# nirvanesque/headCT_foundation

Hardware: AMD Instinct MI355X
Metric: CT-volumes/sec MAE pretrain step (96^3, ViT-B/16^3, mask 0.75) (higher is better)
Workload: dtype bf16; 1 GPU; BASELINE config #2: MAE ViT-B/16^3, 96^3x1ch, mask 0.75, full train step (fwd+bwd+clip+AdamW+LR); per_gpu_batch=256, global_batch=256, parallelism=dp1, init=reference init, seed 42

## Files before the change

headct_foundation_amd/_lib.py:

```python
from __future__ import annotations

import ctypes as C
import os
from typing import Optional

HERE = os.path.dirname(os.path.abspath(__file__))
LIB_PATH = os.path.join(HERE, "libheadct_hip.so")

HCT_F32, HCT_BF16, HCT_F16 = 0, 1, 2
NORM_LAYERNORM, NORM_RMSNORM = 0, 1
HCT_ACT_NONE, HCT_ACT_GELU, HCT_ACT_DGELU, HCT_ACT_TANH, HCT_ACT_GELU_D, HCT_ACT_MULAUX = 0, 1, 2, 3, 4, 5
ACT_NONE, ACT_GELU, ACT_DGELU = 0, 1, 2

c_void_p, c_int, c_float, c_size_t, c_int64 = C.c_void_p, C.c_int, C.c_float, C.c_size_t, C.c_int64


class GemmArgs(C.Structure):
    _fields_ = [
        ("M", c_int), ("N", c_int), ("K", c_int),
        ("A", c_void_p), ("a_dtype", c_int), ("lda", c_int64), ("transA", c_int),
        ("B", c_void_p), ("b_dtype", c_int), ("ldb", c_int64), ("transB", c_int),
        ("C", c_void_p), ("c_dtype", c_int), ("ldc", c_int64),
        ("bias", c_void_p), ("residual", c_void_p), ("ldr", c_int64),
        ("act", c_int),
        ("aux", c_void_p), ("aux_dtype", c_int), ("ldaux", c_int64),
        ("C2", c_void_p), ("c2_dtype", c_int), ("ldc2", c_int64),
        ("alpha", c_float), ("force_generic", c_int), ("colsum_out", c_void_p), ("workspace_armed", c_int),
    ]


class GemmPlanInfo(C.Structure):
    _fields_ = [("kernel", c_int), ("epilogue_mode", c_int), ("fuse_colsum", c_int), ("row_tiles_per_wave", c_int), ("tiles", c_int),
                ("grid", c_int), ("sk_tiles", c_int), ("sk_wgs", c_int), ("splits", c_int), ("r_chunk", c_int), ("colsum_bytes", c_size_t),
                ("stream_k_offset", c_size_t), ("slab_bytes", c_size_t), ("workspace_bytes", c_size_t), ("walk_width", c_int)]


class ProfShape(C.Structure):
    _fields_ = [("M", c_int), ("N", c_int), ("K", c_int), ("mode", c_int), ("tiles", c_int), ("sk_tiles", c_int),
                ("launches", c_int64), ("total_ms", C.c_double), ("work", C.c_double), ("bytes", C.c_double)]


def prof_shapes(lib, kernel_class: int, cap: int = 256):
    buf = (ProfShape * cap)()
    n = lib.hct_prof_shapes(kernel_class, C.cast(buf, c_void_p), cap)
    if n < 0:
        raise HctError("hct_prof_shapes failed")
    return [buf[i] for i in range(min(n, cap))]


class MaeConfig(C.Structure):
    _fields_ = [
        ("input_size", c_int), ("patch_size", c_int), ("in_chans", c_int), ("mask_ratio", C.c_double),
        ("pos_embed", c_int),
        ("encoder_depth", c_int), ("encoder_embed_dim", c_int), ("encoder_mlp_dim", c_int), ("encoder_num_heads", c_int),
        ("decoder_depth", c_int), ("decoder_embed_dim", c_int), ("decoder_mlp_dim", c_int), ("decoder_num_heads", c_int),
        ("norm_pix_loss", c_int), ("use_bias", c_int),
        ("encoder_only", c_int), ("num_register_tokens", c_int), ("final_norm_eps", c_float),
        ("lora_rank", c_int),
        ("norm_kind", c_int),
        ("dropout_rate", c_float),
        ("drop_path_rate", c_float),
        ("patch_dropout", C.c_double),
    ]


class ParamInfo(C.Structure):
    _fields_ = [
        ("name", C.c_char * 96), ("ndim", c_int), ("shape", c_int64 * 5), ("offset", c_int64), ("numel", c_int64),
        ("requires_grad", c_int), ("is_matrix", c_int), ("bf16_t_offset", c_int64),
    ]


_PROTOS = {
    "hct_last_error_string": (C.c_char_p, []),
    "hct_version": (c_int, []),
    "hct_has_mfma_kernels": (c_int, []),
    "hct_gemm_workspace_bytes": (c_size_t, [C.POINTER(GemmArgs)]),
    "hct_gemm_nt_flags_offset": (c_size_t, [c_size_t]),
    "hct_gemm_describe": (c_int, [C.POINTER(GemmArgs), c_int, c_size_t, C.POINTER(GemmPlanInfo)]),
    "hct_gemm_stream_k_items": (c_int, [c_int, c_int, c_int, c_int, C.POINTER(C.c_uint32), C.POINTER(C.c_uint32)]),
    "hct_gemm_nt_walk": (c_int, [c_int, c_int, c_int, c_int, C.POINTER(c_int)]),
    "hct_set_cu_reserve": (None, [c_int]),
    "hct_gemm": (c_int, [C.POINTER(GemmArgs), c_void_p, c_size_t, c_void_p]),
    "hct_mask_rank": (c_int, [c_void_p, c_int, c_int, c_int, c_void_p, c_void_p, c_void_p, c_void_p]),
    "hct_patch_gather": (c_int, [c_void_p, c_int, c_void_p, c_int, c_int, c_int, c_int, c_int, c_int, c_void_p, c_int, c_void_p]),
    "hct_encoder_assemble_fwd": (c_int, [c_void_p, c_int, c_void_p, c_void_p, c_void_p, c_int, c_int, c_int, c_int, c_void_p, c_void_p]),
    "hct_encoder_assemble_bwd": (c_int, [c_void_p, c_void_p, c_int, c_int, c_int, c_int, c_void_p, c_int, c_void_p, c_void_p, c_void_p, c_size_t, c_void_p]),
    "hct_assemble_bwd_workspace_bytes": (c_size_t, [c_int]),
    "hct_layernorm_fwd": (c_int, [c_void_p, c_void_p, c_void_p, c_int, c_int, c_float, c_void_p, c_int, c_void_p, c_void_p, c_void_p]),
    "hct_layernorm_bwd_workspace_bytes": (c_size_t, [c_int, c_int]),
    "hct_layernorm_bwd": (c_int, [c_void_p, c_int, c_void_p, c_void_p, c_void_p, c_void_p, c_void_p, c_int, c_int, c_void_p, c_void_p,
                                  c_int, c_void_p, c_void_p, c_void_p, c_void_p, c_size_t, c_void_p]),
    "hct_layernorm_bwd_mapped": (c_int, [c_void_p, c_int, c_void_p, c_void_p, c_void_p, c_void_p, c_void_p, c_void_p, c_int, c_int, c_void_p,
                                         c_void_p, c_int, c_void_p, c_void_p, c_void_p, c_void_p, c_size_t, c_void_p]),
    "hct_rmsnorm_fwd": (c_int, [c_void_p, c_void_p, c_int, c_int, c_float, c_void_p, c_int, c_void_p, c_void_p]),
    "hct_rmsnorm_bwd_workspace_bytes": (c_size_t, [c_int, c_int]),
    "hct_rmsnorm_bwd": (c_int, [c_void_p, c_int, c_void_p, c_void_p, c_void_p, c_void_p, c_int, c_int, c_void_p, c_void_p, c_int, c_void_p,
                                c_void_p, c_void_p, c_size_t, c_void_p]),
    "hct_rmsnorm_bwd_mapped": (c_int, [c_void_p, c_int, c_void_p, c_void_p, c_void_p, c_void_p, c_void_p, c_int, c_int, c_void_p, c_void_p,
                                       c_int, c_void_p, c_void_p, c_void_p, c_size_t, c_void_p]),
    "hct_tail_rows": (c_int, [c_void_p, c_int, c_int, c_int, c_void_p, c_void_p, c_void_p]),
    "hct_gather_rows": (c_int, [c_void_p, c_void_p, c_int, c_int, c_void_p, c_void_p]),
    "hct_attention_fwd": (c_int, [c_void_p, c_int, c_int, c_int, c_int, c_int, c_void_p, c_void_p, c_void_p]),
    "hct_attention_bwd": (c_int, [c_void_p, c_void_p, c_void_p, c_void_p, c_int, c_int, c_int, c_int, c_int, c_void_p, c_void_p]),
    "hct_debug_force_simple_attention": (None, [c_int]),
    "hct_dropout_mask": (c_int, [C.c_uint64, c_int, c_int, c_int64, c_int, c_int, c_float, c_void_p, c_void_p]),
    "hct_dropout_apply": (c_int, [c_void_p, c_int, c_void_p, c_int, c_void_p, c_void_p, c_void_p, c_int64, c_int64, c_int64, c_int64, C.c_uint64,
                                  c_int, c_float, c_void_p]),
    "hct_attention_dropout_fwd": (c_int, [c_void_p, c_int, c_int, c_int, c_int, c_int, c_float, C.c_uint64, c_int, c_void_p, c_void_p, c_void_p]),
    "hct_attention_dropout_bwd": (c_int, [c_void_p, c_void_p, c_void_p, c_void_p, c_int, c_int, c_int, c_int, c_int, c_float, C.c_uint64, c_int,
                                          c_void_p, c_void_p]),
    "hct_drop_path_scales": (c_int, [C.c_uint64, C.POINTER(c_int), C.POINTER(c_float), c_int, c_int, c_void_p, c_void_p]),
    "hct_residual_drop_apply": (c_int, [c_void_p, c_int, c_void_p, c_int, c_void_p, c_int64, c_int64, c_void_p, C.c_uint64, c_int, c_float,
                                        c_void_p]),
    "hct_mae_plan_set_dropout": (c_int, [c_void_p, c_int, C.c_uint64]),
    "hct_decoder_assemble_fwd": (c_int, [c_void_p, c_int, c_void_p, c_void_p, c_void_p, c_void_p, c_int, c_int, c_int, c_int, c_void_p, c_void_p]),
    "hct_decoder_assemble_bwd": (c_int, [c_void_p, c_void_p, c_void_p, c_int, c_int, c_int, c_int, c_void_p, c_int, c_void_p, c_void_p,
                                         c_void_p, c_size_t, c_void_p]),
    "hct_masked_mse": (c_int, [c_void_p, c_int, c_void_p, c_int, c_void_p, c_int, c_int, c_int, c_int, c_int, c_float, c_void_p, c_void_p, c_void_p, c_void_p, c_void_p]),
    "hct_unpatchify": (c_int, [c_void_p, c_int, c_int, c_int, c_int, c_int, c_int, c_void_p, c_void_p]),
    "hct_vit_assemble_fwd": (c_int, [c_void_p, c_int, c_void_p, c_void_p, c_void_p, c_int, c_int, c_int, c_int, c_void_p, c_void_p]),
    "hct_channel_norm": (c_int, [c_void_p, c_void_p, c_void_p, c_float, c_void_p, c_int, c_int64, c_int, c_void_p]),
    "hct_query_attention": (c_int, [c_void_p, c_int, c_void_p, c_int, c_int, c_int, c_int, c_int, c_float, c_void_p, c_void_p]),
    "hct_head_linear": (c_int, [c_void_p, c_int64, c_int, c_void_p, c_void_p, c_float, c_void_p, c_void_p, c_int, c_void_p, c_int, c_int,
                                c_int, c_void_p]),
    "hct_batchnorm_stats": (c_int, [c_void_p, c_int, c_int, c_float, c_void_p, c_void_p, c_void_p, c_void_p, c_void_p]),
    "hct_softmax_xent": (c_int, [c_void_p, c_void_p, c_int, c_int, c_void_p, c_void_p, c_void_p, c_void_p]),
    "hct_sigmoid_bce_workspace_bytes": (c_size_t, [c_int, c_int]),
    "hct_sigmoid_bce": (c_int, [c_void_p, c_void_p, c_void_p, c_int, c_int, c_void_p, c_void_p, c_void_p, c_void_p, c_void_p, c_size_t, c_void_p]),
    "hct_mix_volumes": (c_int, [c_void_p, c_int, c_int, c_int, c_void_p, c_void_p, c_void_p]),
    "hct_mix_xent": (c_int, [c_void_p, c_void_p, c_void_p, c_float, c_int, c_int, c_void_p, c_void_p, c_void_p, c_void_p]),
    "hct_head_linear_wgrad": (c_int, [c_void_p, c_void_p, c_void_p, c_float, c_void_p, c_int, c_int, c_int, c_void_p, c_void_p, c_void_p]),
    "hct_bn_rows_workspace_bytes": (c_size_t, [c_int, c_int]),
    "hct_bn_stats_rows": (c_int, [c_void_p, c_int, c_int64, c_int, c_int, c_float, c_void_p, c_void_p, c_void_p, c_void_p, c_void_p,
                                  c_size_t, c_void_p]),
    "hct_bn_norm": (c_int, [c_void_p, c_int, c_int64, c_int64, c_int, c_void_p, c_void_p, c_float, c_void_p, c_int, c_void_p]),
    "hct_bn_bwd_input": (c_int, [c_void_p, c_int, c_int64, c_void_p, c_void_p, c_float, c_void_p, c_int64, c_void_p, c_void_p, c_int,
                                 c_int, c_int, c_int, c_void_p, c_int, c_int64, c_void_p, c_size_t, c_void_p]),
    "hct_head_linear_x": (c_int, [c_void_p, c_int, c_int64, c_int, c_void_p, c_void_p, c_float, c_void_p, c_void_p, c_void_p, c_int,
                                  c_int, c_int, c_void_p]),
    "hct_head_linear_bwd": (c_int, [c_void_p, c_int, c_int64, c_int, c_void_p, c_void_p, c_float, c_void_p, c_int, c_int, c_int,
                                    c_void_p, c_void_p, c_void_p]),
    "hct_query_attention_lse": (c_int, [c_void_p, c_int, c_void_p, c_int, c_int, c_int, c_int, c_int, c_float, c_void_p, c_void_p,
                                        c_void_p]),
    "hct_query_attention_bwd_workspace_bytes": (c_size_t, [c_int, c_int, c_int, c_int]),
    "hct_query_attention_bwd": (c_int, [c_void_p, c_int, c_void_p, c_int, c_int, c_int, c_int, c_int, c_float, c_void_p, c_void_p,
                                        c_void_p, c_void_p, c_void_p, c_void_p, c_size_t, c_void_p]),
    "hct_clip_total_norm": (c_int, [c_void_p, c_int64, c_void_p, c_int, c_float, c_void_p, c_void_p]),
    "hct_add_f32": (c_int, [c_void_p, c_void_p, c_int64, c_void_p]),
    "hct_dino_loss_workspace_bytes": (c_size_t, [c_int, c_int, c_int]),
    "hct_dino_loss": (c_int, [c_void_p, c_void_p, c_int, c_int, c_int, c_int, c_void_p, c_float, c_float, c_void_p, c_void_p, c_void_p, c_void_p,
                              c_void_p, c_size_t, c_void_p]),
    "hct_dino_center_update": (c_int, [c_void_p, c_void_p, c_int, C.c_double, C.c_double, c_void_p]),
    "hct_dino_sk_workspace_bytes": (c_size_t, [c_int, c_int]),
    "hct_dino_sk_col_lse": (c_int, [c_void_p, c_int, c_int, c_int, c_float, c_void_p, c_void_p, c_void_p, c_size_t, c_void_p]),
    "hct_dino_sk_row_lse": (c_int, [c_void_p, c_int, c_int, c_int, c_float, c_void_p, c_void_p, c_void_p]),
    "hct_dino_loss_sk_workspace_bytes": (c_size_t, [c_int, c_int, c_int]),
    "hct_dino_loss_sk": (c_int, [c_void_p, c_void_p, c_int, c_int, c_int, c_int, c_void_p, c_void_p, c_float, c_float, c_float, c_void_p, c_void_p,
                                 c_void_p, c_void_p, c_size_t, c_void_p]),
    "hct_koleo_fwd": (c_int, [c_void_p, c_int, c_int, c_int, c_int64, c_void_p, c_void_p, c_void_p, c_void_p, c_void_p]),
    "hct_koleo_bwd": (c_int, [c_void_p, c_int, c_int, c_int, c_int64, c_void_p, c_void_p, c_void_p, c_void_p, c_void_p, c_int64, c_void_p]),
    "hct_ema_update": (c_int, [c_void_p, c_void_p, c_int64, C.c_double, c_void_p]),
    "hct_l2norm_rows_fwd": (c_int, [c_void_p, c_int, c_int, c_void_p, c_int, c_void_p, c_void_p]),
    "hct_l2norm_rows_bwd": (c_int, [c_void_p, c_void_p, c_int, c_void_p, c_int, c_int, c_void_p, c_void_p]),
    "hct_weight_norm_fwd": (c_int, [c_void_p, c_void_p, c_int, c_int, c_void_p, c_int, c_void_p, c_void_p]),
    "hct_weight_norm_bwd": (c_int, [c_void_p, c_void_p, c_void_p, c_void_p, c_int, c_int, c_void_p, c_void_p, c_void_p]),
    "hct_bn_gelu_fwd": (c_int, [c_void_p, c_void_p, c_void_p, c_void_p, c_void_p, c_float, c_int, c_int, c_void_p, c_int, c_void_p, c_void_p, c_void_p]),
    "hct_bn_gelu_bwd_sums": (c_int, [c_void_p, c_int, c_void_p, c_void_p, c_int, c_int, c_void_p, c_void_p]),
    "hct_bn_gelu_bwd_apply": (c_int, [c_void_p, c_int, c_void_p, c_void_p, c_void_p, c_void_p, c_float, c_void_p, C.c_double, c_int, c_int, c_void_p, c_int,
                                      c_void_p]),
    "hct_hu_window": (c_int, [c_void_p, c_int, c_void_p, c_int, c_int, c_int64, c_int, c_void_p, c_void_p, c_void_p]),
    "hct_augment_volume": (c_int, [c_void_p, c_int, c_void_p, c_int, c_int, c_int, c_void_p, c_void_p, c_void_p]),
    "hct_gather_augment": (c_int, [c_void_p, c_void_p, c_void_p, c_int, c_int, c_int, c_int64, c_void_p, c_void_p, c_void_p]),
    "hct_affine_augment": (c_int, [c_void_p, c_int, c_void_p, c_int64, c_void_p, c_int, c_int, c_int, c_void_p, c_void_p, c_void_p, c_void_p,
                                   c_void_p]),
    "hct_gaussian_smooth3d": (c_int, [c_void_p, c_void_p, c_void_p, c_int, c_int, c_int, c_void_p, c_void_p, c_void_p]),
    "hct_crop_resize_area": (c_int, [c_void_p, c_int, c_int, c_int, c_int, c_void_p, c_int, c_int, c_void_p, c_void_p, c_void_p, c_void_p]),
    "hct_adjust_contrast_workspace_bytes": (c_size_t, [c_int, c_int64]),
    "hct_adjust_contrast": (c_int, [c_void_p, c_int, c_int64, c_void_p, c_void_p, c_void_p, c_size_t, c_void_p]),
    "hct_volume_to_ras": (c_int, [c_void_p, c_int, c_int, c_int, c_int, C.POINTER(c_int), C.POINTER(c_int), c_int, C.c_double, C.c_double,
                                  c_void_p, c_void_p]),
    "hct_bspline3_resample_workspace_bytes": (c_size_t, [c_int] * 6),
    "hct_bspline3_resample": (c_int, [c_void_p, c_int, c_int, c_int, c_void_p, c_int, c_int, c_int, c_void_p, c_void_p, c_void_p, c_size_t, c_void_p]),
    "hct_foreground_bbox_workspace_bytes": (c_size_t, [c_int] * 3),
    "hct_foreground_bbox": (c_int, [c_void_p, c_int, c_int, c_int, c_void_p, c_void_p, c_void_p, c_size_t, c_void_p]),
    "hct_crop_window_resize_area": (c_int, [c_void_p, c_int, c_int, c_int, c_void_p, c_int, c_void_p, c_void_p, c_void_p, c_int, c_int, c_int,
                                            c_void_p]),
# ... 154 lines not shown
```

headct_foundation_amd/csrc/attention.hip:

```cpp
#include "common.h"
#include "philox.h"
#include "prof.h"

namespace hct {
int attention_fwd_simple(const void* qkv, int B, int N, int H, int dh, int dtype, void* o, float* lse, hipStream_t s);
int attention_bwd_simple(const void* qkv, const void* o, const void* d_o, const float* lse, int B, int N, int H, int dh,
                         int dtype, void* dqkv, hipStream_t s);
bool attention_mfma_supported(int N, int H, int dh);
int attention_fwd_mfma(const void* qkv, int B, int N, int H, int dh, void* o, float* lse, hipStream_t s);
int attention_bwd_mfma(const void* qkv, const void* o, const void* d_o, const float* lse, int B, int N, int H, int dh,
                       void* dqkv, hipStream_t s);
int attention_dropout_fwd_simple(const void* qkv, int B, int N, int H, int dh, int dtype, void* o, float* lse, const DropArgs& da, hipStream_t s);
int attention_dropout_bwd_simple(const void* qkv, const void* o, const void* d_o, const float* lse, int B, int N, int H, int dh,
                                 int dtype, void* dqkv, const DropArgs& da, hipStream_t s);
int attention_dropout_fwd_mfma(const void* qkv, int B, int N, int H, int dh, void* o, float* lse, const DropArgs& da, hipStream_t s);
int attention_dropout_bwd_mfma(const void* qkv, const void* o, const void* d_o, const float* lse, int B, int N, int H, int dh, void* dqkv,
                               const DropArgs& da, hipStream_t s);
int check_drop_rate(const char* who, float p);
int g_force_simple_attention = 0;
extern int g_attn_general;
}

using namespace hct;

extern "C" {

void hct_debug_force_simple_attention(int mode) {
  g_force_simple_attention = mode == 1;
  g_attn_general = mode == 2;
}

int hct_attention_fwd(const void* qkv, int B, int N, int H, int dh, int dtype, void* o, float* lse, void* stream) {
  HCT_REQUIRE(B > 0 && N > 0 && H > 0 && dh > 0, "hct_attention_fwd: bad shape");
  ProfScope ps(PROF_ATTN_FWD, 4.0 * B * H * (double)N * N * dh, (hipStream_t)stream);
  if (dtype == HCT_BF16 && !g_force_simple_attention && attention_mfma_supported(N, H, dh))
    return attention_fwd_mfma(qkv, B, N, H, dh, o, lse, (hipStream_t)stream);
  return attention_fwd_simple(qkv, B, N, H, dh, dtype, o, lse, (hipStream_t)stream);
}

int hct_attention_bwd(const void* qkv, const void* o, const void* d_o, const float* lse, int B, int N, int H, int dh,
                      int dtype, void* dqkv, void* stream) {
  HCT_REQUIRE(B > 0 && N > 0 && H > 0 && dh > 0, "hct_attention_bwd: bad shape");
  ProfScope ps(PROF_ATTN_BWD, 10.0 * B * H * (double)N * N * dh, (hipStream_t)stream);
  if (dtype == HCT_BF16 && !g_force_simple_attention && attention_mfma_supported(N, H, dh))
    return attention_bwd_mfma(qkv, o, d_o, lse, B, N, H, dh, dqkv, (hipStream_t)stream);
  return attention_bwd_simple(qkv, o, d_o, lse, B, N, H, dh, dtype, dqkv, (hipStream_t)stream);
}

int hct_attention_dropout_fwd(const void* qkv, int B, int N, int H, int dh, int dtype, float p, uint64_t seed, int site, void* o, float* lse,
                              void* stream) {
  HCT_REQUIRE(B > 0 && N > 0 && H > 0 && dh > 0 && site >= 0, "hct_attention_dropout_fwd: bad shape or site");
  if (int rc = check_drop_rate("hct_attention_dropout_fwd", p)) return rc;
  const DropArgs da = make_drop_args(seed, site, p);
  ProfScope ps(PROF_ATTN_FWD, 4.0 * B * H * (double)N * N * dh, (hipStream_t)stream);
  if (dtype == HCT_BF16 && !g_force_simple_attention && attention_mfma_supported(N, H, dh))
    return attention_dropout_fwd_mfma(qkv, B, N, H, dh, o, lse, da, (hipStream_t)stream);
  return attention_dropout_fwd_simple(qkv, B, N, H, dh, dtype, o, lse, da, (hipStream_t)stream);
}

int hct_attention_dropout_bwd(const void* qkv, const void* o, const void* d_o, const float* lse, int B, int N, int H, int dh, int dtype, float p,
                              uint64_t seed, int site, void* dqkv, void* stream) {
  HCT_REQUIRE(B > 0 && N > 0 && H > 0 && dh > 0 && site >= 0, "hct_attention_dropout_bwd: bad shape or site");
  if (int rc = check_drop_rate("hct_attention_dropout_bwd", p)) return rc;
  const DropArgs da = make_drop_args(seed, site, p);
  ProfScope ps(PROF_ATTN_BWD, 10.0 * B * H * (double)N * N * dh, (hipStream_t)stream);
  if (dtype == HCT_BF16 && !g_force_simple_attention && attention_mfma_supported(N, H, dh))
    return attention_dropout_bwd_mfma(qkv, o, d_o, lse, B, N, H, dh, dqkv, da, (hipStream_t)stream);
  return attention_dropout_bwd_simple(qkv, o, d_o, lse, B, N, H, dh, dtype, dqkv, da, (hipStream_t)stream);
}

}
```

headct_foundation_amd/csrc/attention_mfma.hip:

```cpp
#include "common.h"
#include "philox.h"

#include <type_traits>

namespace hct {

int g_attn_general = 0;

namespace {

constexpr int kRowBytes = 128;

__device__ __forceinline__ int img_off(int r, int c) { return r * kRowBytes + ((c ^ ((r >> 1) & 7)) << 4); }

template <int DH>
__device__ __forceinline__ void load_image(unsigned char* img, const bf16* __restrict__ g, int64_t rs, int N, int Npad,
                                           int nthreads) {
  constexpr int U = 8;
  const int total = Npad * 8;
  for (int base = threadIdx.x; base < total; base += nthreads * U) {
    bf16x8 v[U];
#pragma unroll
    for (int u = 0; u < U; ++u) {
      const int idx = base + u * nthreads;
      const int r = idx >> 3, c = idx & 7;
      v[u] = bf16x8{0, 0, 0, 0, 0, 0, 0, 0};
      if (idx < total && r < N && c * 8 < DH) v[u] = *reinterpret_cast<const bf16x8*>(g + (int64_t)r * rs + c * 8);
    }
#pragma unroll
    for (int u = 0; u < U; ++u) {
      const int idx = base + u * nthreads;
      if (idx < total) *reinterpret_cast<bf16x8*>(img + img_off(idx >> 3, idx & 7)) = v[u];
    }
  }
}

__device__ __forceinline__ void dma_image128(unsigned char* img, const bf16* __restrict__ g, int64_t rs, int N, int Npad, int valid_cols,
                                             int wave, int nwaves, int lane) {
  const int64_t bytes = ((int64_t)(N - 1) * rs + valid_cols) * 2;
  __amdgpu_buffer_rsrc_t rsrc = __builtin_amdgcn_make_buffer_rsrc((void*)g, 0, bytes > 0xFFFFFFFFll ? 0xFFFFFFFFu : (uint32_t)bytes, 0x00020000);
  const int pieces = Npad * 8 / 64;
  for (int p = wave; p < pieces; p += nwaves) {
    const int ci = p * 64 + lane;
    const int row = ci >> 3, slot = ci & 7;
    const uint32_t voff = (uint32_t)(row * (int)rs * 2 + ((slot ^ ((row >> 1) & 7)) << 4));
    __builtin_amdgcn_raw_ptr_buffer_load_lds(rsrc, (__attribute__((address_space(3))) void*)(img + p * 1024), 16, voff, 0, 0, 0);
  }
}

template <int DH>
__device__ __forceinline__ void compute_delta(const bf16* __restrict__ ob, const bf16* __restrict__ dob, int64_t os,
                                              const float* __restrict__ lse_row, int N, int Npad, float* sLse, float* sDel,
                                              int nthreads, float lse_mul = 1.44269504088896340736f, float del_mul = 1.0f) {
  constexpr int U = 4;
  const int total = Npad * 8;
  for (int base = threadIdx.x; base < total; base += nthreads * U) {
    bf16x8 a[U], d[U];
#pragma unroll
    for (int u = 0; u < U; ++u) {
      const int idx = base + u * nthreads;
      const int r = idx >> 3, c = idx & 7;
      a[u] = d[u] = bf16x8{0, 0, 0, 0, 0, 0, 0, 0};
      if (idx < total && r < N && c * 8 < DH) {
        a[u] = *reinterpret_cast<const bf16x8*>(ob + (int64_t)r * os + c * 8);
        d[u] = *reinterpret_cast<const bf16x8*>(dob + (int64_t)r * os + c * 8);
      }
    }
#pragma unroll
    for (int u = 0; u < U; ++u) {
      const int idx = base + u * nthreads;
      float part = 0.f;
#pragma unroll
      for (int e = 0; e < 8; ++e) part += (float)a[u][e] * (float)d[u][e];
      part += __shfl_xor(part, 1, 64);
      part += __shfl_xor(part, 2, 64);
      part += __shfl_xor(part, 4, 64);
      if (idx < total && (idx & 7) == 0) {
        const int r = idx >> 3;
        sDel[r] = r < N ? part * del_mul : 0.f;
        sLse[r] = r < N ? lse_row[r] * lse_mul : (lse_mul < 0.f ? -INFINITY : INFINITY);
      }
    }
  }
}

__device__ __forceinline__ bf16x8 frag_row(const unsigned char* img, int r0, int ks, int lane) {
  const int r = r0 + (lane & 15), c = ks * 4 + (lane >> 4);
  return *reinterpret_cast<const bf16x8*>(img + img_off(r, c));
}

__device__ __forceinline__ bf16x8 frag_tr(const unsigned char* img, int rA, int rB, int d0, int lane) {
  const int g = lane >> 4, qq = (lane & 15) >> 2, pp = lane & 3;
  const int c = (d0 >> 3) + (pp >> 1), sub = (pp & 1) * 8;
  const unsigned char* pa = img + img_off(rA + 4 * g + qq, c) + sub;
  const unsigned char* pb = img + img_off(rB + 4 * g + qq, c) + sub;
  s16x4 lo = __builtin_amdgcn_ds_read_tr16_b64_v4i16((__attribute__((address_space(3))) s16x4*)(pa));
  s16x4 hi = __builtin_amdgcn_ds_read_tr16_b64_v4i16((__attribute__((address_space(3))) s16x4*)(pb));
  typedef __attribute__((ext_vector_type(8))) short s16x8;
  s16x8 v = {lo[0], lo[1], lo[2], lo[3], hi[0], hi[1], hi[2], hi[3]};
  return __builtin_bit_cast(bf16x8, v);
}

__device__ __forceinline__ bf16x8 pack8(f32x4 a, f32x4 b) {
  bf16x8 v = {(bf16)a[0], (bf16)a[1], (bf16)a[2], (bf16)a[3], (bf16)b[0], (bf16)b[1], (bf16)b[2], (bf16)b[3]};
  return v;
}

#define MFMA(a, b, c) __builtin_amdgcn_mfma_f32_16x16x32_bf16(a, b, c, 0, 0, 0)

__device__ __forceinline__ int xcd_bh() {
  const int n = gridDim.x, i = blockIdx.x;
  const int xcd = i & 7, q = n >> 3, r = n & 7;
  return (xcd < r ? xcd * (q + 1) : r * (q + 1) + (xcd - r) * q) + (i >> 3);
}

template <int DH, bool DROP = false>
__global__ void __launch_bounds__(256) attn_fwd_mfma_kernel(const bf16* __restrict__ qkv, int N, int H, int Npad,
                                                            bf16* __restrict__ o, float* __restrict__ lse, DropArgs da = DropArgs{}) {
  extern __shared__ __attribute__((aligned(16))) unsigned char smem[];
  unsigned char* Kimg = smem;
  unsigned char* Vimg = smem + Npad * kRowBytes;
  const int lane = threadIdx.x & 63, wave = threadIdx.x >> 6;
  const int bh = xcd_bh(), b = bh / H, h = bh - b * H;
  const int64_t rs = (int64_t)3 * H * DH;
  const bf16* qb = qkv + (int64_t)b * N * rs + h * DH;
  load_image<DH>(Kimg, qb + H * DH, rs, N, Npad, 256);
  load_image<DH>(Vimg, qb + 2 * H * DH, rs, N, Npad, 256);
  __syncthreads();
  const float scale = rsqrtf((float)DH);
  const int g = lane >> 4;
  constexpr int ND = DH / 16;
  const int nqt = (N + 15) >> 4;
  for (int qt = wave; qt < nqt; qt += 4) {
    const int q = qt * 16 + (lane & 15);
    bf16x8 qf[2];
#pragma unroll
    for (int ks = 0; ks < 2; ++ks) {
      const int d = ks * 32 + 8 * g;
      bf16x8 v = {0, 0, 0, 0, 0, 0, 0, 0};
      if (q < N && d < DH) v = *reinterpret_cast<const bf16x8*>(qb + (int64_t)q * rs + d);
      qf[ks] = v;
    }
    float m = -INFINITY, lsum = 0.f;
    f32x4 oacc[ND];
#pragma unroll
    for (int dt = 0; dt < ND; ++dt) oacc[dt] = f32x4{0, 0, 0, 0};
    for (int s = 0; s < (Npad >> 5); ++s) {
      const int k0 = s * 32;
      f32x4 st0 = {0, 0, 0, 0}, st1 = {0, 0, 0, 0};
#pragma unroll
      for (int ks = 0; ks < 2; ++ks) {
        st0 = MFMA(frag_row(Kimg, k0, ks, lane), qf[ks], st0);
        st1 = MFMA(frag_row(Kimg, k0 + 16, ks, lane), qf[ks], st1);
      }
      float mx = -INFINITY;
#pragma unroll
      for (int r = 0; r < 4; ++r) {
        st0[r] = (k0 + 4 * g + r < N) ? st0[r] * scale : -INFINITY;
        st1[r] = (k0 + 16 + 4 * g + r < N) ? st1[r] * scale : -INFINITY;
        mx = fmaxf(mx, fmaxf(st0[r], st1[r]));
      }
      mx = fmaxf(mx, __shfl_xor(mx, 16, 64));
      mx = fmaxf(mx, __shfl_xor(mx, 32, 64));
      const float mnew = fmaxf(m, mx);
      const float corr = __expf(m - mnew);
      float ps = 0.f;
#pragma unroll
      for (int r = 0; r < 4; ++r) {
        st0[r] = __expf(st0[r] - mnew);
        st1[r] = __expf(st1[r] - mnew);
        ps += st0[r] + st1[r];
      }
      lsum = lsum * corr + ps;
      if constexpr (DROP) {
        const Philox4 z0 = drop_words_attn(da, (uint32_t)((k0 >> 2) + g), (uint32_t)q, (uint32_t)bh);
        const Philox4 z1 = drop_words_attn(da, (uint32_t)((k0 >> 2) + 4 + g), (uint32_t)q, (uint32_t)bh);
#pragma unroll
        for (int r = 0; r < 4; ++r) {
          st0[r] *= drop_mul(da, z0.w[r]);
          st1[r] *= drop_mul(da, z1.w[r]);
        }
      }
      const bf16x8 pb = pack8(st0, st1);
#pragma unroll
      for (int dt = 0; dt < ND; ++dt) {
        oacc[dt] = oacc[dt] * corr;
        oacc[dt] = MFMA(frag_tr(Vimg, k0, k0 + 16, dt * 16, lane), pb, oacc[dt]);
      }
      m = mnew;
    }
    lsum += __shfl_xor(lsum, 16, 64);
    lsum += __shfl_xor(lsum, 32, 64);
    if (q < N) {
      const float inv = 1.0f / lsum;
      bf16* orow = o + ((int64_t)b * N + q) * (H * DH) + h * DH + 4 * g;
#pragma unroll
      for (int dt = 0; dt < ND; ++dt) Vec4<bf16>::store(orow + dt * 16, oacc[dt] * inv);
      if (g == 0) lse[(int64_t)bh * N + q] = m + __logf(lsum);
    }
  }
}

template <int DH, int NT, int NW = (NT <= 4 ? 4 : 8)>
__global__ void __launch_bounds__(NW * 64) attn_fwd_row_kernel(const bf16* __restrict__ qkv, int N, int H, bf16* __restrict__ o,
                                                           float* __restrict__ lse) {
  constexpr int Npad = NT * 16;
  extern __shared__ __attribute__((aligned(16))) unsigned char smem[];
  unsigned char* Kimg = smem;
  unsigned char* Vimg = smem + Npad * kRowBytes;
  const int lane = threadIdx.x & 63, wave = threadIdx.x >> 6;
  const int bh = xcd_bh(), b = bh / H, h = bh - b * H;
  const int64_t rs = (int64_t)3 * H * DH;
  const bf16* qb = qkv + (int64_t)b * N * rs + h * DH;
  const int g = lane >> 4;
  constexpr int ND = DH / 16;
  constexpr int MAXT = (NT + NW - 1) / NW;
  const int nqt = (N + 15) >> 4;
  constexpr int QA = MAXT <= 2 ? MAXT : 1;
  bf16x8 qall[QA][2];
  auto load_q = [&](int it, bf16x8* dst) {
    const int q = (wave + it * NW) * 16 + (lane & 15);
#pragma unroll
    for (int ks = 0; ks < 2; ++ks) {
      const int d = ks * 32 + 8 * g;
      bf16x8 v = {0, 0, 0, 0, 0, 0, 0, 0};
      if (q < N && d < DH) v = *reinterpret_cast<const bf16x8*>(qb + (int64_t)q * rs + d);
      dst[ks] = v;
    }
  };
#pragma unroll
  for (int it = 0; it < QA; ++it) load_q(it, qall[it]);
  dma_image128(Kimg, qb + H * DH, rs, N, Npad, DH, wave, NW, lane);
  dma_image128(Vimg, qb + 2 * H * DH, rs, N, Npad, DH, wave, NW, lane);
  __syncthreads();
  const float scale = rsqrtf((float)DH) * 1.44269504088896340736f;
#pragma unroll
  for (int it = 0; it < MAXT; ++it) {
    const int qt = wave + it * NW;
    if (qt >= nqt) break;
    const int q = qt * 16 + (lane & 15);
    bf16x8 qf[2];
    if constexpr (MAXT <= 2) { qf[0] = qall[it][0]; qf[1] = qall[it][1]; }
    else if (it == 0) { qf[0] = qall[0][0]; qf[1] = qall[0][1]; }
    else load_q(it, qf);
    f32x4 st[NT];
#pragma unroll
    for (int t = 0; t < NT; ++t) {
      st[t] = MFMA(frag_row(Kimg, t * 16, 0, lane), qf[0], (f32x4{0, 0, 0, 0}));
      st[t] = MFMA(frag_row(Kimg, t * 16, 1, lane), qf[1], st[t]);
    }
    constexpr int kPrevNT = NT <= 4 ? 0 : NT <= 10 ? 4 : NT <= 14 ? 10 : NT <= 18 ? 14 : 18;
    float mraw = -INFINITY;
#pragma unroll
    for (int t = 0; t < NT; ++t)
#pragma unroll
      for (int r = 0; r < 4; ++r) {
        if (t >= kPrevNT && t * 16 + 4 * g + r >= N) st[t][r] = -INFINITY;
        mraw = fmaxf(mraw, st[t][r]);
      }
    mraw = fmaxf(mraw, __shfl_xor(mraw, 16, 64));
    mraw = fmaxf(mraw, __shfl_xor(mraw, 32, 64));
    const float mx = mraw * scale;
#pragma unroll
    for (int t = 0; t < NT; ++t)
#pragma unroll
      for (int r = 0; r < 4; ++r) st[t][r] = __builtin_amdgcn_exp2f(fmaf(st[t][r], scale, -mx));
    const bf16 one = (bf16)1.0f, zero = (bf16)0.0f, ov = (lane & 3) == 0 ? one : zero;
    const bf16x8 ones_rows = {ov, ov, ov, ov, ov, ov, ov, ov};
    f32x4 oacc[ND], psum = {0, 0, 0, 0};
#pragma unroll
    for (int dt = 0; dt < ND; ++dt) oacc[dt] = f32x4{0, 0, 0, 0};
#pragma unroll
    for (int s2 = 0; s2 < NT / 2; ++s2) {
      const bf16x8 pb = pack8(st[2 * s2], st[2 * s2 + 1]);
#pragma unroll
      for (int dt = 0; dt < ND; ++dt) oacc[dt] = MFMA(frag_tr(Vimg, s2 * 32, s2 * 32 + 16, dt * 16, lane), pb, oacc[dt]);
      psum = MFMA(ones_rows, pb, psum);
    }
    const float ps = psum[0];
    if (q < N) {
      const float inv = 1.0f / ps;
      bf16* orow = o + ((int64_t)b * N + q) * (H * DH) + h * DH + 4 * g;
#pragma unroll
      for (int dt = 0; dt < ND; ++dt) Vec4<bf16>::store(orow + dt * 16, oacc[dt] * inv);
      if (g == 0) lse[(int64_t)bh * N + q] = (mx + __builtin_amdgcn_logf(ps)) * 0.69314718055994530942f;
    }
  }
}

template <int DH>
__device__ __forceinline__ bf16x8 gfrag(const bf16* __restrict__ base, int64_t rs, int r0, int ks, int lane, int N) {
  const int r = r0 + (lane & 15), d = ks * 32 + 8 * (lane >> 4);
  bf16x8 v = {0, 0, 0, 0, 0, 0, 0, 0};
  if (r < N && d < DH) v = *reinterpret_cast<const bf16x8*>(base + (int64_t)r * rs + d);
  return v;
}

constexpr int kBwd2WavesPerEU = 4;
template <int DH, int NW, bool DROP = false>
__global__ void __launch_bounds__(NW * 64, (NW >= 8 ? kBwd2WavesPerEU : 2)) attn_bwd2_mfma_kernel(const bf16* __restrict__ qkv, const bf16* __restrict__ o,
                                                                const bf16* __restrict__ d_o, const float* __restrict__ lse,
                                                                int N, int H, int Npad, bf16* __restrict__ dqkv, DropArgs da = DropArgs{}) {
  extern __shared__ __attribute__((aligned(16))) unsigned char smem[];
  unsigned char* img0 = smem;
  unsigned char* img1 = smem + Npad * kRowBytes;
  float* sLse = reinterpret_cast<float*>(img1 + Npad * kRowBytes);
  float* sDel = sLse + Npad;
  const int lane = threadIdx.x & 63, wave = threadIdx.x >> 6;
  const int bh = xcd_bh(), b = bh / H, h = bh - b * H;
  const int64_t rs = (int64_t)3 * H * DH;
  const int64_t os = (int64_t)H * DH;
  const bf16* qb = qkv + (int64_t)b * N * rs + h * DH;
  const bf16* kb = qb + H * DH;
  const bf16* vb = qb + 2 * H * DH;
  const bf16* ob = o + (int64_t)b * N * os + h * DH;
  const bf16* dob = d_o + (int64_t)b * N * os + h * DH;
  const float scale = rsqrtf((float)DH);
  const float scale2 = scale * 1.44269504088896340736f;
  const int g = lane >> 4;
  constexpr int ND = DH / 16;
  const int npair = Npad >> 5;

  constexpr bool kAhead = DH != 64;
  bf16x8 kf[2], vf[2], kn[2], vn[2];
#pragma unroll
  for (int ks = 0; ks < 2; ++ks) {
    kf[ks] = gfrag<DH>(kb, rs, wave * 16, ks, lane, N);
    vf[ks] = gfrag<DH>(vb, rs, wave * 16, ks, lane, N);
  }
  load_image<DH>(img0, qb, rs, N, Npad, NW * 64);
  load_image<DH>(img1, dob, os, N, Npad, NW * 64);
  compute_delta<DH>(ob, dob, os, lse + (int64_t)bh * N, N, Npad, sLse, sDel, NW * 64, 1.44269504088896340736f, scale);
  __syncthreads();
  for (int kt = wave; kt * 16 < N; kt += NW) {
    const int key0 = kt * 16;
#pragma unroll
    for (int ks = 0; ks < 2; ++ks) {
      if (kAhead) {
        kn[ks] = gfrag<DH>(kb, rs, key0 + NW * 16, ks, lane, N);
        vn[ks] = gfrag<DH>(vb, rs, key0 + NW * 16, ks, lane, N);
      } else if (kt != wave) {
        kf[ks] = gfrag<DH>(kb, rs, key0, ks, lane, N);
        vf[ks] = gfrag<DH>(vb, rs, key0, ks, lane, N);
      }
    }
    const bool key_ok = key0 + (lane & 15) < N;
    const bool tail_tile = key0 + 16 > N;
    f32x4 dKt[ND], dVt[ND];
#pragma unroll
    for (int dt = 0; dt < ND; ++dt) dKt[dt] = dVt[dt] = f32x4{0, 0, 0, 0};
    for (int qp = 0; qp < npair; ++qp) {
      f32x4 P[2], dS[2];
      [[maybe_unused]] f32x4 Pz[2];
#pragma unroll
      for (int hh = 0; hh < 2; ++hh) {
        const int q0 = qp * 32 + hh * 16;
        f32x4 sacc = {0, 0, 0, 0}, dp = {0, 0, 0, 0};
#pragma unroll
        for (int ks = 0; ks < 2; ++ks) {
          sacc = MFMA(frag_row(img0, q0, ks, lane), kf[ks], sacc);
          dp = MFMA(frag_row(img1, q0, ks, lane), vf[ks], dp);
        }
        const f32x4 L4 = *reinterpret_cast<const f32x4*>(sLse + q0 + 4 * g);
        const f32x4 D4 = *reinterpret_cast<const f32x4*>(sDel + q0 + 4 * g);
#pragma unroll
        for (int r = 0; r < 4; ++r) {
          float pv = __builtin_amdgcn_exp2f(fmaf(sacc[r], scale2, -L4[r]));
// ... 267 lines not shown
            for (int r = 0; r < 4; ++r) {
              P[hh][r] = hct_prob(__builtin_amdgcn_exp2f(sacc[r] * scale2));
              dS[hh][r] = P[hh][r] * dp[r];
            }
          }
          const bf16x8 pa = pack8(P[0], P[1]);
          const bf16x8 dsa = pack8(dS[0], dS[1]);
          const bf16x4 d0 = {dsa[0], dsa[1], dsa[2], dsa[3]}, d1 = {dsa[4], dsa[5], dsa[6], dsa[7]};
          if (key0 < Npad) {
            *reinterpret_cast<bf16x4*>(dsT + dst_off(Npad, 0, key, g)) = d0;
            *reinterpret_cast<bf16x4*>(dsT + dst_off(Npad, 1, key, g)) = d1;
          }
#pragma unroll
          for (int dt = 0; dt < ND; ++dt) {
            if constexpr (kHoist) {
              dVt[t][dt] = MFMA(dT[dt], pa, dVt[t][dt]);
              dKt[t][dt] = MFMA(qT[dt], dsa, dKt[t][dt]);
            } else {
              dVt[t][dt] = MFMA(cols_lds<DH>(Dimg, q0, q0 + 16, dt * 16, lane), pa, dVt[t][dt]);
              dKt[t][dt] = MFMA(cols_lds<DH>(Qimg, q0, q0 + 16, dt * 16, lane), dsa, dKt[t][dt]);
            }
          }
        }
      }
    }
    __syncthreads();
    for (int dt = wave; dt < ND; dt += GS) {
      f32x4 dq0 = {0, 0, 0, 0}, dq1 = {0, 0, 0, 0};
      const int G = lane >> 4, qq = (lane & 15) >> 2, pp = lane & 3;
      auto ds_frag = [&](int hh, int k0) -> bf16x8 {
        const int ka = k0 + 4 * G + qq;
        s16x4 lo = __builtin_amdgcn_ds_read_tr16_b64_v4i16((__attribute__((address_space(3))) s16x4*)(dsT + dst_off(Npad, hh, ka, pp)));
        s16x4 hi = __builtin_amdgcn_ds_read_tr16_b64_v4i16((__attribute__((address_space(3))) s16x4*)(dsT + dst_off(Npad, hh, ka + 16, pp)));
        typedef __attribute__((ext_vector_type(8))) short s16x8;
        s16x8 v = {lo[0], lo[1], lo[2], lo[3], hi[0], hi[1], hi[2], hi[3]};
        return __builtin_bit_cast(bf16x8, v);
      };
      bf16x8 kT = cols_lds<DH>(Kimg, 0, 16, dt * 16, lane), b0 = ds_frag(0, 0), b1 = ds_frag(1, 0);
      for (int k0 = 32; k0 < Npad; k0 += 32) {
        const bf16x8 kTn = cols_lds<DH>(Kimg, k0, k0 + 16, dt * 16, lane), b0n = ds_frag(0, k0), b1n = ds_frag(1, k0);
        dq0 = MFMA(kT, b0, dq0);
        dq1 = MFMA(kT, b1, dq1);
        kT = kTn; b0 = b0n; b1 = b1n;
      }
      dq0 = MFMA(kT, b0, dq0);
      dq1 = MFMA(kT, b1, dq1);
      const int q = q0 + (lane & 15);
      if (q < N) Vec4<bf16>::store(dqkv + ((int64_t)b * N + q) * rs + h * DH + dt * 16 + 4 * g, dq0 * scale);
      if (q + 16 < N) Vec4<bf16>::store(dqkv + ((int64_t)b * N + q + 16) * rs + h * DH + dt * 16 + 4 * g, dq1 * scale);
    }
    __syncthreads();
  }
#pragma unroll
  for (int t = 0; t < KT; ++t) {
    const int key = key_base + t * 16 + (lane & 15);
    if (key < N) {
      bf16* outk = dqkv + ((int64_t)b * N + key) * rs + H * DH + h * DH + 4 * g;
      bf16* outv = outk + H * DH;
#pragma unroll
      for (int dt = 0; dt < ND; ++dt) {
        Vec4<bf16>::store(outk + dt * 16, dKt[t][dt] * scale);
        Vec4<bf16>::store(outv + dt * 16, dVt[t][dt]);
      }
    }
  }
}

template <int DH>
inline size_t bwd3_lds(int Npad) { return (size_t)3 * Npad * HeadImg<DH>::kRow + (size_t)2 * Npad * 32 + (size_t)2 * Npad * sizeof(float); }


typedef __attribute__((ext_vector_type(4))) int attn_i32x4;
typedef __attribute__((ext_vector_type(2))) unsigned int u32x2a;
__device__ __forceinline__ attn_i32x4 attn_srd(const void* base, int64_t bytes) {
  const uint64_t pa = (uint64_t)base;
  const uint32_t rec = bytes > 0xFFFFFFFFll ? 0xFFFFFFFFu : (bytes < 0 ? 0u : (uint32_t)bytes);
  return attn_i32x4{(int)__builtin_amdgcn_readfirstlane((uint32_t)pa), (int)(__builtin_amdgcn_readfirstlane((uint32_t)(pa >> 32)) & 0xFFFF),
                    (int)__builtin_amdgcn_readfirstlane(rec), 0x00020000};
}
__device__ __forceinline__ void attn_dma16(attn_i32x4 rsrc, uint32_t lds_base, uint32_t voff) {
  asm volatile("s_mov_b32 m0, %0\n\ts_nop 0\n\tbuffer_load_dwordx4 %1, %2, 0 offen lds" ::"s"(lds_base), "v"(voff), "s"(rsrc) : "memory", "m0");
}

template <int DH, int Npad, int KT = 2>
__global__ void __launch_bounds__(1024 / KT, 2 * 2 / KT) attn_bwd4_kernel(const bf16* __restrict__ qkv, const bf16* __restrict__ o,
                                                           const bf16* __restrict__ d_o, const float* __restrict__ lse, int N, int H,
                                                           bf16* __restrict__ dqkv, int nbh) {
  extern __shared__ __attribute__((aligned(16))) unsigned char smem[];
  constexpr int ROW = HeadImg<DH>::kRow, CH = HeadImg<DH>::kChunks, ND = DH / 16, NW = 16 / KT;
  constexpr int img = Npad * ROW;
  constexpr int bufsz = 3 * img + 32 + 2 * Npad * 4;
  unsigned char* const dsT0 = smem + 2 * bufsz;
  constexpr int dstsz = 2 * Npad * 32;
  const uint32_t lds0 = (uint32_t)(size_t)((__attribute__((address_space(3))) unsigned char*)smem);
  const int lane = threadIdx.x & 63, wave = __builtin_amdgcn_readfirstlane(threadIdx.x >> 6);
  const int64_t rs = (int64_t)3 * H * DH, os = (int64_t)H * DH;
  const float scale = rsqrtf((float)DH);
  const float scale2 = scale * 1.44269504088896340736f;
  const int key_base = wave * (KT * 16);
  constexpr int nqb = Npad >> 5;
  constexpr int pieces = Npad * CH / 64;
  constexpr int MAXP = (pieces + NW - 1) / NW;
  auto opaque = [](int v) { asm volatile("" : "+v"(v)); return v; };
  if (threadIdx.x < 16) {
    *reinterpret_cast<uint32_t*>(smem + (threadIdx.x >> 3) * bufsz + 3 * img + (threadIdx.x & 7) * 4) = 0u;
  }
  auto item_bh = [&](int item) {
    const int xcd = item & 7, q = nbh >> 3, r = nbh & 7;
    return (xcd < r ? xcd * (q + 1) : r * (q + 1) + (xcd - r) * q) + (item >> 3);
  };
  int dq_hh, dq_dt0, dq_n;
  if (KT == 1) {
    dq_hh = wave - (NW - 2); dq_dt0 = 0; dq_n = wave >= NW - 2 ? ND : 0;
  } else if (key_base >= Npad) { dq_hh = 0; dq_dt0 = 0; dq_n = ND; }
  else if (8 * KT * 16 > Npad) { dq_hh = 1; dq_dt0 = wave - 4; dq_n = (wave >= 4 && wave < 4 + ND) ? 1 : 0; }
  else { dq_hh = (wave - 2) / ND; dq_dt0 = (wave - 2) - dq_hh * ND; dq_n = wave >= 2 ? 1 : 0; }

  auto prefetch_images = [&](int item, int buf) {
    const int bh = item_bh(item), b = bh / H, h = bh - b * H;
    const bf16* qb = qkv + (int64_t)b * N * rs + h * DH;
    const bf16* dob = d_o + (int64_t)b * N * os + h * DH;
    const attn_i32x4 rq = attn_srd(qb, ((int64_t)(N - 1) * rs + DH) * 2);
    const attn_i32x4 rk = attn_srd(qb + H * DH, ((int64_t)(N - 1) * rs + DH) * 2);
    const attn_i32x4 rd = attn_srd(dob, ((int64_t)(N - 1) * os + DH) * 2);
    const uint32_t base = lds0 + buf * bufsz;
    const int ln = opaque(lane);
#pragma unroll
    for (int i = 0; i < MAXP; ++i) {
      const int p = wave + NW * i;
      if (p < pieces) {
        const int ci = p * 64 + ln, row = ci / CH, slot = ci - row * CH;
        const uint32_t src = (uint32_t)((DH == 48 ? slot : (slot ^ ((row >> 1) & 7))) * 16);
        const uint32_t vq = (uint32_t)row * (uint32_t)(rs * 2) + src, vd = (uint32_t)row * (uint32_t)(os * 2) + src;
        attn_dma16(rq, base + p * 1024, vq);
        attn_dma16(rd, base + img + p * 1024, vd);
        attn_dma16(rk, base + 2 * img + p * 1024, vq);
      }
    }
  };
  RowFrag<DH> vfN[KT];
  constexpr int NU = (Npad * 8 + NW * 64 - 1) / (NW * 64);
  bf16x8 oN[NU];
  float lN = 0.f;
  auto prefetch_regs = [&](int item) {
    const int bh = item_bh(item), b = bh / H, h = bh - b * H;
    const bf16* vb = qkv + (int64_t)b * N * rs + 2 * H * DH + h * DH;
    const int ln = opaque(lane), tid = wave * 64 + ln;
#pragma unroll
    for (int t = 0; t < KT; ++t) vfN[t] = rows_global<DH>(vb, rs, key_base + t * 16, ln, N);
    const bf16* ob = o + (int64_t)b * N * os + h * DH;
#pragma unroll
    for (int u = 0; u < NU; ++u) {
      const int idx = tid + u * NW * 64, r = idx >> 3, c = idx & 7;
      oN[u] = bf16x8{0, 0, 0, 0, 0, 0, 0, 0};
      if (r < N && c * 8 < DH) oN[u] = *reinterpret_cast<const bf16x8*>(ob + (int64_t)r * os + c * 8);
    }
    lN = tid < N ? lse[(int64_t)bh * N + tid] : 0.f;
  };

  int item = blockIdx.x;
  if (item >= nbh) return;
  prefetch_images(item, 0);
  prefetch_regs(item);
  for (int it = 0; item < nbh; item += gridDim.x, ++it) {
    const int cur = it & 1;
    unsigned char* Qimg = smem + cur * bufsz;
    unsigned char* Dimg = Qimg + img;
    unsigned char* Kimg = Dimg + img;
    float* sLse = reinterpret_cast<float*>(Kimg + img + 32);
    float* sDel = sLse + Npad;
    const int bh = item_bh(item), b = bh / H, h = bh - b * H;
    asm volatile("" ::"v"(lN) : "memory");
    __builtin_amdgcn_s_barrier();
    RowFrag<DH> vf[KT];
#pragma unroll
    for (int t = 0; t < KT; ++t) vf[t] = vfN[t];
    RowFrag<DH> kfh = vf[0];
    if constexpr (KT == 1) kfh = rows_lds<DH>(Kimg, key_base < Npad ? key_base : 0, opaque(lane), true);
    const int tid_top = wave * 64 + opaque(lane);
#pragma unroll
    for (int u = 0; u < NU; ++u) {
      const int idx = tid_top + u * NW * 64, r = idx >> 3, c = idx & 7;
      float part = 0.f;
      if (idx < Npad * 8 && c * 8 < DH) {
        const bf16x8 dv = *reinterpret_cast<const bf16x8*>(Dimg + HeadImg<DH>::off(r, c));
#pragma unroll
        for (int e = 0; e < 8; ++e) part += (float)oN[u][e] * (float)dv[e];
      }
      part += __shfl_xor(part, 1, 64);
      part += __shfl_xor(part, 2, 64);
      part += __shfl_xor(part, 4, 64);
      if (idx < Npad * 8 && c == 0) sDel[r] = r < N ? part * scale : 0.f;
    }
    if (tid_top < Npad) sLse[tid_top] = tid_top < N ? lN * 1.44269504088896340736f : INFINITY;
    asm volatile("s_waitcnt lgkmcnt(0)" ::: "memory");
    __builtin_amdgcn_s_barrier();
    const int next = item + gridDim.x;
    if (next < nbh) prefetch_images(next, cur ^ 1);

    f32x4 dKt[KT][ND], dVt[KT][ND];
#pragma unroll
    for (int t = 0; t < KT; ++t)
#pragma unroll
      for (int dt = 0; dt < ND; ++dt) dKt[t][dt] = dVt[t][dt] = f32x4{0, 0, 0, 0};

    auto main_part = [&](int qbk) {
      const int q0 = qbk * 32;
      unsigned char* dsT = dsT0 + (qbk & 1) * dstsz;
      const int ln = KT == 1 ? opaque(lane) : lane, g = ln >> 4;
      RowFrag<DH> qr[2], dr[2];
      f32x4 L4[2], D4[2];
      if constexpr (KT > 1) {
#pragma unroll
        for (int hh = 0; hh < 2; ++hh) {
          qr[hh] = rows_lds<DH>(Qimg, q0 + 16 * hh, ln, true);
          dr[hh] = rows_lds<DH>(Dimg, q0 + 16 * hh, ln, false);
          L4[hh] = *reinterpret_cast<const f32x4*>(sLse + q0 + 16 * hh + 4 * g);
          D4[hh] = *reinterpret_cast<const f32x4*>(sDel + q0 + 16 * hh + 4 * g);
        }
      }
      bf16x8 qT[ND], dT[ND];
#pragma unroll
      for (int dt = 0; dt < ND; ++dt) {
        qT[dt] = cols_lds<DH>(Qimg, q0, q0 + 16, dt * 16, ln);
        dT[dt] = cols_lds<DH>(Dimg, q0, q0 + 16, dt * 16, ln);
      }
#pragma unroll
      for (int t = 0; t < KT; ++t) {
        const int key0 = key_base + t * 16;
        const RowFrag<DH> kf = KT == 1 ? kfh : rows_lds<DH>(Kimg, key0, ln, false);
        const int key = key0 + (ln & 15);
        f32x4 P[2], dS[2];
#pragma unroll
        for (int hh = 0; hh < 2; ++hh) {
          if constexpr (KT == 1) {
            qr[hh] = rows_lds<DH>(Qimg, q0 + 16 * hh, ln, false);
            dr[hh] = rows_lds<DH>(Dimg, q0 + 16 * hh, ln, false);
            L4[hh] = *reinterpret_cast<const f32x4*>(sLse + q0 + 16 * hh + 4 * g);
            D4[hh] = *reinterpret_cast<const f32x4*>(sDel + q0 + 16 * hh + 4 * g);
          }
          const f32x4 sacc = mma_rows<DH>(qr[hh], kf, f32x4{0, 0, 0, 0});
          const f32x4 dp = mma_rows<DH>(dr[hh], vf[t], f32x4{0, 0, 0, 0});
#pragma unroll
          for (int r = 0; r < 4; ++r) {
            P[hh][r] = hct_prob(__builtin_amdgcn_exp2f(fmaf(sacc[r], scale2, -L4[hh][r])));
            dS[hh][r] = P[hh][r] * fmaf(dp[r], scale, -D4[hh][r]);
          }
        }
        const bf16x8 pa = pack8(P[0], P[1]);
        const bf16x8 dsa = pack8(dS[0], dS[1]);
        const bf16x4 d0 = {dsa[0], dsa[1], dsa[2], dsa[3]}, d1 = {dsa[4], dsa[5], dsa[6], dsa[7]};
        *reinterpret_cast<bf16x4*>(dsT + dst_off(Npad, 0, key, g)) = d0;
        *reinterpret_cast<bf16x4*>(dsT + dst_off(Npad, 1, key, g)) = d1;
#pragma unroll
        for (int dt = 0; dt < ND; ++dt) {
          dVt[t][dt] = MFMA(dT[dt], pa, dVt[t][dt]);
          dKt[t][dt] = MFMA(qT[dt], dsa, dKt[t][dt]);
        }
      }
    };
    auto dq_tiles = [&](int qbk, int hh, int dt0, auto nt_tag, int ln) {
      constexpr int NT = decltype(nt_tag)::value;
      const unsigned char* dsT = dsT0 + (qbk & 1) * dstsz;
      const int qq = (ln & 15) >> 2, pp = ln & 3, g = ln >> 4;
      auto ds_frag = [&](int k0) -> bf16x8 {
        const int ka = k0 + 4 * g + qq;
        s16x4 lo = __builtin_amdgcn_ds_read_tr16_b64_v4i16((__attribute__((address_space(3))) s16x4*)(dsT + dst_off(Npad, hh, ka, pp)));
        s16x4 hi = __builtin_amdgcn_ds_read_tr16_b64_v4i16((__attribute__((address_space(3))) s16x4*)(dsT + dst_off(Npad, hh, ka + 16, pp)));
        typedef __attribute__((ext_vector_type(8))) short s16x8;
        s16x8 v = {lo[0], lo[1], lo[2], lo[3], hi[0], hi[1], hi[2], hi[3]};
        return __builtin_bit_cast(bf16x8, v);
      };
      f32x4 dq[NT];
#pragma unroll
      for (int j = 0; j < NT; ++j) dq[j] = f32x4{0, 0, 0, 0};
      constexpr int kHalf = (KT == 1 && NT > 1) ? (nqb + 1) / 2 : nqb;
#pragma unroll
      for (int k0 = 0; k0 < nqb; k0 += kHalf) {
        bf16x8 kT[kHalf][NT], bq[kHalf];
#pragma unroll
        for (int kb = 0; kb < kHalf; ++kb)
          if (k0 + kb < nqb) {
            bq[kb] = ds_frag((k0 + kb) * 32);
#pragma unroll
            for (int j = 0; j < NT; ++j) kT[kb][j] = cols_lds<DH>(Kimg, (k0 + kb) * 32, (k0 + kb) * 32 + 16, (dt0 + j) * 16, ln);
          }
#pragma unroll
        for (int kb = 0; kb < kHalf; ++kb)
          if (k0 + kb < nqb) {
#pragma unroll
            for (int j = 0; j < NT; ++j) dq[j] = MFMA(kT[kb][j], bq[kb], dq[j]);
          }
      }
      const int q = qbk * 32 + 16 * hh + (ln & 15);
#pragma unroll
      for (int j = 0; j < NT; ++j)
        if (q < N) Vec4<bf16>::store(dqkv + ((int64_t)b * N + q) * rs + h * DH + (dt0 + j) * 16 + 4 * g, dq[j]);
    };
    auto dq_part = [&](int qbk, int ln) {
      if (dq_n == 1) dq_tiles(qbk, dq_hh, dq_dt0, std::integral_constant<int, 1>{}, ln);
      else if (dq_n == ND) dq_tiles(qbk, dq_hh, dq_dt0, std::integral_constant<int, ND>{}, ln);
    };
    const bool owns_keys = key_base < Npad;
    for (int qbk = 0; qbk < nqb; ++qbk) {
      if (wave < NW / 2) {
        if (owns_keys) main_part(qbk);
        if (qbk > 0) dq_part(qbk - 1, KT == 1 ? opaque(lane) : lane);
      } else {
        if (qbk > 0) dq_part(qbk - 1, KT == 1 ? opaque(lane) : lane);
        if (owns_keys) main_part(qbk);
      }
      asm volatile("s_waitcnt lgkmcnt(0)" ::: "memory");
      __builtin_amdgcn_s_barrier();
    }
    if (next < nbh) prefetch_regs(next);
    dq_part(nqb - 1, opaque(lane));
    if (owns_keys) {
      const int ln = opaque(lane);
#pragma unroll
      for (int t = 0; t < KT; ++t) {
        const int key = key_base + t * 16 + (ln & 15);
        if (key < N) {
          bf16* outk = dqkv + ((int64_t)b * N + key) * rs + H * DH + h * DH + 4 * (ln >> 4);
          bf16* outv = outk + H * DH;
#pragma unroll
          for (int dt = 0; dt < ND; ++dt) {
            Vec4<bf16>::store(outk + dt * 16, dKt[t][dt]);
            Vec4<bf16>::store(outv + dt * 16, dVt[t][dt]);
          }
        }
      }
    }
  }
}

template <int DH, int KT>
__global__ void __launch_bounds__(256, 1) attn_bwd5_kernel(const bf16* __restrict__ qkv, const bf16* __restrict__ o,
                                                           const bf16* __restrict__ d_o, const float* __restrict__ lse, int N, int H,
                                                           int Npad, bf16* __restrict__ dqkv) {
  extern __shared__ __attribute__((aligned(16))) unsigned char smem[];
  constexpr int ROW = HeadImg<DH>::kRow, CH = HeadImg<DH>::kChunks, ND = DH / 16;
  constexpr int blk = 32 * ROW;
  unsigned char* const Kimg = smem;
  unsigned char* const ring = Kimg + Npad * ROW + 32;
  unsigned char* const dsT0 = ring + 4 * blk + 32;
  constexpr int kRows = 4 * KT * 16;
  constexpr int dstsz = 2 * kRows * 32;
  float* const sLse = reinterpret_cast<float*>(dsT0 + 2 * dstsz);
  float* const sDel = sLse + 64;
  const int lane = threadIdx.x & 63, wave = __builtin_amdgcn_readfirstlane(threadIdx.x >> 6);
  const int bh = xcd_bh(), b = bh / H, h = bh - b * H;
  const int64_t rs = (int64_t)3 * H * DH, os = (int64_t)H * DH;
  const bf16* qb = qkv + (int64_t)b * N * rs + h * DH;
  const bf16* kb = qb + H * DH;
  const bf16* vb = qb + 2 * H * DH;
  const bf16* ob = o + (int64_t)b * N * os + h * DH;
  const bf16* dob = d_o + (int64_t)b * N * os + h * DH;
  const float* lse_row = lse + (int64_t)bh * N;
  const float scale = rsqrtf((float)DH);
  const float scale2 = scale * 1.44269504088896340736f;
  const int g = lane >> 4;
  const int key_base = wave * (KT * 16);
  const int nqb = Npad >> 5;

  for (int i = threadIdx.x * 16; i < 4 * blk + 32; i += 256 * 16) *reinterpret_cast<f32x4*>(ring + i) = f32x4{0, 0, 0, 0};
  if (threadIdx.x < 2) *reinterpret_cast<f32x4*>(Kimg + Npad * ROW + threadIdx.x * 16) = f32x4{0, 0, 0, 0};
  dma_image<DH>(Kimg, kb, rs, N, Npad, wave, 4, lane);
  RowFrag<DH> vf[KT];
#pragma unroll
  for (int t = 0; t < KT; ++t) vf[t] = rows_global<DH>(vb, rs, key_base + t * 16, lane, N);

  const int srow = threadIdx.x >> 3, sc = threadIdx.x & 7;
  bf16x8 sq, sd, so;
  float sl = 0.f;
  auto stage_load = [&](int j) {
    const int r = j * 32 + srow;
    sq = sd = so = bf16x8{0, 0, 0, 0, 0, 0, 0, 0};
    if (r < N && sc < CH) {
      sq = *reinterpret_cast<const bf16x8*>(qb + (int64_t)r * rs + sc * 8);
      sd = *reinterpret_cast<const bf16x8*>(dob + (int64_t)r * os + sc * 8);
      so = *reinterpret_cast<const bf16x8*>(ob + (int64_t)r * os + sc * 8);
    }
    const int rl = j * 32 + (int)threadIdx.x;
    sl = (threadIdx.x < 32 && rl < N) ? lse_row[rl] : 0.f;
  };
  auto stage_write = [&](int j) {
    unsigned char* Qb = ring + (j & 1) * 2 * blk;
    if (sc < CH) {
      *reinterpret_cast<bf16x8*>(Qb + HeadImg<DH>::off(srow, sc)) = sq;
      *reinterpret_cast<bf16x8*>(Qb + blk + HeadImg<DH>::off(srow, sc)) = sd;
    }
    float part = 0.f;
#pragma unroll
    for (int e = 0; e < 8; ++e) part += (float)so[e] * (float)sd[e];
    part += __shfl_xor(part, 1, 64);
    part += __shfl_xor(part, 2, 64);
    part += __shfl_xor(part, 4, 64);
// ... 88 lines not shown
      constexpr int D = 4;
      bf16x8 kT[D], b0[D], b1[D];
#pragma unroll
      for (int u = 0; u < D; ++u) {
        const int k0 = u * 32 < Npad ? u * 32 : 0;
        kT[u] = cols_lds<DH>(Kimg, k0, k0 + 16, dt * 16, lane);
        b0[u] = ds_frag(0, k0);
        b1[u] = ds_frag(1, k0);
      }
      for (int k0 = 0; k0 < Npad; k0 += 32 * D) {
#pragma unroll
        for (int u = 0; u < D; ++u) {
          if (k0 + u * 32 < Npad) {
            dq0 = MFMA(kT[u], b0[u], dq0);
            dq1 = MFMA(kT[u], b1[u], dq1);
          }
          const int kn = k0 + (u + D) * 32;
          if (kn < Npad) {
            kT[u] = cols_lds<DH>(Kimg, kn, kn + 16, dt * 16, lane);
            b0[u] = ds_frag(0, kn);
            b1[u] = ds_frag(1, kn);
          }
        }
      }
      const int q = j * 32 + (lane & 15);
      if (q < N) Vec4<bf16>::store(dqkv + ((int64_t)b * N + q) * rs + h * DH + dt * 16 + 4 * g, dq0);
      if (q + 16 < N) Vec4<bf16>::store(dqkv + ((int64_t)b * N + q + 16) * rs + h * DH + dt * 16 + 4 * g, dq1);
    }
  };

  for (int j = 0; j < nqb; ++j) {
    if (j + 1 < nqb) stage_load(j + 1);
    main_part(j);
    if (j > 0) dq_part(j - 1);
    if (j + 1 < nqb) stage_write(j + 1);
    asm volatile("s_waitcnt lgkmcnt(0)" ::: "memory");
    __builtin_amdgcn_s_barrier();
  }
  dq_part(nqb - 1);
#pragma unroll
  for (int t = 0; t < KT; ++t) {
    const int key = key_base + t * 16 + (lane & 15);
    if (key < N) {
      bf16* outk = dqkv + ((int64_t)b * N + key) * rs + H * DH + h * DH + 4 * g;
      bf16* outv = outk + H * DH;
#pragma unroll
      for (int dt = 0; dt < ND; ++dt) {
        Vec4<bf16>::store(outk + dt * 16, dKt[t][dt]);
        Vec4<bf16>::store(outv + dt * 16, dVt[t][dt]);
      }
    }
  }
}
template <int DH>
inline size_t bwd5_lds(int Npad, int KT) { return (size_t)Npad * HeadImg<DH>::kRow + 32 + (size_t)4 * 32 * HeadImg<DH>::kRow + 32 + (size_t)2 * 2 * (4 * KT * 16) * 32 + 512; }

template <int DH>
constexpr size_t bwd4_lds(int Npad) { return (size_t)2 * (3 * Npad * HeadImg<DH>::kRow + 32 + 2 * Npad * 4) + (size_t)2 * (2 * Npad * 32); }

inline size_t bwd2_lds(int N) { return (size_t)2 * ((N + 31) / 32 * 32) * kRowBytes + (size_t)2 * ((N + 31) / 32 * 32) * sizeof(float); }

constexpr int kMaxLds = 160 * 1024;
inline int npad_of(int N) { return (N + 31) / 32 * 32; }
inline size_t fwd_lds(int N) { return (size_t)2 * npad_of(N) * kRowBytes; }

template <typename F>
int set_lds(F func, size_t bytes) {
  if (bytes <= 64 * 1024) return 0;
  return check_hip(hipFuncSetAttribute(reinterpret_cast<const void*>(func), hipFuncAttributeMaxDynamicSharedMemorySize, (int)bytes),
                   "hipFuncSetAttribute(LDS)");
}

}

bool attention_mfma_supported(int N, int H, int dh) {
  (void)H;
  return (dh == 48 || dh == 64) && fwd_lds(N) <= (size_t)kMaxLds && bwd2_lds(N) <= (size_t)kMaxLds;
}

template <int DH, int NT>
static int launch_fwd_row(const void* qkv, int B, int N, int H, void* o, float* lse, hipStream_t s) {
  const size_t lds = (size_t)2 * NT * 16 * kRowBytes;
  if (int rc = set_lds(attn_fwd_row_kernel<DH, NT>, lds)) return rc;
  hipLaunchKernelGGL((attn_fwd_row_kernel<DH, NT>), dim3(B * H), dim3(NT <= 4 ? 256 : 512), lds, s, (const bf16*)qkv, N, H, (bf16*)o, lse);
  return check_hip(hipGetLastError(), "attention_fwd_row");
}

static int num_cus_cached() {
  static int n = 0;
  if (n == 0) {
    int dev = 0;
    hipDeviceProp_t prop;
    n = (hipGetDevice(&dev) == hipSuccess && hipGetDeviceProperties(&prop, dev) == hipSuccess) ? prop.multiProcessorCount : 256;
  }
  return n;
}

int attention_fwd_mfma(const void* qkv, int B, int N, int H, int dh, void* o, float* lse, hipStream_t s) {
  const int Npad = npad_of(N);
  const size_t lds = fwd_lds(N);
  if (!g_attn_general) {
    const int nt = Npad / 16;
#define HCT_ROW(DH_, NT_) if (dh == DH_ && nt <= NT_) return launch_fwd_row<DH_, NT_>(qkv, B, N, H, o, lse, s)
    HCT_ROW(64, 4); HCT_ROW(48, 4); HCT_ROW(64, 10); HCT_ROW(48, 10); HCT_ROW(64, 14); HCT_ROW(48, 14); HCT_ROW(64, 18); HCT_ROW(48, 18);
    HCT_ROW(64, 34); HCT_ROW(48, 34);
#undef HCT_ROW
  }
  if (dh == 48) {
    if (int rc = set_lds(attn_fwd_mfma_kernel<48>, lds)) return rc;
    hipLaunchKernelGGL(attn_fwd_mfma_kernel<48>, dim3(B * H), dim3(256), lds, s, (const bf16*)qkv, N, H, Npad, (bf16*)o, lse, DropArgs{});
  } else {
    if (int rc = set_lds(attn_fwd_mfma_kernel<64>, lds)) return rc;
    hipLaunchKernelGGL(attn_fwd_mfma_kernel<64>, dim3(B * H), dim3(256), lds, s, (const bf16*)qkv, N, H, Npad, (bf16*)o, lse, DropArgs{});
  }
  return check_hip(hipGetLastError(), "attention_fwd_mfma");
}

int attention_bwd_mfma(const void* qkv, const void* o, const void* d_o, const float* lse, int B, int N, int H, int dh,
                       void* dqkv, hipStream_t s) {
  const int Npad = npad_of(N);
  const int ncu = num_cus_cached();
  const int nbh = B * H, grid = nbh < ncu ? nbh : ncu;
#define HCT_BWD4(DH_, NPAD_)                                                                                                  \
  do {                                                                                                                     \
    constexpr size_t l4 = bwd4_lds<DH_>(NPAD_);                                                                            \
    static_assert(l4 <= (size_t)kMaxLds, "bwd4 LDS");                                                                      \
    if (int rc = set_lds(attn_bwd4_kernel<DH_, NPAD_, 1>, l4)) return rc;                                                  \
    hipLaunchKernelGGL((attn_bwd4_kernel<DH_, NPAD_, 1>), dim3(grid), dim3(1024), l4, s, (const bf16*)qkv, (const bf16*)o, \
                       (const bf16*)d_o, lse, N, H, (bf16*)dqkv, nbh);                                                     \
    return check_hip(hipGetLastError(), "attention_bwd4");                                                                 \
  } while (0)
  if (!g_attn_general) {
    if (dh == 64 && Npad == 160) HCT_BWD4(64, 160);
    if (dh == 48 && Npad == 224) HCT_BWD4(48, 224);
    if (dh == 64 && Npad <= 64) {
      const size_t l3 = bwd3_lds<64>(Npad);
      if (int rc = set_lds(attn_bwd3_kernel<64, 4, 1, 4>, l3)) return rc;
      hipLaunchKernelGGL((attn_bwd3_kernel<64, 4, 1, 4>), dim3(B * H), dim3(4 * 64), l3, s, (const bf16*)qkv, (const bf16*)o,
                         (const bf16*)d_o, lse, N, H, Npad, (bf16*)dqkv, ncu, (int)(Npad * Npad / 4096));
      return check_hip(hipGetLastError(), "attention_bwd3");
    }
    if (dh == 48 && Npad > 448 && Npad <= 576) {
      const size_t l5 = bwd5_lds<48>(Npad, 9);
      if (int rc = set_lds(attn_bwd5_kernel<48, 9>, l5)) return rc;
      hipLaunchKernelGGL((attn_bwd5_kernel<48, 9>), dim3(B * H), dim3(256), l5, s, (const bf16*)qkv, (const bf16*)o, (const bf16*)d_o,
                         lse, N, H, Npad, (bf16*)dqkv);
      return check_hip(hipGetLastError(), "attention_bwd5");
    }
  }
#undef HCT_BWD4
  const size_t l2 = bwd2_lds(N);
#define HCT_BWD2(DH_, NW_)                                                                                           \
  do {                                                                                                               \
    if (int rc = set_lds(attn_bwd2_mfma_kernel<DH_, NW_>, l2)) return rc;                                            \
    hipLaunchKernelGGL((attn_bwd2_mfma_kernel<DH_, NW_>), dim3(B * H), dim3(NW_ * 64), l2, s, (const bf16*)qkv,       \
                       (const bf16*)o, (const bf16*)d_o, lse, N, H, Npad, (bf16*)dqkv, DropArgs{});                  \
  } while (0)
  const bool w8 = N > 64;
  const bool w16 = w8 && l2 > (size_t)81408;
  if (dh == 48) { if (w16) HCT_BWD2(48, 16); else if (w8) HCT_BWD2(48, 8); else HCT_BWD2(48, 4); }
  else { if (w16) HCT_BWD2(64, 16); else if (w8) HCT_BWD2(64, 8); else HCT_BWD2(64, 4); }
#undef HCT_BWD2
  return check_hip(hipGetLastError(), "attention_bwd2_mfma");
}

int attention_dropout_fwd_mfma(const void* qkv, int B, int N, int H, int dh, void* o, float* lse, const DropArgs& da, hipStream_t s) {
  const int Npad = npad_of(N);
  const size_t lds = fwd_lds(N);
  if (dh == 48) {
    if (int rc = set_lds(attn_fwd_mfma_kernel<48, true>, lds)) return rc;
    hipLaunchKernelGGL((attn_fwd_mfma_kernel<48, true>), dim3(B * H), dim3(256), lds, s, (const bf16*)qkv, N, H, Npad, (bf16*)o, lse, da);
  } else {
    if (int rc = set_lds(attn_fwd_mfma_kernel<64, true>, lds)) return rc;
    hipLaunchKernelGGL((attn_fwd_mfma_kernel<64, true>), dim3(B * H), dim3(256), lds, s, (const bf16*)qkv, N, H, Npad, (bf16*)o, lse, da);
  }
  return check_hip(hipGetLastError(), "attention_dropout_fwd_mfma");
}

int attention_dropout_bwd_mfma(const void* qkv, const void* o, const void* d_o, const float* lse, int B, int N, int H, int dh, void* dqkv,
                               const DropArgs& da, hipStream_t s) {
  const int Npad = npad_of(N);
  const size_t l2 = bwd2_lds(N);
#define HCT_BWD2D(DH_, NW_)                                                                                                 \
  do {                                                                                                                      \
    if (int rc = set_lds(attn_bwd2_mfma_kernel<DH_, NW_, true>, l2)) return rc;                                             \
    hipLaunchKernelGGL((attn_bwd2_mfma_kernel<DH_, NW_, true>), dim3(B * H), dim3(NW_ * 64), l2, s, (const bf16*)qkv,       \
                       (const bf16*)o, (const bf16*)d_o, lse, N, H, Npad, (bf16*)dqkv, da);                                 \
  } while (0)
  const bool w8 = N > 64, w16 = w8 && l2 > (size_t)81408;
  if (dh == 48) { if (w16) HCT_BWD2D(48, 16); else if (w8) HCT_BWD2D(48, 8); else HCT_BWD2D(48, 4); }
  else { if (w16) HCT_BWD2D(64, 16); else if (w8) HCT_BWD2D(64, 8); else HCT_BWD2D(64, 4); }
#undef HCT_BWD2D
  return check_hip(hipGetLastError(), "attention_dropout_bwd_mfma");
}

}
```

headct_foundation_amd/csrc/mae_plan.hip:

```cpp
#include <cstdlib>
#include "common.h"
#include "gemm_plan.h"

#include <algorithm>
#include <map>
#include <string>
#include <vector>

using namespace hct;

namespace {

constexpr int64_t kUnitElems = 1024;

struct BlockP {
  int ln1_w, ln1_b, qkv_w, qkv_b, proj_w, proj_b, ln2_w, ln2_b, fc1_w, fc1_b, fc2_w, fc2_b;
  int lq_b = -1, lq_a = -1, lv_b = -1, lv_a = -1;
  int site = 0;
  float path_q = 0.f;
  int path_row = 0;
};
struct BlockA {
  size_t x1, mean1, rstd1, qkv, o, lse, h_mid, x2, mean2, rstd2, u, g;
  size_t lora_t = 0;
};
struct Act { size_t off; int64_t rows, cols; int dtype; };
struct BlockG { size_t out, big, mid, qkv, lora_du = 0, lora_dt = 0, dm_out = 0, dm_mid = 0; };
constexpr int kWgSlots = 8;

struct Side {
  const std::vector<BlockP>& bp;
  const std::vector<BlockA>& ba;
  const std::vector<BlockG>& ring;
  const std::vector<size_t>& h;
  int N, d, m, heads;
};
enum class Rows {
  kEvery,
  kCat,
  kTail,
};
struct Mode {
  bool can = false;
  bool on = false;
  bool fwd = false;
};
struct SinkScope {
  FoldSink* prev;
  explicit SinkScope(FoldSink* sink) : prev(g_fold_sink) { g_fold_sink = sink; }
  ~SinkScope() { g_fold_sink = prev; }
};

}

struct hct_mae_plan {
  hct_mae_config cfg;
  int B, dt;
  int g, L, K, pd, Ne, Nd, Me, Md;
  int D, Dd, Mlp, Mlpd, H, Hd;
  std::vector<hct_param_info> params;
  std::map<std::string, int> pindex;
  int64_t param_elems = 0, bf16t_elems = 0;
  bool vit = false;
  bool keep = false;
  int R = 0;
  int lora = 0;
  int norm_kind = 0;
  float drop_p = 0.f;
  Mode drop;
  uint64_t drop_seed = 0;
  size_t s_drop_y = 0;
  Mode path;
  size_t s_path = 0;
  bool t_all_done = false;
  float norm_eps = 1e-5f;
  int p_reg = -1;
  int p_pe_w, p_pe_b, p_pos, p_cls, p_norm_w, p_norm_b, p_de_w, p_de_b, p_mask, p_dcls, p_dpos, p_dnorm_w, p_dnorm_b,
      p_pred_w, p_pred_b;
  std::vector<BlockP> enc, dec;
  std::vector<std::pair<int64_t, int64_t>> stage_range;
  size_t ws_bytes = 0;
  size_t a_ids_restore, a_ids_shuffle, a_mask, a_row_loss, a_patches, a_tok, a_latent, a_lat_mean, a_lat_rstd, a_e,
      a_ynorm, a_yn_mean, a_yn_rstd, a_pred, a_dpred;
  Mode tail;
  int Mc = 0;
  size_t a_tail_rows = 0, a_tail_inv = 0, a_oc = 0, s_dhc = 0;
  Mode dec0;
  int Rcat = 0;
  size_t a_kept_rows = 0, a_cat_idx = 0, a_hk = 0, a_x1c = 0, a_mean_c = 0, a_rstd_c = 0, a_qkv_cat = 0, a_dqkv_cat = 0, a_dcat = 0;
  std::vector<size_t> h_enc, h_dec;
  std::vector<BlockA> aenc, adec;
  size_t s_dh, s_dh_shadow, s_dx, s_do, s_small, s_small_bytes, s_gemm, s_gemm_bytes, s_nt_bytes = 0;
  size_t s_fold_a = 0, s_fold_b = 0, s_fold_bytes = 0, s_small2 = 0, s_small2_bytes = 0;
  bool defer_folds = true;
  std::map<std::string, Act> acts;
  bool wg_defer = false;
  int wg_blocks = 0;
  int wg_blocks_pending = 0, wg_slot = 0;
  std::vector<BlockG> genc, gdec;
  size_t a_de = 0, a_dtok = 0;
  std::vector<hct_gemm_args> wg_pending;
  std::vector<hct_gemm_args> wg_prepared[kWgSlots];
  size_t s_wg[kWgSlots] = {0}, s_wg_bytes = 0;
  int64_t final_off = 0;
  float* params_f32 = nullptr;
  float* grads = nullptr;
  bf16* params_bf16 = nullptr;
  bf16* params_bf16_t = nullptr;
  unsigned char* ws = nullptr;
  bool fwd_done = false;
  bool nt_ws_armed = false;
  bool dpred_done = false;
  const float* dloss = nullptr;

  size_t esz() const { return dtype_size(dt); }
  template <typename T> T* W(size_t off) const { return reinterpret_cast<T*>(ws + off); }
  const float* pf(int i) const { return i < 0 ? nullptr : params_f32 + params[i].offset; }
  float* gf(int i) const { return i < 0 ? nullptr : grads + params[i].offset; }
  const void* wop(int i) const { return dt == HCT_BF16 ? (const void*)(params_bf16 + params[i].offset) : (const void*)(params_f32 + params[i].offset); }
  const void* wop_t(int i) const { return (const void*)(params_bf16_t + params[i].bf16_t_offset); }
  int tr(int i) const { return i >= 0 && params[i].requires_grad ? i : -1; }
  Side enc_side() const { return Side{enc, aenc, genc, h_enc, Ne, D, Mlp, H}; }
  Side dec_side() const { return Side{dec, adec, gdec, h_dec, Nd, Dd, Mlpd, Hd}; }
  size_t out_grad(const Side& sd, int i) const { return i >= 0 ? sd.ring[i % sd.ring.size()].out : s_dh_shadow; }
  bool path_drops(const BlockP& bp) const { return path.fwd && bp.path_q > 0.f; }
  bool masks_residual(const BlockP& bp) const { return drop.fwd || path_drops(bp); }
  Rows decoder_rows(int i) const {
    return dec0.fwd && i == 0 ? Rows::kCat : tail.fwd && i == cfg.decoder_depth - 1 ? Rows::kTail : Rows::kEvery;
  }
};

namespace {

int add_param(hct_mae_plan* p, const std::string& name, std::vector<int64_t> shape, bool rg, bool matrix, bool needs_t) {
  hct_param_info pi;
  memset(&pi, 0, sizeof(pi));
  snprintf(pi.name, sizeof(pi.name), "%s", name.c_str());
  pi.ndim = (int)shape.size();
  int64_t n = 1;
  for (size_t i = 0; i < shape.size(); ++i) { pi.shape[i] = shape[i]; n *= shape[i]; }
  pi.numel = n;
  pi.offset = p->param_elems;
  pi.requires_grad = rg ? 1 : 0;
  pi.is_matrix = matrix ? 1 : 0;
  pi.bf16_t_offset = -1;
  if (needs_t) {
    pi.bf16_t_offset = p->bf16t_elems;
    p->bf16t_elems += (n + 63) / 64 * 64;
  }
  p->param_elems += (n + kUnitElems - 1) / kUnitElems * kUnitElems;
  p->params.push_back(pi);
  p->pindex[name] = (int)p->params.size() - 1;
  return (int)p->params.size() - 1;
}

BlockP add_block(hct_mae_plan* p, const std::string& pre, int d, int m, bool use_bias) {
  BlockP b;
  b.ln1_w = add_param(p, pre + ".att_norm.weight", {d}, true, false, false);
  b.ln1_b = p->norm_kind == 1 ? -1 : add_param(p, pre + ".att_norm.bias", {d}, true, false, false);
  b.qkv_w = add_param(p, pre + ".attn.qkv.weight", {3 * d, d}, true, true, true);
  b.qkv_b = use_bias ? add_param(p, pre + ".attn.qkv.bias", {3 * d}, true, false, false) : -1;
  b.proj_w = add_param(p, pre + ".attn.proj.weight", {d, d}, true, true, true);
  b.proj_b = add_param(p, pre + ".attn.proj.bias", {d}, true, false, false);
  if (p->lora > 0) {
    const int r = p->lora;
    b.lq_b = add_param(p, pre + ".attn.lora_q.lora_matrix_B", {d, r}, true, true, true);
    b.lv_b = add_param(p, pre + ".attn.lora_v.lora_matrix_B", {d, r}, true, true, true);
    b.lq_a = add_param(p, pre + ".attn.lora_q.lora_matrix_A", {r, d}, true, true, true);
    b.lv_a = add_param(p, pre + ".attn.lora_v.lora_matrix_A", {r, d}, true, true, true);
  }
  b.ln2_w = add_param(p, pre + ".ffn_norm.weight", {d}, true, false, false);
  b.ln2_b = p->norm_kind == 1 ? -1 : add_param(p, pre + ".ffn_norm.bias", {d}, true, false, false);
  b.fc1_w = add_param(p, pre + ".mlp.linear1.weight", {m, d}, true, true, true);
  b.fc1_b = add_param(p, pre + ".mlp.linear1.bias", {m}, true, false, false);
  b.fc2_w = add_param(p, pre + ".mlp.linear2.weight", {d, m}, true, true, true);
  b.fc2_b = add_param(p, pre + ".mlp.linear2.bias", {d}, true, false, false);
  return b;
}

constexpr int kMaxT = 112;
struct TransposeTable {
  int n;
  int tile_start[kMaxT + 1];
  int rows[kMaxT], cols[kMaxT];
  long long src[kMaxT], dst[kMaxT];
};

__global__ void __launch_bounds__(256) transpose_cast_batched_kernel(const float* __restrict__ src, bf16* __restrict__ dst,
                                                                     TransposeTable t) {
  __shared__ float tile[64][65];
  int lo = 0, hi = t.n;
  while (hi - lo > 1) {
    const int mid = (lo + hi) >> 1;
    if (t.tile_start[mid] <= (int)blockIdx.x) lo = mid; else hi = mid;
  }
  const int rows = t.rows[lo], cols = t.cols[lo];
  const int local = blockIdx.x - t.tile_start[lo];
  const int tcols = (cols + 63) >> 6;
  const int r0 = (local / tcols) * 64, c0 = (local % tcols) * 64;
  const float* s = src + t.src[lo];
  bf16* d = dst + t.dst[lo];
  const int q = threadIdx.x & 15, rr = threadIdx.x >> 4;
  const bool vec = (cols & 3) == 0 && (rows & 3) == 0;
  if (vec) {
#pragma unroll
    for (int i = 0; i < 4; ++i) {
      const int r = r0 + rr + 16 * i, c = c0 + q * 4;
      f32x4 v = {0, 0, 0, 0};
      if (r < rows && c < cols) v = Vec4<float>::load(s + (size_t)r * cols + c);
#pragma unroll
      for (int e = 0; e < 4; ++e) tile[rr + 16 * i][q * 4 + e] = v[e];
    }
    __syncthreads();
#pragma unroll
    for (int i = 0; i < 4; ++i) {
      const int c = c0 + rr + 16 * i, r = r0 + q * 4;
      if (c < cols && r < rows) {
        const f32x4 v = {tile[q * 4 + 0][rr + 16 * i], tile[q * 4 + 1][rr + 16 * i], tile[q * 4 + 2][rr + 16 * i], tile[q * 4 + 3][rr + 16 * i]};
        Vec4<bf16>::store(d + (size_t)c * rows + r, v);
      }
    }
    return;
  }
  const int tx = threadIdx.x & 63, ty = threadIdx.x >> 6;
  for (int i = ty; i < 64; i += 4) {
    const int r = r0 + i, c = c0 + tx;
    tile[i][tx] = (r < rows && c < cols) ? s[(size_t)r * cols + c] : 0.f;
  }
  __syncthreads();
  for (int i = ty; i < 64; i += 4) {
    const int c = c0 + i, r = r0 + tx;
    if (c < cols && r < rows) d[(size_t)c * rows + r] = (bf16)tile[tx][i];
  }
}

struct WsAlloc {
  size_t cur = 0;
  size_t take(size_t bytes) {
    size_t o = cur;
    cur += align_up(bytes ? bytes : 16, 256);
    return o;
  }
};

BlockA alloc_block(WsAlloc& w, size_t M, size_t d, size_t m, size_t heads_tokens, size_t es) {
  BlockA a;
  a.x1 = w.take(M * d * es);
  a.mean1 = w.take(M * 4);
  a.rstd1 = w.take(M * 4);
  a.qkv = w.take(M * 3 * d * es);
  a.o = w.take(M * d * es);
  a.lse = w.take(heads_tokens * 4);
  a.h_mid = w.take(M * d * 4);
  a.x2 = w.take(M * d * es);
  a.mean2 = w.take(M * 4);
  a.rstd2 = w.take(M * 4);
  a.u = w.take(M * m * es);
  a.g = w.take(M * m * es);
  return a;
}

#define RC(x)            \
  do {                   \
    int _rc = (x);       \
    if (_rc) return _rc; \
  } while (0)

constexpr float kRmsEps = 1e-6f;

int norm_fwd(hct_mae_plan* p, const float* x, const float* gamma, const float* beta, int rows, int D, float eps, void* y, int y_dtype,
             float* mean, float* rstd, hipStream_t s) {
  if (p->norm_kind == 1) return hct_rmsnorm_fwd(x, gamma, rows, D, kRmsEps, y, y_dtype, rstd, s);
  return hct_layernorm_fwd(x, gamma, beta, rows, D, eps, y, y_dtype, mean, rstd, s);
}

int norm_bwd(hct_mae_plan* p, const void* dy, int dy_dtype, const float* x, const float* mean, const float* rstd, const float* gamma,
             const float* dres, const int32_t* dres_rows, int rows, int D, float* dx, void* dx_shadow, int shadow_dtype, float* dgamma,
             float* dbeta, float* dcolsum, void* workspace, size_t workspace_bytes, hipStream_t s) {
  if (p->norm_kind == 1)
    return hct_rmsnorm_bwd_mapped(dy, dy_dtype, x, rstd, gamma, dres, dres_rows, rows, D, dx, dx_shadow, shadow_dtype, dgamma, dcolsum,
                                  workspace, workspace_bytes, s);
  return hct_layernorm_bwd_mapped(dy, dy_dtype, x, mean, rstd, gamma, dres, dres_rows, rows, D, dx, dx_shadow, shadow_dtype, dgamma, dbeta,
                                  dcolsum, workspace, workspace_bytes, s);
}

hct_gemm_args base_args() {
  hct_gemm_args a;
  memset(&a, 0, sizeof(a));
  a.alpha = 1.0f;
  return a;
}

int nt_gemm(hct_mae_plan* p, hct_gemm_args& a, hipStream_t s) {
  if (p->s_nt_bytes == 0) return hct_gemm(&a, a.colsum_out ? p->ws + p->s_small : nullptr, a.colsum_out ? p->s_small_bytes : 0, s);
  if (!p->nt_ws_armed) {
    if (hipMemsetAsync(p->ws + p->s_small + p->s_small_bytes, 0, p->s_nt_bytes, s) != hipSuccess) {
      set_error("plan: clearing the stream-K region of the GEMM workspace failed");
      return HCT_E_WORKSPACE;
    }
    p->nt_ws_armed = true;
  }
  a.workspace_armed = 1;
  return hct_gemm(&a, p->ws + p->s_small, p->s_small_bytes + p->s_nt_bytes, s);
}

int linear_fwd(hct_mae_plan* p, const void* X, int M, int K, int w, int b, int N, void* Y, int y_dtype, int act, void* aux,
               const float* residual, hipStream_t s) {
  hct_gemm_args a = base_args();
  a.M = M; a.N = N; a.K = K;
  a.A = X; a.a_dtype = p->dt; a.lda = K; a.transA = 0;
  a.B = p->wop(w); a.b_dtype = p->dt; a.ldb = K; a.transB = 1;
  a.C = Y; a.c_dtype = y_dtype; a.ldc = N;
  a.bias = p->pf(b);
  a.residual = residual; a.ldr = N;
  a.act = act; a.aux = aux; a.aux_dtype = p->dt; a.ldaux = N;
  return nt_gemm(p, a, s);
}

// ... 104 lines not shown
  std::vector<hct_gemm_args>& jobs = p->wg_pending;
  std::stable_sort(jobs.begin(), jobs.end(), [](const hct_gemm_args& x, const hct_gemm_args& y) { return x.K > y.K; });
  const int slot = p->wg_slot < kWgSlots ? p->wg_slot : kWgSlots - 1;
  ++p->wg_slot;
  const int n = (int)jobs.size();
  if (hct_gemm_tn_group_workspace_bytes(n) > p->s_wg_bytes) {
    set_error("plan: %d queued weight gradients exceed the grouped launch's workspace", n);
    return HCT_E_WORKSPACE;
  }
  std::vector<hct_gemm_args>& prep = p->wg_prepared[slot];
  if (prep.size() != jobs.size() || memcmp(prep.data(), jobs.data(), jobs.size() * sizeof(hct_gemm_args)) != 0) {
    RC(hct_gemm_tn_group_prepare(jobs.data(), n, p->ws + p->s_wg[slot], p->s_wg_bytes, s));
    prep = jobs;
  }
  RC(hct_gemm_tn_group_run(jobs.data(), n, p->ws + p->s_wg[slot], p->s_wg_bytes, s));
  jobs.clear();
  return 0;
}

int end_stage(hct_mae_plan* p, int stage, bool block_stage, bool boundary, int ring, int depth, hipStream_t s) {
  if (block_stage) ++p->wg_blocks_pending;
  const bool last = stage + 1 == (int)p->stage_range.size();
  int limit = p->wg_blocks > 0 ? p->wg_blocks : (1 << 30);
  if (ring > 0 && ring < depth && ring - 1 < limit) limit = ring - 1;
  if (last || boundary || p->wg_blocks_pending >= limit) RC(flush_wgrads(p, s));
  if (p->wg_pending.empty()) p->final_off = p->stage_range[stage].first;
  return 0;
}

constexpr int kActFc1 = HCT_ACT_GELU_D, kActFc2Dgrad = HCT_ACT_MULAUX;

int drop_apply(hct_mae_plan* p, const void* x, int x_dtype, void* y, int y_dtype, const float* residual, const void* x2, void* y2, int64_t n,
               int site, hipStream_t s) {
  return hct_dropout_apply(x, x_dtype, y, y_dtype, residual, x2, y2, 1, 0, 0, n, p->drop_seed, site, p->drop_p, s);
}
int branch_apply(hct_mae_plan* p, const BlockP& bp, int branch, const void* x, int x_dtype, void* y, int y_dtype, const float* residual, int M, int d,
                 hipStream_t s) {
  const int site = bp.site + 1 + 2 * branch;
  if (!p->path_drops(bp)) return drop_apply(p, x, x_dtype, y, y_dtype, residual, nullptr, nullptr, (int64_t)M * d, site, s);
  const float* scales = (const float*)(p->ws + p->s_path) + (size_t)(bp.path_row + branch) * p->B;
  return hct_residual_drop_apply(x, x_dtype, y, y_dtype, residual, p->B, (int64_t)(M / p->B) * d, scales, p->drop_seed, site,
                                 p->drop.fwd ? p->drop_p : 0.f, s);
}
int drop_embedding(hct_mae_plan* p, float* h, hipStream_t s) {
  const int64_t lead = 1 + p->R;
  return hct_dropout_apply(h, HCT_F32, h, HCT_F32, nullptr, nullptr, nullptr, p->B, (int64_t)p->Ne * p->D, lead * p->D, (int64_t)(p->Ne - lead) * p->D,
                           p->drop_seed, 0, p->drop_p, s);
}

int back_half_forward(hct_mae_plan* p, const BlockP& bp, const BlockA& ba, int M, const void* o, const float* h_in, float* h_out, int d, int m,
                      hipStream_t s) {
  unsigned char* ws = p->ws;
  float* h_mid = (float*)(ws + ba.h_mid);
  const bool masked = p->masks_residual(bp);
  void* y = ws + p->s_drop_y;
  if (masked) {
    RC(linear_fwd(p, o, M, d, bp.proj_w, bp.proj_b, d, y, p->dt, HCT_ACT_NONE, nullptr, nullptr, s));
    RC(branch_apply(p, bp, 0, y, p->dt, h_mid, HCT_F32, h_in, M, d, s));
  } else {
    RC(linear_fwd(p, o, M, d, bp.proj_w, bp.proj_b, d, h_mid, HCT_F32, HCT_ACT_NONE, nullptr, h_in, s));
  }
  RC(norm_fwd(p, h_mid, p->pf(bp.ln2_w), p->pf(bp.ln2_b), M, d, 1e-5f, ws + ba.x2, p->dt, (float*)(ws + ba.mean2), (float*)(ws + ba.rstd2), s));
  RC(linear_fwd(p, ws + ba.x2, M, d, bp.fc1_w, bp.fc1_b, m, ws + ba.g, p->dt, kActFc1, ws + ba.u, nullptr, s));
  if (!masked) return linear_fwd(p, ws + ba.g, M, m, bp.fc2_w, bp.fc2_b, d, h_out, HCT_F32, HCT_ACT_NONE, nullptr, h_mid, s);
  if (p->drop.fwd) RC(drop_apply(p, ws + ba.g, p->dt, ws + ba.g, p->dt, nullptr, ws + ba.u, ws + ba.u, (int64_t)M * m, bp.site + 2, s));
  RC(linear_fwd(p, ws + ba.g, M, m, bp.fc2_w, bp.fc2_b, d, y, p->dt, HCT_ACT_NONE, nullptr, nullptr, s));
  return branch_apply(p, bp, 1, y, p->dt, h_out, HCT_F32, h_mid, M, d, s);
}

int block_forward(hct_mae_plan* p, const Side& sd, int i, Rows rows, hipStream_t s) {
  const BlockP& bp = sd.bp[i];
  const BlockA& ba = sd.ba[i];
  const int B = p->B, N = sd.N, d = sd.d, heads = sd.heads, M = B * N;
  unsigned char* ws = p->ws;
  const float* h_in = (const float*)(ws + sd.h[i]);
  float* h_out = (float*)(ws + sd.h[i + 1]);
  if (rows == Rows::kCat) {
    const int Rc = p->Rcat, Nc = p->Me;
    float* hk = (float*)(ws + p->a_hk);
    RC(hct_gather_rows(h_in, (const int32_t*)(ws + p->a_kept_rows), Nc, d * 4, hk, s));
    RC(dec0_table(p->pf(p->p_mask), p->pf(p->p_dpos), p->L, d, hk + (size_t)Nc * d, s));
    RC(norm_fwd(p, hk, p->pf(bp.ln1_w), p->pf(bp.ln1_b), Rc, d, 1e-5f, ws + p->a_x1c, p->dt, (float*)(ws + p->a_mean_c), (float*)(ws + p->a_rstd_c), s));
    RC(linear_fwd(p, ws + p->a_x1c, Rc, d, bp.qkv_w, bp.qkv_b, 3 * d, ws + p->a_qkv_cat, p->dt, HCT_ACT_NONE, nullptr, nullptr, s));
    RC(hct_gather_rows(ws + p->a_qkv_cat, (const int32_t*)(ws + p->a_cat_idx), M, (int)(3 * d * p->esz()), ws + ba.qkv, s));
  } else {
    RC(norm_fwd(p, h_in, p->pf(bp.ln1_w), p->pf(bp.ln1_b), M, d, 1e-5f, ws + ba.x1, p->dt, (float*)(ws + ba.mean1), (float*)(ws + ba.rstd1), s));
    RC(linear_fwd(p, ws + ba.x1, M, d, bp.qkv_w, bp.qkv_b, 3 * d, ws + ba.qkv, p->dt, HCT_ACT_NONE, nullptr, nullptr, s));
    if (bp.lq_a >= 0) RC(lora_forward(p, bp, ba, B, N, d, heads, s));
  }
  if (p->drop.fwd)
    RC(hct_attention_dropout_fwd(ws + ba.qkv, B, N, heads, d / heads, p->dt, p->drop_p, p->drop_seed, bp.site, ws + ba.o, (float*)(ws + ba.lse), s));
  else
    RC(hct_attention_fwd(ws + ba.qkv, B, N, heads, d / heads, p->dt, ws + ba.o, (float*)(ws + ba.lse), s));
  if (rows != Rows::kTail) return back_half_forward(p, bp, ba, M, ws + ba.o, h_in, h_out, d, sd.m, s);
  const int32_t* tail_rows = (const int32_t*)(ws + p->a_tail_rows);
  float* hin_c = (float*)(ws + p->s_dh);
  RC(hct_gather_rows(ws + ba.o, tail_rows, p->Mc, (int)(d * p->esz()), ws + p->a_oc, s));
  RC(hct_gather_rows(h_in, tail_rows, p->Mc, d * 4, hin_c, s));
  return back_half_forward(p, bp, ba, p->Mc, ws + p->a_oc, hin_c, h_out, d, sd.m, s);
}

int back_half_backward(hct_mae_plan* p, const BlockP& bp, const BlockA& ba, const BlockG& bg, int M, const void* o, float* dh, void* d_o, int d, int m,
                       hipStream_t s) {
  unsigned char* ws = p->ws;
  const void* dhs = ws + bg.out;
  void* dhs_mid = ws + bg.mid;
  void* dbig = ws + bg.big;
  void* dx = ws + p->s_dx;
  const bool masked = p->masks_residual(bp);
  if (masked) {
    RC(branch_apply(p, bp, 1, dh, HCT_F32, ws + bg.dm_out, p->dt, nullptr, M, d, s));
    dhs = ws + bg.dm_out;
    if (p->tr(bp.fc2_b) >= 0) RC(hct_colsum(dhs, p->dt, M, d, d, p->gf(bp.fc2_b), ws + p->s_small2, p->s_small2_bytes, s));
  }
  RC(linear_wgrad(p, dhs, ws + ba.g, M, d, m, p->tr(bp.fc2_w), -1, s));
  RC(linear_dgrad(p, dhs, M, d, bp.fc2_w, m, dbig, kActFc2Dgrad, ws + ba.u, s, p->gf(bp.fc1_b)));
  RC(linear_wgrad(p, dbig, ws + ba.x2, M, m, d, p->tr(bp.fc1_w), -1, s));
  RC(linear_dgrad(p, dbig, M, m, bp.fc1_w, d, dx, HCT_ACT_NONE, nullptr, s));
  RC(norm_bwd(p, dx, p->dt, (const float*)(ws + ba.h_mid), (const float*)(ws + ba.mean2), (const float*)(ws + ba.rstd2), p->pf(bp.ln2_w), dh, nullptr,
              M, d, dh, dhs_mid, p->dt, p->gf(bp.ln2_w), p->gf(bp.ln2_b), masked ? nullptr : p->gf(bp.proj_b), ws + p->s_fold_a, p->s_fold_bytes, s));
  if (masked) {
    RC(branch_apply(p, bp, 0, dh, HCT_F32, ws + bg.dm_mid, p->dt, nullptr, M, d, s));
    dhs_mid = ws + bg.dm_mid;
    if (p->tr(bp.proj_b) >= 0) RC(hct_colsum(dhs_mid, p->dt, M, d, d, p->gf(bp.proj_b), ws + p->s_small2, p->s_small2_bytes, s));
  }
  RC(linear_wgrad(p, dhs_mid, o, M, d, d, p->tr(bp.proj_w), -1, s));
  return linear_dgrad(p, dhs_mid, M, d, bp.proj_w, d, d_o, HCT_ACT_NONE, nullptr, s);
}

int block_backward(hct_mae_plan* p, const Side& sd, int i, Rows rows, hipStream_t s) {
  const BlockP& bp = sd.bp[i];
  const BlockA& ba = sd.ba[i];
  const BlockG& bg = sd.ring[i % sd.ring.size()];
  const int B = p->B, N = sd.N, d = sd.d, heads = sd.heads, M = B * N;
  const bool tail = rows == Rows::kTail, drop = p->drop.fwd;
  unsigned char* ws = p->ws;
  float* dh = (float*)(ws + p->s_dh);
  void* dx = ws + p->s_dx;
  void* d_o = ws + p->s_do;
  void* dqkv = ws + bg.qkv;
  FoldSink sink;
  SinkScope scope(p->defer_folds ? &sink : g_fold_sink);
  if (tail) {
    const int32_t* inv = (const int32_t*)(ws + p->a_tail_inv);
    RC(back_half_backward(p, bp, ba, bg, p->Mc, ws + p->a_oc, (float*)(ws + p->s_dhc), dx, d, sd.m, s));
    RC(hct_gather_rows(dx, inv, M, (int)(d * p->esz()), d_o, s));
  } else {
    RC(back_half_backward(p, bp, ba, bg, M, ws + ba.o, dh, d_o, d, sd.m, s));
  }
  if (drop)
    RC(hct_attention_dropout_bwd(ws + ba.qkv, ws + ba.o, d_o, (const float*)(ws + ba.lse), B, N, heads, d / heads, p->dt, p->drop_p, p->drop_seed,
                                 bp.site, dqkv, s));
  else
    RC(hct_attention_bwd(ws + ba.qkv, ws + ba.o, d_o, (const float*)(ws + ba.lse), B, N, heads, d / heads, p->dt, dqkv, s));
  if (rows == Rows::kCat) {
    const int Rc = p->Rcat;
    const int32_t* kept = (const int32_t*)(ws + p->a_kept_rows);
    if (p->tr(bp.qkv_b) >= 0) RC(hct_colsum(dqkv, p->dt, M, 3 * d, 3 * d, p->gf(bp.qkv_b), ws + p->s_small2, p->s_small2_bytes, s));
    RC(dec0_aggregate(dqkv, p->dt, kept, (const int32_t*)(ws + p->a_ids_restore), B, p->L, p->K, 3 * d, ws + p->a_dqkv_cat, s));
    RC(linear_wgrad(p, ws + p->a_dqkv_cat, ws + p->a_x1c, Rc, 3 * d, d, p->tr(bp.qkv_w), -1, s));
    RC(linear_dgrad(p, ws + p->a_dqkv_cat, Rc, 3 * d, bp.qkv_w, d, dx, HCT_ACT_NONE, nullptr, s));
    RC(norm_bwd(p, dx, p->dt, (const float*)(ws + p->a_hk), (const float*)(ws + p->a_mean_c), (const float*)(ws + p->a_rstd_c), p->pf(bp.ln1_w), dh, kept,
                Rc, d, (float*)(ws + p->a_dcat), ws + p->a_de, p->dt, p->gf(bp.ln1_w), p->gf(bp.ln1_b), nullptr, ws + p->s_fold_b, p->s_fold_bytes, s));
  } else {
    RC(linear_wgrad(p, dqkv, ws + ba.x1, M, 3 * d, d, p->tr(bp.qkv_w), p->tr(bp.qkv_b), s));
    RC(linear_dgrad(p, dqkv, M, 3 * d, bp.qkv_w, d, dx, HCT_ACT_NONE, nullptr, s));
    if (bp.lq_a >= 0) RC(lora_backward(p, bp, ba, bg, dqkv, dx, B, N, d, heads, s));
    const float* dres = tail ? (const float*)(ws + p->s_dhc) : dh;
    const int32_t* dres_rows = tail ? (const int32_t*)(ws + p->a_tail_inv) : nullptr;
    float* prev_fc2_b = i > 0 && !p->masks_residual(sd.bp[i - 1]) ? p->gf(sd.bp[i - 1].fc2_b) : nullptr;
    RC(norm_bwd(p, dx, p->dt, (const float*)(ws + sd.h[i]), (const float*)(ws + ba.mean1), (const float*)(ws + ba.rstd1), p->pf(bp.ln1_w), dres, dres_rows,
                M, d, dh, ws + p->out_grad(sd, i - 1), p->dt, p->gf(bp.ln1_w), p->gf(bp.ln1_b), prev_fc2_b, ws + p->s_fold_b, p->s_fold_bytes, s));
  }
  return fold_flush(sink, s);
}

int encoder_forward(hct_mae_plan* p, float eps, hipStream_t s) {
  unsigned char* ws = p->ws;
  const int ne = p->cfg.encoder_depth;
  const Side enc = p->enc_side();
  if (p->drop.fwd) RC(drop_embedding(p, (float*)(ws + p->h_enc[0]), s));
  for (int i = 0; i < ne; ++i) RC(block_forward(p, enc, i, Rows::kEvery, s));
  return norm_fwd(p, (const float*)(ws + p->h_enc[ne]), p->pf(p->p_norm_w), p->pf(p->p_norm_b), p->Me, p->D, eps, ws + p->a_latent, p->dt,
                  (float*)(ws + p->a_lat_mean), (float*)(ws + p->a_lat_rstd), s);
}

int encoder_norm_backward(hct_mae_plan* p, const void* dlatent, hipStream_t s) {
  unsigned char* ws = p->ws;
  const int ne = p->cfg.encoder_depth;
  const Side enc = p->enc_side();
  return norm_bwd(p, dlatent, p->dt, (const float*)(ws + p->h_enc[ne]), (const float*)(ws + p->a_lat_mean), (const float*)(ws + p->a_lat_rstd),
                  p->pf(p->p_norm_w), nullptr, nullptr, p->Me, p->D, (float*)(ws + p->s_dh), ws + p->out_grad(enc, ne - 1), p->dt, p->gf(p->p_norm_w),
                  p->gf(p->p_norm_b), ne > 0 && !p->masks_residual(p->enc[ne - 1]) ? p->gf(p->enc[ne - 1].fc2_b) : nullptr, ws + p->s_small, p->s_small_bytes, s);
}

int encoder_block_stage(hct_mae_plan* p, int stage, int i, hipStream_t s) {
  const Side enc = p->enc_side();
  RC(block_backward(p, enc, i, Rows::kEvery, s));
  return end_stage(p, stage, true, false, (int)enc.ring.size(), p->cfg.encoder_depth, s);
}

void read_env(hct_mae_plan* p) {
  auto off = [](const char* name) { const char* v = getenv(name); return v && v[0] == '0'; };
  p->defer_folds = !off("HCT_DEFER_FOLDS");
  p->dec0.on = p->dec0.can && !off("HCT_DEC0_TABLE");
  p->wg_defer = p->dt == HCT_BF16 && !off("HCT_WGRAD_DEFER");
  const char* eb = getenv("HCT_WGRAD_GROUP_BLOCKS");
  p->wg_blocks = eb && *eb ? std::max(0, atoi(eb)) : 0;
}

int vit_arm_modes(hct_mae_plan* p, hipStream_t s) {
  p->drop.fwd = p->drop.can && p->drop.on;
  p->path.fwd = p->path.can && p->path.on;
  if (p->path.fwd) {
    std::vector<int> sites;
    std::vector<float> rates;
    for (const BlockP& bp : p->enc)
      for (int branch = 0; branch < 2; ++branch) { sites.push_back(bp.site + 1 + 2 * branch); rates.push_back(bp.path_q); }
    RC(hct_drop_path_scales(p->drop_seed, sites.data(), rates.data(), (int)sites.size(), p->B, (float*)(p->ws + p->s_path), s));
  }
  return 0;
}

}

extern "C" {

hct_mae_plan* hct_mae_plan_create(const hct_mae_config* c, int batch, int compute_dtype) {
  if (!c || batch <= 0 || (compute_dtype != HCT_F32 && compute_dtype != HCT_BF16)) { set_error("hct_mae_plan_create: bad arguments"); return nullptr; }
  if (c->patch_size <= 0 || c->input_size % c->patch_size || c->patch_size % 4) { set_error("hct_mae_plan_create: input_size %% patch_size != 0 or patch_size %% 4 != 0"); return nullptr; }
  const bool enc_only = c->encoder_only != 0;
  if (c->encoder_embed_dim % c->encoder_num_heads || (!enc_only && c->decoder_embed_dim % c->decoder_num_heads)) { set_error("hidden size should be divisible by num_heads"); return nullptr; }
  if (c->encoder_embed_dim % 4 || c->encoder_mlp_dim % 4 || (!enc_only && (c->decoder_embed_dim % 4 || c->decoder_mlp_dim % 4))) { set_error("embed/mlp dims must be multiples of 4"); return nullptr; }
  if (c->lora_rank != 0 && !enc_only) { set_error("hct_mae_plan_create: lora_rank is for encoder-only (plain ViT) plans; the MAE plan has no adapters"); return nullptr; }
  if (c->lora_rank < 0 || c->lora_rank % 32) { set_error("hct_mae_plan_create: lora_rank must be 0 or a positive multiple of 32 (%d)", c->lora_rank); return nullptr; }
  if (c->norm_kind != 0 && c->norm_kind != 1) { set_error("hct_mae_plan_create: norm_kind must be 0 (LayerNorm) or 1 (RMSNorm), got %d", c->norm_kind); return nullptr; }
  if (!(c->dropout_rate >= 0.f) || !(c->dropout_rate < 1.f)) { set_error("hct_mae_plan_create: dropout_rate must satisfy 0 <= p < 1 (p = 1 drops everything), got %g", (double)c->dropout_rate); return nullptr; }
  if (!(c->drop_path_rate >= 0.f) || !(c->drop_path_rate < 1.f)) { set_error("hct_mae_plan_create: drop_path_rate must satisfy 0 <= r < 1 (r = 1 drops every sample in the last block), got %g", (double)c->drop_path_rate); return nullptr; }
  if (c->drop_path_rate > 0.f && !enc_only) { set_error("hct_mae_plan_create: drop_path_rate is for encoder-only (plain ViT) plans; the MAE plan has no stochastic depth"); return nullptr; }
  if (!(c->patch_dropout >= 0.0) || !(c->patch_dropout < 1.0)) { set_error("hct_mae_plan_create: patch_dropout must satisfy 0 <= r < 1 (r = 1 drops every patch), got %g", c->patch_dropout); return nullptr; }
  if (c->patch_dropout > 0.0 && !enc_only) { set_error("hct_mae_plan_create: patch_dropout is for encoder-only (plain ViT) plans; the MAE plan masks by mask_ratio"); return nullptr; }
  hct_mae_plan* p = new hct_mae_plan();
  p->cfg = *c;
  p->drop_p = c->dropout_rate;
  p->lora = c->lora_rank;
  p->norm_kind = c->norm_kind;
  p->B = batch; p->dt = compute_dtype;
  p->g = c->input_size / c->patch_size;
  p->L = p->g * p->g * p->g;
  p->vit = c->encoder_only != 0;
  p->R = p->vit ? c->num_register_tokens : 0;
  p->norm_eps = (p->vit && c->final_norm_eps > 0.f) ? c->final_norm_eps : 1e-5f;
  if (p->R < 0) { set_error("num_register_tokens < 0"); delete p; return nullptr; }
  p->K = (int)((double)p->L * (1.0 - c->mask_ratio));
  p->keep = p->vit && c->patch_dropout > 0.0;
  if (p->vit) p->K = p->keep ? (int)((double)p->L * (1.0 - c->patch_dropout)) : p->L;
  p->pd = c->in_chans * c->patch_size * c->patch_size * c->patch_size;
  p->Ne = p->K + 1 + p->R; p->Nd = p->vit ? 0 : p->L + 1;
  p->Me = batch * p->Ne; p->Md = batch * p->Nd;
  if (p->vit) p->cfg.decoder_depth = 0;
  p->D = c->encoder_embed_dim; p->Dd = p->vit ? c->encoder_embed_dim : c->decoder_embed_dim;
  p->Mlp = c->encoder_mlp_dim; p->Mlpd = p->vit ? c->encoder_mlp_dim : c->decoder_mlp_dim;
  p->H = c->encoder_num_heads; p->Hd = p->vit ? c->encoder_num_heads : c->decoder_num_heads;
  if (p->K < 1) { set_error(p->keep ? "hct_mae_plan_create: patch_dropout leaves no patch (K = int(L * (1 - r)) < 1)" : "mask_ratio leaves no visible patches"); delete p; return nullptr; }
  const bool ub = c->use_bias != 0;
  const int P = c->patch_size, C = c->in_chans;
  std::vector<std::pair<int64_t, int64_t>> seg;
  int64_t g0 = p->param_elems;
  p->p_pe_w = add_param(p, "patch_embedding.patch_embeddings.weight", {p->D, C, P, P, P}, true, true, false);
  p->p_pe_b = add_param(p, "patch_embedding.patch_embeddings.bias", {p->D}, true, false, false);
  p->p_pos = c->pos_embed ? add_param(p, "patch_embedding.position_embeddings", {1, p->L, p->D}, true, false, false) : -1;
  p->p_cls = add_param(p, "cls_token", {1, 1, p->D}, true, false, false);
  if (p->R > 0) p->p_reg = add_param(p, "register_tokens", {1, p->R, p->D}, true, false, false);
  seg.push_back({g0, p->param_elems});
  for (int i = 0; i < c->encoder_depth; ++i) {
    g0 = p->param_elems;
    p->enc.push_back(add_block(p, "blocks." + std::to_string(i), p->D, p->Mlp, ub));
    seg.push_back({g0, p->param_elems});
  }
  g0 = p->param_elems;
  p->p_norm_w = add_param(p, "norm.weight", {p->D}, true, false, false);
  p->p_norm_b = p->norm_kind == 1 ? -1 : add_param(p, "norm.bias", {p->D}, true, false, false);
  if (p->vit) {
    seg.push_back({g0, p->param_elems});
    p->p_de_w = p->p_de_b = p->p_mask = p->p_dcls = p->p_dpos = p->p_dnorm_w = p->p_dnorm_b = p->p_pred_w = p->p_pred_b = -1;
  } else {
  p->p_de_w = add_param(p, "decoder_embed.weight", {p->Dd, p->D}, true, true, true);
  p->p_de_b = ub ? add_param(p, "decoder_embed.bias", {p->Dd}, true, false, false) : -1;
  p->p_mask = add_param(p, "mask_token", {1, 1, p->Dd}, true, false, false);
  p->p_dcls = add_param(p, "decoder_cls_token", {1, 1, p->Dd}, true, false, false);
  p->p_dpos = add_param(p, "decoder_pos_embed", {1, p->L, p->Dd}, false, false, false);
  seg.push_back({g0, p->param_elems});
  for (int i = 0; i < p->cfg.decoder_depth; ++i) {
    g0 = p->param_elems;
    p->dec.push_back(add_block(p, "decoder_blocks." + std::to_string(i), p->Dd, p->Mlpd, ub));
    seg.push_back({g0, p->param_elems});
  }
  g0 = p->param_elems;
  p->p_dnorm_w = add_param(p, "decoder_norm.weight", {p->Dd}, true, false, false);
  p->p_dnorm_b = p->norm_kind == 1 ? -1 : add_param(p, "decoder_norm.bias", {p->Dd}, true, false, false);
  p->p_pred_w = add_param(p, "decoder_pred.weight", {p->pd, p->Dd}, true, true, true);
  p->p_pred_b = ub ? add_param(p, "decoder_pred.bias", {p->pd}, true, false, false) : -1;
  seg.push_back({g0, p->param_elems});
  }
  for (size_t i = 0; i < p->enc.size(); ++i) p->enc[i].site = 1 + 4 * (int)i;
  for (size_t i = 0; i < p->dec.size(); ++i) p->dec[i].site = 1 + 4 * (int)(p->enc.size() + i);
  for (size_t i = 0; i < p->enc.size(); ++i) {
    p->enc[i].path_q = p->enc.size() > 1 ? (float)((double)c->drop_path_rate * (double)i / (double)(p->enc.size() - 1)) : 0.f;
    p->enc[i].path_row = 2 * (int)i;
    if (p->enc[i].path_q > 0.f) p->path.can = true;
  }
  for (int i = (int)seg.size() - 1; i >= 0; --i) p->stage_range.push_back(seg[i]);

  const size_t es = p->esz();
  p->Mc = p->vit ? 0 : batch * (p->L - p->K);
  p->Rcat = p->vit ? 0 : p->Me + p->L;
  p->drop.can = p->drop_p > 0.f;
  p->tail.can = !p->vit && p->cfg.decoder_depth >= 1 && p->Mc > 0 && (p->Dd * es) % 16 == 0;
  p->dec0.can = !p->vit && p->cfg.decoder_depth >= 2 && (p->Dd * es) % 16 == 0 && (3 * p->Dd * es) % 16 == 0;
  read_env(p);

  WsAlloc w;
  const size_t B = batch, L = p->L, K = p->K, Me = p->Me, Md = p->Md, D = p->D, Dd = p->Dd;
  p->a_ids_restore = w.take(B * L * 4);
  p->a_ids_shuffle = w.take(B * L * 4);
  p->a_mask = w.take(B * L * 4);
  p->a_row_loss = w.take(B * L * 4);
  p->a_patches = w.take(B * K * p->pd * es);
  p->a_tok = w.take(B * K * D * es);
  for (int i = 0; i <= c->encoder_depth; ++i) p->h_enc.push_back(w.take(Me * D * 4));
  for (int i = 0; i < c->encoder_depth; ++i) {
    p->aenc.push_back(alloc_block(w, Me, D, p->Mlp, (size_t)batch * p->H * p->Ne, es));
    if (p->lora > 0) p->aenc.back().lora_t = w.take(Me * 2 * (size_t)p->lora * es);
  }
  p->a_latent = w.take(Me * D * es);
  p->a_lat_mean = w.take(Me * 4);
  p->a_lat_rstd = w.take(Me * 4);
  p->a_e = w.take(Me * Dd * es);
  for (int i = 0; i <= p->cfg.decoder_depth; ++i) p->h_dec.push_back(w.take(Md * Dd * 4));
  for (int i = 0; i < p->cfg.decoder_depth; ++i) p->adec.push_back(alloc_block(w, Md, Dd, p->Mlpd, (size_t)batch * p->Hd * p->Nd, es));
  p->a_ynorm = w.take(Md * Dd * es);
  p->a_yn_mean = w.take(Md * 4);
  p->a_yn_rstd = w.take(Md * 4);
  p->a_pred = w.take(Md * p->pd * es);
  p->a_dpred = w.take(Md * p->pd * es);
  p->a_tail_rows = w.take((size_t)p->Mc * 4);
  p->a_tail_inv = w.take(Md * 4);
  p->a_oc = w.take((size_t)p->Mc * Dd * es);
  p->s_dhc = w.take((size_t)p->Mc * Dd * 4);
  const size_t Mx = Md > Me ? Md : Me, Dx = Dd > D ? Dd : D;
  const size_t mlpx = (size_t)(p->Mlp > p->Mlpd ? p->Mlp : p->Mlpd);
  p->s_dh = w.take(Mx * Dx * 4);
  p->s_dh_shadow = w.take(Mx * Dx * es);
  p->s_dx = w.take(Mx * Dx * es);
  p->s_do = w.take(Mx * Dx * es);
  auto alloc_ring = [&](std::vector<BlockG>& ring, int depth, size_t M, size_t d, size_t m) {
    const size_t lora_cols = p->lora > 0 ? 2 * d + 2 * (size_t)p->lora : 0;
    const bool masked = p->drop_p > 0.f || c->drop_path_rate > 0.f;
    const size_t drop_cols = masked ? 2 * d : 0;
    const size_t set_bytes = M * (5 * d + m + lora_cols + drop_cols) * es, budget = (size_t)32 << 30;
    int nsets = depth;
    if (depth > 0 && set_bytes * (size_t)depth > budget) nsets = std::max(2, (int)(budget / set_bytes));
    nsets = std::min(nsets, depth);
    for (int i = 0; i < nsets; ++i) {
      BlockG g;
      g.out = w.take(M * d * es);
      g.big = w.take(M * m * es);
      g.mid = w.take(M * d * es);
      g.qkv = w.take(M * 3 * d * es);
      if (p->lora > 0) {
        g.lora_du = w.take(M * 2 * d * es);
        g.lora_dt = w.take(M * 2 * (size_t)p->lora * es);
      }
      if (masked) {
        g.dm_out = w.take(M * d * es);
        g.dm_mid = w.take(M * d * es);
      }
      ring.push_back(g);
    }
  };
  alloc_ring(p->genc, c->encoder_depth, Me, D, (size_t)p->Mlp);
  alloc_ring(p->gdec, p->cfg.decoder_depth, Md, Dd, (size_t)p->Mlpd);
  {
    const size_t Rc = (size_t)p->Rcat;
    p->a_kept_rows = w.take(Rc * 4);
    p->a_cat_idx = w.take(Md * 4);
    p->a_hk = w.take(Rc * Dd * 4);
    p->a_x1c = w.take(Rc * Dd * es);
    p->a_mean_c = w.take(Rc * 4);
    p->a_rstd_c = w.take(Rc * 4);
    p->a_qkv_cat = w.take(Rc * 3 * Dd * es);
    p->a_dqkv_cat = w.take(Rc * 3 * Dd * es);
    p->a_dcat = w.take(Rc * Dd * 4);
  }
  p->a_de = w.take((Me + L) * Dd * es);
  p->a_dtok = w.take(B * K * D * es);
  size_t small = hct_layernorm_bwd_workspace_bytes((int)Mx, (int)Dx);
  small = std::max(small, hct_assemble_bwd_workspace_bytes((int)Dx));
  small = std::max(small, hct_colsum_workspace_bytes((int)Mx, (int)(3 * Dx)));
  small = std::max(small, hct_colsum_workspace_bytes((int)Mx, (int)mlpx));
  small = std::max(small, hct_colsum_workspace_bytes((int)Md, p->pd));
  small = std::max(small, (size_t)((Mx + 255) / 256) * 4 * mlpx * sizeof(float));
// ... 1 lines not shown
  p->s_fold_bytes = hct_layernorm_bwd_workspace_bytes((int)Mx, (int)Dx);
  p->s_fold_a = w.take(p->s_fold_bytes);
  p->s_fold_b = w.take(p->s_fold_bytes);
  p->s_small2_bytes = small;
  p->s_small2 = w.take(p->s_small2_bytes);
  p->s_small_bytes = small;
  p->s_small = w.take(small);
  if (p->dt == HCT_BF16) {
    p->s_nt_bytes = hct_gemm_nt_stream_k_bytes();
    w.take(p->s_nt_bytes);
  }
  size_t gw = 0;
  for (int side = 0; side < 2; ++side) {
    const int M = side ? p->Md : p->Me, d = side ? p->Dd : p->D, m = side ? p->Mlpd : p->Mlp;
    gw = std::max(gw, wgrad_ws(p->dt, M, d, m));
    gw = std::max(gw, wgrad_ws(p->dt, M, m, d));
    gw = std::max(gw, wgrad_ws(p->dt, M, d, d));
    gw = std::max(gw, wgrad_ws(p->dt, M, 3 * d, d));
  }
  gw = std::max(gw, wgrad_ws(p->dt, p->Md, p->pd, p->Dd));
  gw = std::max(gw, wgrad_ws(p->dt, p->Me, p->Dd, p->D));
  gw = std::max(gw, wgrad_ws(p->dt, batch * p->K, p->D, p->pd));
  if (p->lora > 0) {
    gw = std::max(gw, strided_wgrad_ws(p->dt, p->Me, p->D, 2 * p->D, p->lora, 2 * p->lora));
    gw = std::max(gw, strided_wgrad_ws(p->dt, p->Me, p->lora, 2 * p->lora, p->D, p->D));
  }
  p->s_gemm_bytes = gw;
  p->s_gemm = w.take(gw);
  {
    p->s_wg_bytes = hct_gemm_tn_group_workspace_bytes((p->lora > 0 ? 8 : 4) * (c->encoder_depth + p->cfg.decoder_depth) + 4);
    for (int i = 0; i < kWgSlots; ++i) p->s_wg[i] = p->wg_defer ? w.take(p->s_wg_bytes) : 0;
  }
  if (p->drop_p > 0.f || c->drop_path_rate > 0.f) {
    p->s_drop_y = w.take(Mx * Dx * es);
    p->s_path = w.take(2 * p->enc.size() * B * sizeof(float));
  }
  p->final_off = p->param_elems;
  p->ws_bytes = w.cur;

  auto reg = [&](const std::string& n, size_t off, int64_t r, int64_t cc, int dtp) { p->acts[n] = Act{off, r, cc, dtp}; };
  reg("ids_restore", p->a_ids_restore, batch, p->L, 2);
  reg("ids_shuffle", p->a_ids_shuffle, batch, p->L, 2);
  reg("mask", p->a_mask, batch, p->L, HCT_F32);
  reg("patches", p->a_patches, (int64_t)batch * p->K, p->pd, p->dt);
  reg("tok", p->a_tok, (int64_t)batch * p->K, p->D, p->dt);
  reg("enc_in", p->h_enc[0], p->Me, p->D, HCT_F32);
  for (int i = 0; i < c->encoder_depth; ++i) reg("enc" + std::to_string(i) + ".out", p->h_enc[i + 1], p->Me, p->D, HCT_F32);
  reg("latent", p->a_latent, p->Me, p->D, p->dt);
  reg("dec_in", p->h_dec[0], p->Md, p->Dd, HCT_F32);
  for (int i = 0; i < p->cfg.decoder_depth; ++i) reg("dec" + std::to_string(i) + ".out", p->h_dec[i + 1], p->Md, p->Dd, HCT_F32);
  reg("tail_rows", p->a_tail_rows, 1, p->Mc, 2);
  reg("pred_full", p->a_pred, p->Md, p->pd, p->dt);
  reg("dpred_full", p->a_dpred, p->Md, p->pd, p->dt);
  if (c->encoder_depth > 0) {
    reg("enc0.qkv", p->aenc[0].qkv, p->Me, 3 * p->D, p->dt);
    reg("enc0.attn_o", p->aenc[0].o, p->Me, p->D, p->dt);
    if (p->lora > 0) reg("enc0.lora_t", p->aenc[0].lora_t, p->Me, 2 * p->lora, p->dt);
  }
  return p;
}

void hct_mae_plan_destroy(hct_mae_plan* p) { delete p; }
int hct_mae_plan_num_params(const hct_mae_plan* p) { return (int)p->params.size(); }
int hct_mae_plan_param_info(const hct_mae_plan* p, int index, hct_param_info* out) {
  HCT_REQUIRE(p && out && index >= 0 && index < (int)p->params.size(), "hct_mae_plan_param_info: bad index");
  *out = p->params[index];
  return 0;
}
int64_t hct_mae_plan_param_elems(const hct_mae_plan* p) { return p->param_elems; }
int64_t hct_mae_plan_bf16_t_elems(const hct_mae_plan* p) { return p->bf16t_elems; }
size_t hct_mae_plan_workspace_bytes(const hct_mae_plan* p) { return p->ws_bytes; }
int hct_mae_plan_len_keep(const hct_mae_plan* p) { return p ? p->K : -1; }
int hct_mae_plan_set_requires_grad(hct_mae_plan* p, int index, int flag) {
  HCT_REQUIRE(p && index >= 0 && index < (int)p->params.size(), "hct_mae_plan_set_requires_grad: bad index");
  if (p->params[index].requires_grad != (flag ? 1 : 0)) p->t_all_done = false;
  p->params[index].requires_grad = flag ? 1 : 0;
  return 0;
}
int hct_mae_plan_set_dec0(hct_mae_plan* p, int on) {
  if (!p) return -1;
  p->dec0.on = on != 0 && p->dec0.can;
  return p->dec0.on ? 1 : 0;
}
int hct_mae_plan_set_dropout(hct_mae_plan* p, int active, uint64_t seed) {
  if (!p) return -1;
  p->drop.on = active != 0 && p->drop.can;
  p->path.on = active != 0 && p->path.can;
  p->drop_seed = seed;
  return p->drop.on || p->path.on ? 1 : 0;
}
int hct_mae_plan_set_tail(hct_mae_plan* p, int compact) {
  if (!p) return -1;
  p->tail.on = compact != 0 && p->tail.can;
  return p->tail.on ? 1 : 0;
}

int hct_mae_plan_bind(hct_mae_plan* p, float* params, float* grads, void* params_bf16, void* params_bf16_t, void* workspace,
                      size_t workspace_bytes) {
  HCT_REQUIRE(p && params && workspace, "hct_mae_plan_bind: null buffer");
  HCT_REQUIRE(p->dt == HCT_F32 || (params_bf16 && params_bf16_t), "hct_mae_plan_bind: bf16 mode needs the bf16 weight buffers");
  if (workspace_bytes < p->ws_bytes) { set_error("hct_mae_plan_bind: workspace too small"); return HCT_E_WORKSPACE; }
  p->params_f32 = params; p->grads = grads;
  p->params_bf16 = (bf16*)params_bf16; p->params_bf16_t = (bf16*)params_bf16_t;
  p->ws = (unsigned char*)workspace;
  p->nt_ws_armed = false;
  p->t_all_done = false;
  p->fwd_done = false;
  for (auto& v : p->wg_prepared) v.clear();
  p->wg_pending.clear();
  return 0;
}

int hct_mae_refresh_weights(hct_mae_plan* p, int with_plain, void* stream) {
  HCT_REQUIRE(p && p->params_f32, "hct_mae_refresh_weights: plan not bound");
  if (p->dt != HCT_BF16) return 0;
  if (with_plain) RC(hct_cast(p->params_f32, HCT_F32, p->params_bf16, HCT_BF16, p->param_elems, stream));
  TransposeTable t;
  t.n = 0;
  t.tile_start[0] = 0;
  auto flush = [&]() -> int {
    if (t.n == 0) return 0;
    hipLaunchKernelGGL(transpose_cast_batched_kernel, dim3(t.tile_start[t.n]), dim3(256), 0, (hipStream_t)stream, p->params_f32,
                       p->params_bf16_t, t);
    t.n = 0;
    return check_hip(hipGetLastError(), "hct_mae_refresh_weights");
  };
  for (const auto& pi : p->params) {
    if (pi.bf16_t_offset < 0) continue;
    if (!with_plain && p->t_all_done && !pi.requires_grad) continue;
    const int rows = (int)pi.shape[0], cols = (int)(pi.numel / pi.shape[0]);
    t.rows[t.n] = rows; t.cols[t.n] = cols; t.src[t.n] = pi.offset; t.dst[t.n] = pi.bf16_t_offset;
    t.tile_start[t.n + 1] = t.tile_start[t.n] + ((rows + 63) / 64) * ((cols + 63) / 64);
    if (++t.n == kMaxT) RC(flush());
  }
  RC(flush());
  p->t_all_done = true;
  return 0;
}

int hct_mae_forward(hct_mae_plan* p, const void* x, int x_dtype, const float* noise, float* loss, float grad_scale, void* stream) {
  HCT_REQUIRE(p && p->ws && x && noise && loss, "hct_mae_forward: plan not bound or null argument");
  HCT_REQUIRE(!p->vit, "hct_mae_forward: encoder-only plans are driven by hct_vit_forward");
  HCT_REQUIRE(x_dtype == HCT_F32 || x_dtype == HCT_F16, "hct_mae_forward: volumes are fp32 or fp16");
  hipStream_t s = (hipStream_t)stream;
  unsigned char* ws = p->ws;
  const hct_mae_config& c = p->cfg;
  const int B = p->B;
  p->drop.fwd = p->drop.can && p->drop.on;
  p->path.fwd = false;
  p->tail.fwd = p->tail.can && p->tail.on && !p->drop.fwd;
  p->dec0.fwd = p->dec0.can && p->dec0.on && !p->drop.fwd;
  const bool tail = p->tail.fwd, dec0 = p->dec0.fwd;
  int32_t* ids_restore = (int32_t*)(ws + p->a_ids_restore);
  int32_t* ids_shuffle = (int32_t*)(ws + p->a_ids_shuffle);
  float* mask = (float*)(ws + p->a_mask);
  RC(hct_mask_rank(noise, B, p->L, p->K, ids_restore, ids_shuffle, mask, s));
  RC(hct_patch_gather(x, x_dtype, ids_shuffle, B, c.in_chans, c.input_size, c.patch_size, p->L, p->K, ws + p->a_patches, p->dt, s));
  RC(linear_fwd(p, ws + p->a_patches, B * p->K, p->pd, p->p_pe_w, p->p_pe_b, p->D, ws + p->a_tok, p->dt, HCT_ACT_NONE, nullptr, nullptr, s));
  RC(hct_encoder_assemble_fwd(ws + p->a_tok, p->dt, p->pf(p->p_cls), p->pf(p->p_pos), ids_shuffle, B, p->L, p->K, p->D, (float*)(ws + p->h_enc[0]), s));
  RC(encoder_forward(p, 1e-5f, s));
  RC(linear_fwd(p, ws + p->a_latent, p->Me, p->D, p->p_de_w, p->p_de_b, p->Dd, ws + p->a_e, p->dt, HCT_ACT_NONE, nullptr, nullptr, s));
  RC(hct_decoder_assemble_fwd(ws + p->a_e, p->dt, p->pf(p->p_mask), p->pf(p->p_dcls), p->pf(p->p_dpos), ids_restore, B, p->L, p->K, p->Dd,
                              (float*)(ws + p->h_dec[0]), s));
  if (tail) RC(hct_tail_rows(ids_restore, B, p->L, p->K, (int32_t*)(ws + p->a_tail_rows), (int32_t*)(ws + p->a_tail_inv), s));
  if (dec0) RC(dec0_index(ids_restore, B, p->L, p->K, (int32_t*)(ws + p->a_kept_rows), (int32_t*)(ws + p->a_cat_idx), s));
  const Side dec = p->dec_side();
  for (int i = 0; i < c.decoder_depth; ++i) RC(block_forward(p, dec, i, p->decoder_rows(i), s));
  const int Mt = tail ? p->Mc : p->Md;
  RC(norm_fwd(p, (const float*)(ws + p->h_dec[c.decoder_depth]), p->pf(p->p_dnorm_w), p->pf(p->p_dnorm_b), Mt, p->Dd, 1e-5f,
                       ws + p->a_ynorm, p->dt, (float*)(ws + p->a_yn_mean), (float*)(ws + p->a_yn_rstd), s));
  RC(linear_fwd(p, ws + p->a_ynorm, Mt, p->Dd, p->p_pred_w, p->p_pred_b, p->pd, ws + p->a_pred, p->dt, HCT_ACT_NONE, nullptr, nullptr, s));
  const bool train = grad_scale != 0.0f;
  RC(masked_mse_launch(ws + p->a_pred, p->dt, x, x_dtype, mask, B, c.in_chans, c.input_size, c.patch_size, c.norm_pix_loss,
                       (float)((int64_t)B * (p->L - p->K)), (float*)(ws + p->a_row_loss), loss, train ? ws + p->a_dpred : nullptr, nullptr,
                       train ? grad_scale : 1.0f, s, tail ? ids_shuffle : nullptr, p->K));
  p->fwd_done = true;
  p->dpred_done = train;
  return 0;
}

int hct_vit_forward(hct_mae_plan* p, const void* x, int x_dtype, void* stream) {
  HCT_REQUIRE(x, "hct_vit_forward: null argument");
  return hct_vit_forward_parts(p, &x, 1, x_dtype, stream);
}

int hct_vit_forward_parts(hct_mae_plan* p, const void* const* xs, int n_parts, int x_dtype, void* stream) {
  HCT_REQUIRE(p && p->ws && xs && n_parts > 0, "hct_vit_forward: plan not bound or null argument");
  HCT_REQUIRE(p->vit, "hct_vit_forward: the plan was not created with encoder_only = 1");
  HCT_REQUIRE(x_dtype == HCT_F32 || x_dtype == HCT_F16, "hct_vit_forward: volumes are fp32 or fp16");
  HCT_REQUIRE(p->B % n_parts == 0, "hct_vit_forward_parts: the plan's batch (%d) is not a multiple of the number of parts (%d)", p->B, n_parts);
  HCT_REQUIRE(!p->keep, "hct_vit_forward: the plan was created with patch_dropout > 0 and is driven by hct_vit_forward_parts_keep");
  hipStream_t s = (hipStream_t)stream;
  unsigned char* ws = p->ws;
  const hct_mae_config& c = p->cfg;
  const int B = p->B, Bp = B / n_parts;
  RC(vit_arm_modes(p, s));
  for (int i = 0; i < n_parts; ++i) {
    HCT_REQUIRE(xs[i], "hct_vit_forward_parts: null part %d", i);
    RC(hct_patch_gather(xs[i], x_dtype, nullptr, Bp, c.in_chans, c.input_size, c.patch_size, p->L, p->L,
                        ws + p->a_patches + (size_t)i * Bp * p->L * p->pd * p->esz(), p->dt, s));
  }
  RC(linear_fwd(p, ws + p->a_patches, B * p->L, p->pd, p->p_pe_w, p->p_pe_b, p->D, ws + p->a_tok, p->dt, HCT_ACT_NONE, nullptr, nullptr, s));
  RC(hct_vit_assemble_fwd(ws + p->a_tok, p->dt, p->pf(p->p_cls), p->p_reg >= 0 ? p->pf(p->p_reg) : nullptr, p->p_pos >= 0 ? p->pf(p->p_pos) : nullptr, B,
                          p->L, p->R, p->D, (float*)(ws + p->h_enc[0]), s));
  RC(encoder_forward(p, p->norm_eps, s));
  p->fwd_done = true;
  return 0;
}

int hct_vit_forward_parts_keep(hct_mae_plan* p, const void* const* xs, int n_parts, int x_dtype, const float* noise, void* stream) {
  HCT_REQUIRE(p && p->ws && xs && noise && n_parts > 0, "hct_vit_forward_parts_keep: plan not bound or null argument");
  HCT_REQUIRE(p->vit, "hct_vit_forward_parts_keep: the plan was not created with encoder_only = 1");
  HCT_REQUIRE(p->keep, "hct_vit_forward_parts_keep: the plan was created without patch_dropout and is driven by hct_vit_forward / hct_vit_forward_parts");
  HCT_REQUIRE(x_dtype == HCT_F32 || x_dtype == HCT_F16, "hct_vit_forward_parts_keep: volumes are fp32 or fp16");
  HCT_REQUIRE(p->B % n_parts == 0, "hct_vit_forward_parts_keep: the plan's batch (%d) is not a multiple of the number of parts (%d)", p->B, n_parts);
  hipStream_t s = (hipStream_t)stream;
  unsigned char* ws = p->ws;
  const hct_mae_config& c = p->cfg;
  const int B = p->B, Bp = B / n_parts;
  RC(vit_arm_modes(p, s));
  int32_t* ids_restore = (int32_t*)(ws + p->a_ids_restore);
  int32_t* ids_shuffle = (int32_t*)(ws + p->a_ids_shuffle);
  RC(hct_mask_rank(noise, B, p->L, p->K, ids_restore, ids_shuffle, (float*)(ws + p->a_mask), s));
  for (int i = 0; i < n_parts; ++i) {
    HCT_REQUIRE(xs[i], "hct_vit_forward_parts_keep: null part %d", i);
    RC(hct_patch_gather(xs[i], x_dtype, ids_shuffle + (size_t)i * Bp * p->L, Bp, c.in_chans, c.input_size, c.patch_size, p->L, p->K,
                        ws + p->a_patches + (size_t)i * Bp * p->K * p->pd * p->esz(), p->dt, s));
  }
  RC(linear_fwd(p, ws + p->a_patches, B * p->K, p->pd, p->p_pe_w, p->p_pe_b, p->D, ws + p->a_tok, p->dt, HCT_ACT_NONE, nullptr, nullptr, s));
  RC(hct_vit_assemble_keep_fwd(ws + p->a_tok, p->dt, p->pf(p->p_cls), p->p_reg >= 0 ? p->pf(p->p_reg) : nullptr,
                               p->p_pos >= 0 ? p->pf(p->p_pos) : nullptr, ids_shuffle, B, p->L, p->K, p->R, p->D, (float*)(ws + p->h_enc[0]), s));
  RC(encoder_forward(p, p->norm_eps, s));
  p->fwd_done = true;
  return 0;
// ... 122 lines not shown
```

headct_foundation_amd/mae.py:

```python
from __future__ import annotations

from typing import Optional

import numpy as np
import torch
import torch.nn as nn

from . import _lib
from ._lib import HCT_BF16, HCT_F32, HctError
from .flat import FlatPlanModule
from .layers import POS_CODES, _Affine, _Holder, _block, _norm, _to_3tuple, build_sincos_position_embedding, init_linear_, norm_kind


class _MAEFunction(torch.autograd.Function):

    @staticmethod
    def forward(ctx, anchor, model, x, noise, train):
        plan = model._plan_for(x.shape[0])
        st = _lib.stream_ptr()
        model._sync_frozen(plan)
        model._ensure_weights_fresh(plan, st)
        dropping = model._arm_dropout(plan)
        plan.tail = bool(plan.lib.hct_mae_plan_set_tail(plan.handle, int(train and not dropping and not getattr(model, "full_pred", False))) == 1)
        if not getattr(model, "dec0_table", True):
            plan.lib.hct_mae_plan_set_dec0(plan.handle, 0)
        _lib.check(plan.lib.hct_mae_forward(plan.handle, x.data_ptr(), _lib.dtype_code(x), noise.data_ptr(), plan.loss.data_ptr(),
                                            float(model._grad_prescale) if train else 0.0, st), "hct_mae_forward")
        plan.serial += 1
        ctx.model, ctx.plan, ctx.x, ctx.serial = model, plan, x, plan.serial
        return plan.loss[0].clone()

    @staticmethod
    def backward(ctx, grad_out):
        model, plan, x = ctx.model, ctx.plan, ctx.x
        if plan.serial != ctx.serial:
            raise HctError("backward of a stale forward: another forward at the same batch size has overwritten the activation "
                           "workspace (run loss.backward() before the next model(...) call, e.g. before an eval pass)")
        model._run_backward(plan, x, grad_out)
        return None, None, None, None, None


class MaskedAutoencoderViT(FlatPlanModule):

    def __init__(self, input_size: int, patch_size: int, mask_ratio: float, in_chans: int = 1, dropout_rate: float = 0.,
                 spatial_dims: int = 3, patch_embed: str = 'conv', pos_embed: str = 'learnable', encoder_depth: int = 12,
                 encoder_embed_dim: int = 768, encoder_mlp_dim: int = 3072, encoder_num_heads: int = 12,
                 decoder_depth: int = 8, decoder_embed_dim: int = 768, decoder_mlp_dim: int = 3072,
                 decoder_num_heads: int = 16, norm_pix_loss: bool = False, use_bias: bool = False,
                 norm_layer=nn.LayerNorm, compute_dtype: str = "bf16"):
        super().__init__()
        input_size, patch_size = _to_3tuple(input_size), _to_3tuple(patch_size)
        if spatial_dims != 3 or len(set(input_size)) != 1 or len(set(patch_size)) != 1:
            raise HctError("the HIP MAE path supports cubic 3-D volumes and patches")
        if patch_embed != "conv":
            raise ValueError(f"patch_embed type {patch_embed} not supported.")
        if pos_embed not in POS_CODES:
            raise ValueError(f"pos_embed type {pos_embed} not supported.")
        if not (0 <= dropout_rate <= 1):
            raise ValueError("dropout_rate should be between 0 and 1.")
        if dropout_rate == 1:
            raise ValueError("dropout_rate 1 drops every value and has no finite scale 1 / (1 - p): the HIP path takes 0 <= dropout_rate < 1")
        self.norm_kind = norm_kind(norm_layer, "MaskedAutoencoderViT")
        if encoder_embed_dim % encoder_num_heads or decoder_embed_dim % decoder_num_heads:
            raise ValueError("hidden_size should be divisible by num_heads.")
        for m, p in zip(input_size, patch_size):
            if m < p:
                raise ValueError("patch_size should be smaller than img_size.")
            assert m % p == 0, "input size and patch size are not proper"
        if compute_dtype not in ("bf16", "fp32"):
            raise ValueError("compute_dtype must be 'bf16' or 'fp32'")

        self.input_size, self.patch_size = input_size, patch_size
        self.mask_ratio, self.spatial_dims, self.pos_embed, self.norm_pix_loss = mask_ratio, spatial_dims, pos_embed, norm_pix_loss
        self.encoder_embed_dim, self.decoder_embed_dim = encoder_embed_dim, decoder_embed_dim
        self.in_chans = in_chans
        self.out_chans = in_chans * int(np.prod(patch_size))
        self.grid_size = [i // p for i, p in zip(input_size, patch_size)]
        self.compute_dtype = compute_dtype
        num_patches = int(np.prod(self.grid_size))
        self.num_patches = num_patches
        D, Dd, P = encoder_embed_dim, decoder_embed_dim, patch_size[0]

        self.cls_token = nn.Parameter(torch.zeros(1, 1, D))
        self.decoder_cls_token = nn.Parameter(torch.zeros(1, 1, Dd))
        self.decoder_pos_embed = nn.Parameter(torch.zeros(1, num_patches, Dd), requires_grad=False)
        self.patch_embedding = _Holder()
        self.patch_embedding.n_patches = num_patches
        if pos_embed != "none":
            self.patch_embedding.position_embeddings = nn.Parameter(torch.zeros(1, num_patches, D))
        else:
            self.patch_embedding.position_embeddings = None
        self.patch_embedding.patch_embeddings = _Affine(D, in_chans, P, P, P, bias_shape=(D,))
        self.blocks = nn.ModuleList([_block(D, encoder_mlp_dim, use_bias, norm_layer=norm_layer) for _ in range(encoder_depth)])
        self.decoder_blocks = nn.ModuleList([_block(Dd, decoder_mlp_dim, use_bias, norm_layer=norm_layer) for _ in range(decoder_depth)])
        self.norm = _norm(D, norm_layer)
        self.decoder_norm = _norm(Dd, norm_layer)
        self.decoder_embed = _Affine(Dd, D, bias_shape=(Dd,) if use_bias else None)
        self.decoder_pred = _Affine(P ** 3 * in_chans, Dd, bias_shape=(P ** 3 * in_chans,) if use_bias else None)
        self.mask_token = nn.Parameter(torch.zeros(1, 1, Dd))

        self._ccfg = _lib.MaeConfig(
            input_size=input_size[0], patch_size=P, in_chans=in_chans, mask_ratio=float(mask_ratio), pos_embed=POS_CODES[pos_embed],
            encoder_depth=encoder_depth, encoder_embed_dim=D, encoder_mlp_dim=encoder_mlp_dim, encoder_num_heads=encoder_num_heads,
            decoder_depth=decoder_depth, decoder_embed_dim=Dd, decoder_mlp_dim=decoder_mlp_dim, decoder_num_heads=decoder_num_heads,
            norm_pix_loss=int(bool(norm_pix_loss)), use_bias=int(bool(use_bias)), norm_kind=self.norm_kind, dropout_rate=float(dropout_rate))
        self._dt = HCT_BF16 if compute_dtype == "bf16" else HCT_F32
        self.len_keep = int(num_patches * (1 - mask_ratio))
        self.full_pred = False
# ... 100 lines not shown
```

include/headct_hip.h:

```cpp
#ifndef HEADCT_HIP_H
#define HEADCT_HIP_H

#include <stddef.h>
#include <stdint.h>

#ifdef __cplusplus
extern "C" {
#endif

#define HCT_F32 0
#define HCT_BF16 1
#define HCT_F16 2

#define HCT_E_BADARG (-1)
#define HCT_E_UNSUPPORTED (-2)
#define HCT_E_WORKSPACE (-3)
#define HCT_E_STATE (-4)

#define HCT_ACT_NONE 0
#define HCT_ACT_GELU 1
#define HCT_ACT_DGELU 2
#define HCT_ACT_TANH 3
#define HCT_ACT_GELU_D 4
#define HCT_ACT_MULAUX 5
// ... 10 lines not shown
  const float* bias;
  const float* residual;
  int64_t ldr;
  int act;
  void* aux; int aux_dtype; int64_t ldaux;
  void* C2; int c2_dtype; int64_t ldc2;
  float alpha;
  int force_generic;
  float* colsum_out;
  int workspace_armed;
} hct_gemm_args;

size_t hct_gemm_workspace_bytes(const hct_gemm_args* a);
size_t hct_gemm_nt_flags_offset(size_t workspace_bytes);
size_t hct_gemm_nt_stream_k_bytes(void);
void hct_set_cu_reserve(int n);
int hct_gemm(const hct_gemm_args* a, void* workspace, size_t workspace_bytes, void* stream);
#define HCT_GEMM_GENERIC 0
#define HCT_GEMM_NT128 1
#define HCT_GEMM_NT256 2
#define HCT_GEMM_TN128 3
#define HCT_GEMM_TN256 4
typedef struct hct_gemm_plan_info {
  int kernel;
  int epilogue_mode;
  int fuse_colsum;
  int row_tiles_per_wave;
  int tiles, grid;
  int sk_tiles, sk_wgs;
  int splits, r_chunk;
  size_t colsum_bytes;
  size_t stream_k_offset;
  size_t slab_bytes;
  size_t workspace_bytes;
  int walk_width;
} hct_gemm_plan_info;
int hct_gemm_describe(const hct_gemm_args* a, int num_cus, size_t workspace_bytes, hct_gemm_plan_info* out);
int hct_gemm_stream_k_items(int grid, int sk_tiles, int sk_wgs, int pairs, uint32_t* first, uint32_t* owner);
int hct_gemm_nt_walk(int tiles, int n_col_tiles, int sk_tiles, int walk_width, int* ids);
size_t hct_gemm_tn_group_workspace_bytes(int n_jobs);
int hct_gemm_tn_group_prepare(const hct_gemm_args* jobs, int n_jobs, void* workspace, size_t workspace_bytes, void* stream);
int hct_gemm_tn_group_run(const hct_gemm_args* jobs, int n_jobs, void* workspace, size_t workspace_bytes, void* stream);

int hct_mask_rank(const float* noise, int B, int L, int K, int32_t* ids_restore, int32_t* ids_shuffle,
                  float* mask, void* stream);

int hct_patch_gather(const void* x, int x_dtype , const int32_t* ids_shuffle, int B, int C, int S, int P, int L, int K,
                     void* rows, int rows_dtype, void* stream);

int hct_encoder_assemble_fwd(const void* tok, int tok_dtype, const float* cls, const float* pos,
                             const int32_t* ids_shuffle, int B, int L, int K, int D, float* h0, void* stream);
int hct_encoder_assemble_bwd(const float* dh0, const int32_t* ids_restore, int B, int L, int K, int D,
                             void* dtok, int dtok_dtype, float* dcls, float* dpos, void* workspace,
                             size_t workspace_bytes, void* stream);
size_t hct_assemble_bwd_workspace_bytes(int D);

int hct_layernorm_fwd(const float* x, const float* gamma, const float* beta, int rows, int D, float eps,
                      void* y, int y_dtype, float* mean, float* rstd, void* stream);
size_t hct_layernorm_bwd_workspace_bytes(int rows, int D);
int hct_layernorm_bwd(const void* dy, int dy_dtype, const float* x, const float* mean, const float* rstd,
                      const float* gamma, const float* dres, int rows, int D, float* dx, void* dx_shadow,
                      int shadow_dtype, float* dgamma, float* dbeta, float* dcolsum, void* workspace,
                      size_t workspace_bytes, void* stream);
int hct_layernorm_bwd_mapped(const void* dy, int dy_dtype, const float* x, const float* mean, const float* rstd,
                             const float* gamma, const float* dres, const int32_t* dres_rows, int rows, int D, float* dx,
                             void* dx_shadow, int shadow_dtype, float* dgamma, float* dbeta, float* dcolsum, void* workspace,
                             size_t workspace_bytes, void* stream);
int hct_rmsnorm_fwd(const float* x, const float* gamma, int rows, int D, float eps, void* y, int y_dtype, float* rstd,
                    void* stream);
size_t hct_rmsnorm_bwd_workspace_bytes(int rows, int D);
int hct_rmsnorm_bwd(const void* dy, int dy_dtype, const float* x, const float* rstd, const float* gamma, const float* dres,
                    int rows, int D, float* dx, void* dx_shadow, int shadow_dtype, float* dgamma, float* dcolsum,
                    void* workspace, size_t workspace_bytes, void* stream);
int hct_rmsnorm_bwd_mapped(const void* dy, int dy_dtype, const float* x, const float* rstd, const float* gamma,
                           const float* dres, const int32_t* dres_rows, int rows, int D, float* dx, void* dx_shadow,
                           int shadow_dtype, float* dgamma, float* dcolsum, void* workspace, size_t workspace_bytes,
                           void* stream);
int hct_tail_rows(const int32_t* ids_restore, int B, int L, int K, int32_t* tail_rows, int32_t* tail_inv, void* stream);
int hct_gather_rows(const void* src, const int32_t* idx, int n_rows, int row_bytes, void* dst, void* stream);

int hct_attention_fwd(const void* qkv, int B, int N, int H, int dh, int dtype, void* o, float* lse, void* stream);
int hct_attention_bwd(const void* qkv, const void* o, const void* d_o, const float* lse, int B, int N, int H,
                      int dh, int dtype, void* dqkv, void* stream);

int hct_dropout_mask(uint64_t seed, int site, int kind, int64_t n, int BH, int N, float p, unsigned char* out, void* stream);
int hct_dropout_apply(const void* x, int x_dtype, void* y, int y_dtype, const float* residual, const void* x2, void* y2,
                      int64_t batches, int64_t stride, int64_t off, int64_t seg, uint64_t seed, int site, float p, void* stream);
int hct_attention_dropout_fwd(const void* qkv, int B, int N, int H, int dh, int dtype, float p, uint64_t seed, int site, void* o,
                              float* lse, void* stream);
int hct_attention_dropout_bwd(const void* qkv, const void* o, const void* d_o, const float* lse, int B, int N, int H, int dh,
                              int dtype, float p, uint64_t seed, int site, void* dqkv, void* stream);
int hct_drop_path_scales(uint64_t seed, const int* sites, const float* rates, int n_sites, int B, float* out, void* stream);
int hct_residual_drop_apply(const void* x, int x_dtype, void* y, int y_dtype, const float* residual, int64_t B, int64_t seg,
                            const float* scales, uint64_t seed, int site, float p, void* stream);

int hct_decoder_assemble_fwd(const void* e, int e_dtype, const float* mask_token, const float* dec_cls,
                             const float* dec_pos, const int32_t* ids_restore, int B, int L, int K, int D,
                             float* y, void* stream);
int hct_decoder_assemble_bwd(const float* dy, const int32_t* ids_restore, const int32_t* ids_shuffle, int B,
                             int L, int K, int D, void* de, int de_dtype, float* dmask_token, float* ddec_cls,
                             void* workspace, size_t workspace_bytes, void* stream);

int hct_masked_mse(const void* pred, int pred_dtype, const void* x, int x_dtype , const float* mask, int B, int C, int S,
                   int P, int norm_pix, float mask_sum, float* row_loss, float* loss, void* dpred,
                   const float* dpred_scale, void* stream);
int hct_unpatchify(const void* pred, int pred_dtype, int has_cls_row, int B, int C, int S, int P, float* vol,
                   void* stream);

int hct_vit_assemble_fwd(const void* tok, int tok_dtype, const float* cls, const float* reg, const float* pos, int B,
                         int L, int R, int D, float* h, void* stream);

int hct_channel_norm(const float* x, const float* mean, const float* var, float eps, void* out, int out_dtype, int64_t rows,
                     int C, void* stream);
int hct_query_attention(const float* q, int Q, const void* kv, int kv_dtype, int B, int N, int H, int dh, float logit_scale,
                        float* out, void* stream);
int hct_head_linear(const float* x, int64_t ldx, int nq, const float* mean, const float* var, float eps, const float* W,
                    const float* bias, int act, float* out, int rows, int D, int n_out, void* stream);

int hct_batchnorm_stats(const float* x, int B, int D, float momentum, float* mean, float* var, float* running_mean,
                        float* running_var, void* stream);
int hct_softmax_xent(const float* logits, const int64_t* target, int B, int n_classes, const float* dloss, float* loss,
                     float* dlogits, void* stream);
int hct_head_linear_wgrad(const float* x, const float* mean, const float* var, float eps, const float* dlogits, int B, int D,
                          int n_out, float* dW, float* db, void* stream);

size_t hct_sigmoid_bce_workspace_bytes(int B, int T);
int hct_sigmoid_bce(const float* logits, const float* target, const float* pos_weight, int B, int T, const float* dloss, float* loss,
                    float* label_loss, float* dlogits, void* workspace, size_t workspace_bytes, void* stream);

int hct_mix_volumes(float* x, int B, int C, int S, const float* lam, const int32_t* box, void* stream);
int hct_mix_xent(const float* logits, const int64_t* target, const float* lam, float smoothing, int B, int n_classes, const float* dloss,
                 float* loss, float* dlogits, void* stream);

size_t hct_bn_rows_workspace_bytes(int rows, int D);
int hct_bn_stats_rows(const void* x, int x_dtype, int64_t ldx, int rows, int D, float momentum, float* mean, float* var,
                      float* running_mean, float* running_var, void* workspace, size_t workspace_bytes, void* stream);
int hct_bn_norm(const void* x, int x_dtype, int64_t ldx, int64_t rows, int D, const float* mean, const float* var, float eps,
                void* out, int out_dtype, void* stream);
int hct_bn_bwd_input(const void* x, int x_dtype, int64_t ldx, const float* mean, const float* var, float eps, const float* g,
                     int64_t ldg, const float* dlogits, const float* W, int nq, int n_classes, int rows, int D, void* dx,
                     int dx_dtype, int64_t ldo, void* workspace, size_t workspace_bytes, void* stream);
int hct_head_linear_x(const void* x, int x_dtype, int64_t ldx, int nq, const float* mean, const float* var, float eps,
                      const float* W, const float* bias, float* out, int rows, int D, int n_out, void* stream);
int hct_head_linear_bwd(const void* x, int x_dtype, int64_t ldx, int nq, const float* mean, const float* var, float eps,
                        const float* dlogits, int B, int D, int n_out, float* dW, float* db, void* stream);
int hct_query_attention_lse(const float* q, int Q, const void* kv, int kv_dtype, int B, int N, int H, int dh, float logit_scale,
                            float* out, float* lse, void* stream);
size_t hct_query_attention_bwd_workspace_bytes(int B, int Q, int H, int dh);
int hct_query_attention_bwd(const float* q, int Q, const void* kv, int kv_dtype, int B, int N, int H, int dh, float logit_scale,
                            const float* out, const float* lse, const float* dout, void* dkv, float* dq, void* workspace,
                            size_t workspace_bytes, void* stream);
int hct_clip_total_norm(float* grads, int64_t total, const float* norms, int nseg, float max_norm, float* nrm, void* stream);
int hct_add_f32(float* dst, const float* src, int64_t n, void* stream);

size_t hct_dino_loss_workspace_bytes(int n_crops, int B, int K);
int hct_dino_loss(const void* student, const void* teacher, int dtype, int n_crops, int B, int K, const float* center, float student_temp,
                  float teacher_temp, float* loss, void* dstudent, const float* dloss, float* batch_center_sum, void* workspace,
                  size_t workspace_bytes, void* stream);
int hct_dino_center_update(float* center, const float* batch_center_sum, int K, double momentum, double count, void* stream);
int hct_ema_update(float* momentum_params, const float* params, int64_t n, double m, void* stream);
size_t hct_dino_sk_workspace_bytes(int R, int K);
int hct_dino_sk_col_lse(const void* teacher, int dtype, int R, int K, float inv_temp, const float* lr, float* out, void* workspace,
                        size_t workspace_bytes, void* stream);
int hct_dino_sk_row_lse(const void* teacher, int dtype, int R, int K, float inv_temp, const float* lc, float* out, void* stream);
size_t hct_dino_loss_sk_workspace_bytes(int n_crops, int B, int K);
int hct_dino_loss_sk(const void* student, const void* teacher, int dtype, int n_crops, int B, int K, const float* lc, const float* lr, float log_n,
// ... 43 lines not shown
int hct_crop_window_resize_area(const float* vol, int m0, int m1, int m2, const int32_t* box, int n_windows, const float* a_min, const float* a_max,
                                void* out, int R0, int R1, int R2, void* stream);

int hct_pos_embed_interp3d(const float* src, int g_src, float* dst, int g_dst, int D, int extra, void* stream);

size_t hct_colsum_workspace_bytes(int rows, int cols);
int hct_colsum(const void* x, int dtype, int rows, int cols, int64_t ld, float* out, void* workspace,
               size_t workspace_bytes, void* stream);

int hct_cast(const void* src, int src_dtype, void* dst, int dst_dtype, int64_t n, void* stream);
int hct_transpose_cast(const void* src, int src_dtype, void* dst, int dst_dtype, int rows, int cols, void* stream);

size_t hct_grad_norms_workspace_bytes(int64_t total);
int hct_grad_norms(float* grads, const int64_t* seg_off, int nseg, int64_t total, float clip, int scale_in_place,
                   float* norms, float* coef, void* workspace, size_t workspace_bytes, void* stream);
int hct_adamw_step(float* params, float* grads, float* exp_avg, float* exp_avg_sq, const int64_t* seg_off,
                   const float* coef, const uint8_t* skip, int nseg, int64_t total, float lr, float beta1,
                   float beta2, float eps, float weight_decay, int step, void* params_bf16, void* stream);
int hct_lion_step(float* params, float* grads, float* exp_avg, const int64_t* seg_off, const float* coef,
                  const uint8_t* skip, int nseg, int64_t total, double lr, double beta1, double beta2, double weight_decay,
                  void* params_bf16, void* stream);
int hct_sgd_step(float* params, float* grads, float* momentum_buf, const int64_t* seg_off, const float* coef,
                 const uint8_t* skip, int nseg, int64_t total, double lr, double momentum, void* params_bf16, void* stream);
size_t hct_lamb_workspace_bytes(int64_t total, int nseg);
int hct_lamb_step(float* params, float* grads, float* exp_avg, float* exp_avg_sq, const int64_t* seg_off, const float* coef,
                  const uint8_t* skip, int nseg, int64_t total, double lr, double beta1, double beta2, double eps,
                  double weight_decay, float* weight_norm, float* adam_norm, float* trust_ratio, void* workspace,
                  size_t workspace_bytes, void* params_bf16, void* stream);

int hct_adamw_step_scaled(float* params, float* grads, float* exp_avg, float* exp_avg_sq, const int64_t* seg_off,
                          const float* coef, const uint8_t* skip, int nseg, int64_t total, float lr, float beta1,
                          float beta2, float eps, float weight_decay, int step, void* params_bf16, const float* lr_scale,
                          const float* wd_scale, void* stream);
int hct_lion_step_scaled(float* params, float* grads, float* exp_avg, const int64_t* seg_off, const float* coef,
                         const uint8_t* skip, int nseg, int64_t total, double lr, double beta1, double beta2, double weight_decay,
                         void* params_bf16, const float* lr_scale, const float* wd_scale, void* stream);
int hct_sgd_step_scaled(float* params, float* grads, float* momentum_buf, const int64_t* seg_off, const float* coef,
                        const uint8_t* skip, int nseg, int64_t total, double lr, double momentum, void* params_bf16,
                        const float* lr_scale, void* stream);
int hct_lamb_step_scaled(float* params, float* grads, float* exp_avg, float* exp_avg_sq, const int64_t* seg_off, const float* coef,
                         const uint8_t* skip, int nseg, int64_t total, double lr, double beta1, double beta2, double eps,
                         double weight_decay, float* weight_norm, float* adam_norm, float* trust_ratio, void* workspace,
                         size_t workspace_bytes, void* params_bf16, const float* lr_scale, const float* wd_scale, void* stream);

typedef struct hct_mae_config {
  int input_size, patch_size, in_chans;
  double mask_ratio;
  int pos_embed;
  int encoder_depth, encoder_embed_dim, encoder_mlp_dim, encoder_num_heads;
  int decoder_depth, decoder_embed_dim, decoder_mlp_dim, decoder_num_heads;
  int norm_pix_loss, use_bias;
  int encoder_only, num_register_tokens;
  float final_norm_eps;
  int lora_rank;
  int norm_kind;
  float dropout_rate;
  float drop_path_rate;
  double patch_dropout;
} hct_mae_config;

typedef struct hct_mae_plan hct_mae_plan;

typedef struct hct_param_info {
  char name[96];
  int ndim;
  int64_t shape[5];
  int64_t offset;
  int64_t numel;
  int requires_grad;
  int is_matrix;
  int64_t bf16_t_offset;
} hct_param_info;

hct_mae_plan* hct_mae_plan_create(const hct_mae_config* cfg, int batch, int compute_dtype);
void hct_mae_plan_destroy(hct_mae_plan*);
int hct_mae_plan_num_params(const hct_mae_plan*);
int hct_mae_plan_param_info(const hct_mae_plan*, int index, hct_param_info* out);
int64_t hct_mae_plan_param_elems(const hct_mae_plan*);
int64_t hct_mae_plan_bf16_t_elems(const hct_mae_plan*);
size_t hct_mae_plan_workspace_bytes(const hct_mae_plan*);
int hct_mae_plan_len_keep(const hct_mae_plan*);
int hct_mae_plan_set_tail(hct_mae_plan*, int compact);
int hct_mae_plan_set_dec0(hct_mae_plan*, int on);
int hct_mae_plan_set_dropout(hct_mae_plan*, int active, uint64_t seed);
int hct_mae_plan_bind(hct_mae_plan*, float* params, float* grads, void* params_bf16, void* params_bf16_t,
                      void* workspace, size_t workspace_bytes);
int hct_mae_refresh_weights(hct_mae_plan*, int with_plain, void* stream);
int hct_mae_forward(hct_mae_plan*, const void* x, int x_dtype, const float* noise, float* loss, float grad_scale, void* stream);
int hct_mae_set_loss_grad(hct_mae_plan*, const float* dloss);
int hct_mae_num_backward_stages(const hct_mae_plan*);
int hct_mae_backward_stage_range(const hct_mae_plan*, int stage, int64_t* begin, int64_t* end);
int hct_mae_backward_stage(hct_mae_plan*, int stage, void* stream);
int64_t hct_mae_backward_final_offset(const hct_mae_plan*);
int hct_mae_plan_set_wgrad_defer(hct_mae_plan*, int defer, int group_blocks);
int hct_mae_plan_set_requires_grad(hct_mae_plan*, int index, int flag);
int hct_vit_forward(hct_mae_plan*, const void* x, int x_dtype, void* stream);
int hct_vit_forward_parts(hct_mae_plan*, const void* const* xs, int n_parts, int x_dtype, void* stream);
int hct_vit_backward_stage(hct_mae_plan*, int stage, const void* dlatent, void* stream);
int hct_vit_assemble_bwd(const float* dh0, int B, int L, int R, int D, void* dtok, int dtok_dtype, float* dcls, float* dreg, float* dpos,
                         void* stream);
int hct_vit_assemble_keep_fwd(const void* tok, int tok_dtype, const float* cls, const float* reg, const float* pos,
                              const int32_t* ids_shuffle, int B, int L, int K, int R, int D, float* h0, void* stream);
int hct_vit_assemble_keep_bwd(const float* dh0, const int32_t* ids_restore, int B, int L, int K, int R, int D, void* dtok, int dtok_dtype,
                              float* dcls, float* dreg, float* dpos, void* stream);
int hct_vit_forward_parts_keep(hct_mae_plan*, const void* const* xs, int n_parts, int x_dtype, const float* noise, void* stream);
int hct_lora_qv_fwd(const void* x1, const void* Aq, const void* Av, const void* Bq, const void* Bv, int B, int N, int H, int dh, int r, int dtype,
                    void* T, void* qkv, void* stream);
size_t hct_lora_qv_bwd_workspace_bytes(int M, int D, int r, int dtype);
int hct_lora_qv_bwd(const void* dqkv, const void* x1, const void* T, const void* Aq, const void* Av, const void* Bq, const void* Bv,
                    const void* AqT, const void* AvT, const void* BqT, const void* BvT, int B, int N, int H, int dh, int r, int dtype, float* dAq,
                    float* dAv, float* dBq, float* dBv, void* dx1, void* workspace, size_t workspace_bytes, void* stream);
int hct_topk_dot_chunks(int Q, int64_t G);
size_t hct_topk_dot_workspace(int Q, int64_t G, int k);
int hct_topk_dot(const void* q, int Q, const void* g, int64_t G, int D, int dtype, const int32_t* exclude, int k, float* scores, int32_t* idx,
                 void* workspace, size_t workspace_bytes, void* stream);
int hct_attention_row_probs(const void* qkv, int B, int N, int H, int dh, int dtype, const int32_t* rows, int n_rows, float* probs, void* stream);
int hct_mae_recon_accum(const void* pred, int pred_dtype, int has_cls_row, const void* x, int x_dtype , const float* mask,
                        int B, int C, int S, int P, int norm_pix, float* recon_sum, float* err_sum, int32_t* cnt, void* stream);
int hct_mae_recon_finish(const float* recon_sum, const float* err_sum, const int32_t* cnt, const void* x, int x_dtype, int B, int C, int S, int P,
                         float* recon, float* err, float* err_vol, void* stream);
const void* hct_mae_plan_activation(const hct_mae_plan*, const char* name, int64_t* rows, int64_t* cols, int* dtype);

void hct_prof_enable(int mask);
void hct_prof_reset(void);
int hct_prof_read(int id, double* total_ms, int64_t* launches, double* work);
int hct_prof_read_bytes(int id, double* bytes);
typedef struct hct_prof_shape {
  int M, N, K, mode, tiles, sk_tiles;
  int64_t launches;
  double total_ms, work, bytes;
} hct_prof_shape;
int hct_prof_shapes(int id, hct_prof_shape* out, int cap);
void hct_debug_force_simple_attention(int mode);
void hct_debug_set_gemm_variant(int v);

#ifdef __cplusplus
}
#endif
#endif
```

Baseline: 7120 CT-volumes/s.

## Add row-mapped attention kernels to skip decoder gather/scatter copies

Adds mapped variants of the MFMA attention forward and backward kernels that read qkv and dO through row index maps and can write a compacted output directly. The MAE decoder uses them to drop separate gather_rows passes around attention for the tail-compaction and concatenated paths. The weight refresh also now transposes from the already-cast bf16 weights instead of re-reading fp32. The cost is extra index loads and per-row offsets in the kernels, plus more template instances and register pressure.

```diff
diff --git a/headct_foundation_amd/_lib.py b/headct_foundation_amd/_lib.py
--- a/headct_foundation_amd/_lib.py
+++ b/headct_foundation_amd/_lib.py
@@ -103,6 +103,13 @@
     "hct_gather_rows": (c_int, [c_void_p, c_void_p, c_int, c_int, c_void_p, c_void_p]),
     "hct_attention_fwd": (c_int, [c_void_p, c_int, c_int, c_int, c_int, c_int, c_void_p, c_void_p, c_void_p]),
     "hct_attention_bwd": (c_int, [c_void_p, c_void_p, c_void_p, c_void_p, c_int, c_int, c_int, c_int, c_int, c_void_p, c_void_p]),
+    "hct_attention_maps_supported": (c_int, [c_int, c_int, c_int, c_int, c_int]),
+    "hct_attention_fwd_mapped": (c_int, [c_void_p, c_void_p, c_int, c_int, c_int, c_int, c_int, c_int, c_void_p, c_void_p, c_void_p, c_void_p,
+                                         c_void_p]),
+    "hct_attention_bwd_mapped": (c_int, [c_void_p, c_void_p, c_int, c_void_p, c_void_p, c_void_p, c_int, c_void_p, c_int, c_int, c_int, c_int,
+                                         c_int, c_void_p, c_void_p]),
+    "hct_weight_transpose": (c_int, [c_void_p, c_int, c_int, c_int, c_void_p, c_void_p]),
+    "hct_mae_plan_set_row_maps": (c_int, [c_void_p, c_int]),
     "hct_debug_force_simple_attention": (None, [c_int]),
     "hct_dropout_mask": (c_int, [C.c_uint64, c_int, c_int, c_int64, c_int, c_int, c_float, c_void_p, c_void_p]),
     "hct_dropout_apply": (c_int, [c_void_p, c_int, c_void_p, c_int, c_void_p, c_void_p, c_void_p, c_int64, c_int64, c_int64, c_int64, C.c_uint64,
diff --git a/headct_foundation_amd/csrc/attention.hip b/headct_foundation_amd/csrc/attention.hip
--- a/headct_foundation_amd/csrc/attention.hip
+++ b/headct_foundation_amd/csrc/attention.hip
@@ -16,6 +16,11 @@
 int attention_dropout_fwd_mfma(const void* qkv, int B, int N, int H, int dh, void* o, float* lse, const DropArgs& da, hipStream_t s);
 int attention_dropout_bwd_mfma(const void* qkv, const void* o, const void* d_o, const float* lse, int B, int N, int H, int dh, void* dqkv,
                                const DropArgs& da, hipStream_t s);
+bool attention_maps_supported(int N, int H, int dh);
+int attention_fwd_mapped_mfma(const void* qkv, const int32_t* qkv_rows, int qkv_src_rows, int B, int N, int H, void* o, float* lse,
+                              void* o_compact, const int32_t* o_rows, hipStream_t s);
+int attention_bwd_mapped_mfma(const void* qkv, const int32_t* qkv_rows, int qkv_src_rows, const void* o, const void* d_o,
+                              const int32_t* do_rows, int do_src_rows, const float* lse, int B, int N, int H, void* dqkv, hipStream_t s);
 int check_drop_rate(const char* who, float p);
 int g_force_simple_attention = 0;
 extern int g_attn_general;
@@ -30,21 +35,57 @@
   g_attn_general = mode == 2;
 }
 
-int hct_attention_fwd(const void* qkv, int B, int N, int H, int dh, int dtype, void* o, float* lse, void* stream) {
+static bool map_source_fits(int64_t rows, int64_t row_elems) { return rows > 0 && rows * row_elems * 2 < (int64_t(1) << 31); }
+
+int hct_attention_maps_supported(int B, int N, int H, int dh, int dtype) {
+  return dtype == HCT_BF16 && !g_force_simple_attention && B > 0 && H > 0 && attention_maps_supported(N, H, dh) &&
+                 map_source_fits((int64_t)B * N, (int64_t)3 * H * dh)
+             ? 1
+             : 0;
+}
+
+int hct_attention_fwd_mapped(const void* qkv, const int32_t* qkv_rows, int qkv_src_rows, int B, int N, int H, int dh, int dtype, void* o,
+                             float* lse, void* o_compact, const int32_t* o_rows, void* stream) {
   HCT_REQUIRE(B > 0 && N > 0 && H > 0 && dh > 0, "hct_attention_fwd: bad shape");
+  HCT_REQUIRE((o_compact == nullptr) == (o_rows == nullptr), "hct_attention_fwd_mapped: o_compact and o_rows come together");
   ProfScope ps(PROF_ATTN_FWD, 4.0 * B * H * (double)N * N * dh, (hipStream_t)stream);
+  if (qkv_rows || o_rows) {
+    HCT_REQUIRE(hct_attention_maps_supported(B, N, H, dh, dtype),
+                "hct_attention_fwd_mapped: row maps need bf16 at head dim 48 with 193 .. 224 tokens (hct_attention_maps_supported)");
+    const int src_rows = qkv_rows ? qkv_src_rows : B * N;
+    HCT_REQUIRE(map_source_fits(src_rows, (int64_t)3 * H * dh), "hct_attention_fwd_mapped: the qkv source must be 1 row .. under 2 GiB");
+    return attention_fwd_mapped_mfma(qkv, qkv_rows, src_rows, B, N, H, o, lse, o_compact, o_rows, (hipStream_t)stream);
+  }
   if (dtype == HCT_BF16 && !g_force_simple_attention && attention_mfma_supported(N, H, dh))
     return attention_fwd_mfma(qkv, B, N, H, dh, o, lse, (hipStream_t)stream);
   return attention_fwd_simple(qkv, B, N, H, dh, dtype, o, lse, (hipStream_t)stream);
 }
 
-int hct_attention_bwd(const void* qkv, const void* o, const void* d_o, const float* lse, int B, int N, int H, int dh,
-                      int dtype, void* dqkv, void* stream) {
+int hct_attention_fwd(const void* qkv, int B, int N, int H, int dh, int dtype, void* o, float* lse, void* stream) {
+  return hct_attention_fwd_mapped(qkv, nullptr, 0, B, N, H, dh, dtype, o, lse, nullptr, nullptr, stream);
+}
+
+int hct_attention_bwd_mapped(const void* qkv, const int32_t* qkv_rows, int qkv_src_rows, const void* o, const void* d_o,
+                             const int32_t* do_rows, int do_src_rows, const float* lse, int B, int N, int H, int dh, int dtype, void* dqkv,
+                             void* stream) {
   HCT_REQUIRE(B > 0 && N > 0 && H > 0 && dh > 0, "hct_attention_bwd: bad shape");
   ProfScope ps(PROF_ATTN_BWD, 10.0 * B * H * (double)N * N * dh, (hipStream_t)stream);
+  if (qkv_rows || do_rows) {
+    HCT_REQUIRE(hct_attention_maps_supported(B, N, H, dh, dtype),
+                "hct_attention_bwd_mapped: row maps need bf16 at head dim 48 with 193 .. 224 tokens (hct_attention_maps_supported)");
+    const int src_rows = qkv_rows ? qkv_src_rows : B * N, dsrc_rows = do_rows ? do_src_rows : B * N;
+    HCT_REQUIRE(map_source_fits(src_rows, (int64_t)3 * H * dh) && map_source_fits(dsrc_rows, (int64_t)H * dh),
+                "hct_attention_bwd_mapped: the qkv and dO sources must be 1 row .. under 2 GiB");
+    return attention_bwd_mapped_mfma(qkv, qkv_rows, src_rows, o, d_o, do_rows, dsrc_rows, lse, B, N, H, dqkv, (hipStream_t)stream);
+  }
   if (dtype == HCT_BF16 && !g_force_simple_attention && attention_mfma_supported(N, H, dh))
     return attention_bwd_mfma(qkv, o, d_o, lse, B, N, H, dh, dqkv, (hipStream_t)stream);
   return attention_bwd_simple(qkv, o, d_o, lse, B, N, H, dh, dtype, dqkv, (hipStream_t)stream);
+}
+
+int hct_attention_bwd(const void* qkv, const void* o, const void* d_o, const float* lse, int B, int N, int H, int dh,
+                      int dtype, void* dqkv, void* stream) {
+  return hct_attention_bwd_mapped(qkv, nullptr, 0, o, d_o, nullptr, 0, lse, B, N, H, dh, dtype, dqkv, stream);
 }
 
 int hct_attention_dropout_fwd(const void* qkv, int B, int N, int H, int dh, int dtype, float p, uint64_t seed, int site, void* o, float* lse,
diff --git a/headct_foundation_amd/csrc/attention_mfma.hip b/headct_foundation_amd/csrc/attention_mfma.hip
--- a/headct_foundation_amd/csrc/attention_mfma.hip
+++ b/headct_foundation_amd/csrc/attention_mfma.hip
@@ -45,6 +45,46 @@
     const int row = ci >> 3, slot = ci & 7;
     const uint32_t voff = (uint32_t)(row * (int)rs * 2 + ((slot ^ ((row >> 1) & 7)) << 4));
     __builtin_amdgcn_raw_ptr_buffer_load_lds(rsrc, (__attribute__((address_space(3))) void*)(img + p * 1024), 16, voff, 0, 0, 0);
+  }
+}
+
+struct AttnMaps {
+  const int32_t* qkv_rows = nullptr;
+  const int32_t* do_rows = nullptr;
+  const int32_t* o_rows = nullptr;
+  bf16* o_compact = nullptr;
+  int qkv_src_rows = 0, do_src_rows = 0;
+};
+constexpr uint32_t kZeroRow = 0x80000000u;
+
+template <int MAXP>
+__device__ __forceinline__ void map_image128_offsets(uint32_t (&voff)[MAXP], int64_t rs, const int32_t* __restrict__ rows, int row0, int N, int Npad,
+                                                     int wave, int nwaves, int lane) {
+  const int pieces = Npad * 8 / 64;
+#pragma unroll
+  for (int i = 0; i < MAXP; ++i) {
+    const int p = wave + i * nwaves;
+    voff[i] = kZeroRow;
+    if (p < pieces) {
+      const int ci = p * 64 + lane;
+      const int row = ci >> 3, slot = ci & 7;
+      if (row < N) {
+        const int sr = rows ? rows[row0 + row] : row0 + row;
+        voff[i] = (uint32_t)sr * (uint32_t)(rs * 2) + (uint32_t)((slot ^ ((row >> 1) & 7)) << 4);
+      }
+    }
+  }
+}
+template <int MAXP>
+__device__ __forceinline__ void dma_image128_offsets(unsigned char* img, const bf16* __restrict__ g, int64_t rs, const uint32_t (&voff)[MAXP],
+                                                     int src_rows, int Npad, int valid_cols, int wave, int nwaves) {
+  const int64_t bytes = ((int64_t)(src_rows - 1) * rs + valid_cols) * 2;
+  __amdgpu_buffer_rsrc_t rsrc = __builtin_amdgcn_make_buffer_rsrc((void*)g, 0, (uint32_t)bytes, 0x00020000);
+  const int pieces = Npad * 8 / 64;
+#pragma unroll
+  for (int i = 0; i < MAXP; ++i) {
+    const int p = wave + i * nwaves;
+    if (p < pieces) __builtin_amdgcn_raw_ptr_buffer_load_lds(rsrc, (__attribute__((address_space(3))) void*)(img + p * 1024), 16, voff[i], 0, 0, 0);
   }
 }
 
@@ -201,9 +241,9 @@
   }
 }
 
-template <int DH, int NT, int NW = (NT <= 4 ? 4 : 8)>
+template <int DH, int NT, int NW = (NT <= 4 ? 4 : 8), bool MAP = false>
 __global__ void __launch_bounds__(NW * 64) attn_fwd_row_kernel(const bf16* __restrict__ qkv, int N, int H, bf16* __restrict__ o,
-                                                           float* __restrict__ lse) {
+                                                           float* __restrict__ lse, AttnMaps mp) {
   constexpr int Npad = NT * 16;
   extern __shared__ __attribute__((aligned(16))) unsigned char smem[];
   unsigned char* Kimg = smem;
@@ -211,27 +251,49 @@
   const int lane = threadIdx.x & 63, wave = threadIdx.x >> 6;
   const int bh = xcd_bh(), b = bh / H, h = bh - b * H;
   const int64_t rs = (int64_t)3 * H * DH;
-  const bf16* qb = qkv + (int64_t)b * N * rs + h * DH;
+  const bf16* qb = MAP ? qkv + h * DH : qkv + (int64_t)b * N * rs + h * DH;
   const int g = lane >> 4;
   constexpr int ND = DH / 16;
   constexpr int MAXT = (NT + NW - 1) / NW;
   const int nqt = (N + 15) >> 4;
   constexpr int QA = MAXT <= 2 ? MAXT : 1;
   bf16x8 qall[QA][2];
+  static_assert(!MAP || MAXT <= 2, "the mapped instance fetches all of its Q fragments up front");
+  constexpr int MAXPC = MAP ? (Npad * 8 / 64 + NW - 1) / NW : 1;
+  uint32_t voff[MAXPC];
+  int64_t qsrc[QA];
+  if constexpr (MAP) {
+#pragma unroll
+    for (int it = 0; it < QA; ++it) {
+      const int q = (wave + it * NW) * 16 + (lane & 15);
+      qsrc[it] = 0;
+      if (q < N) qsrc[it] = mp.qkv_rows ? mp.qkv_rows[b * N + q] : b * N + q;
+    }
+    map_image128_offsets<MAXPC>(voff, rs, mp.qkv_rows, b * N, N, Npad, wave, NW, lane);
+  }
   auto load_q = [&](int it, bf16x8* dst) {
     const int q = (wave + it * NW) * 16 + (lane & 15);
 #pragma unroll
     for (int ks = 0; ks < 2; ++ks) {
       const int d = ks * 32 + 8 * g;
       bf16x8 v = {0, 0, 0, 0, 0, 0, 0, 0};
-      if (q < N && d < DH) v = *reinterpret_cast<const bf16x8*>(qb + (int64_t)q * rs + d);
+      if (q < N && d < DH) {
+        int64_t sr = q;
+        if constexpr (MAP) sr = qsrc[it];
+        v = *reinterpret_cast<const bf16x8*>(qb + sr * rs + d);
+      }
       dst[ks] = v;
     }
   };
 #pragma unroll
   for (int it = 0; it < QA; ++it) load_q(it, qall[it]);
-  dma_image128(Kimg, qb + H * DH, rs, N, Npad, DH, wave, NW, lane);
-  dma_image128(Vimg, qb + 2 * H * DH, rs, N, Npad, DH, wave, NW, lane);
+  if constexpr (MAP) {
+    dma_image128_offsets<MAXPC>(Kimg, qb + H * DH, rs, voff, mp.qkv_src_rows, Npad, DH, wave, NW);
+    dma_image128_offsets<MAXPC>(Vimg, qb + 2 * H * DH, rs, voff, mp.qkv_src_rows, Npad, DH, wave, NW);
+  } else {
+    dma_image128(Kimg, qb + H * DH, rs, N, Npad, DH, wave, NW, lane);
+    dma_image128(Vimg, qb + 2 * H * DH, rs, N, Npad, DH, wave, NW, lane);
+  }
   __syncthreads();
   const float scale = rsqrtf((float)DH) * 1.44269504088896340736f;
 #pragma unroll
@@ -243,6 +305,8 @@
     if constexpr (MAXT <= 2) { qf[0] = qall[it][0]; qf[1] = qall[it][1]; }
     else if (it == 0) { qf[0] = qall[0][0]; qf[1] = qall[0][1]; }
     else load_q(it, qf);
+    int crow = -1;
+    if constexpr (MAP) if (mp.o_rows && q < N) crow = mp.o_rows[b * N + q];
     f32x4 st[NT];
 #pragma unroll
     for (int t = 0; t < NT; ++t) {
@@ -283,6 +347,13 @@
       bf16* orow = o + ((int64_t)b * N + q) * (H * DH) + h * DH + 4 * g;
 #pragma unroll
       for (int dt = 0; dt < ND; ++dt) Vec4<bf16>::store(orow + dt * 16, oacc[dt] * inv);
+      if constexpr (MAP) {
+        if (crow >= 0) {
+          bf16* ocrow = mp.o_compact + (int64_t)crow * (H * DH) + h * DH + 4 * g;
+#pragma unroll
+          for (int dt = 0; dt < ND; ++dt) Vec4<bf16>::store(ocrow + dt * 16, oacc[dt] * inv);
+        }
+      }
       if (g == 0) lse[(int64_t)bh * N + q] = (mx + __builtin_amdgcn_logf(ps)) * 0.69314718055994530942f;
     }
   }
@@ -716,10 +787,10 @@
   asm volatile("s_mov_b32 m0, %0\n\ts_nop 0\n\tbuffer_load_dwordx4 %1, %2, 0 offen lds" ::"s"(lds_base), "v"(voff), "s"(rsrc) : "memory", "m0");
 }
 
-template <int DH, int Npad, int KT = 2>
+template <int DH, int Npad, int KT = 2, bool MAP = false>
 __global__ void __launch_bounds__(1024 / KT, 2 * 2 / KT) attn_bwd4_kernel(const bf16* __restrict__ qkv, const bf16* __restrict__ o,
                                                            const bf16* __restrict__ d_o, const float* __restrict__ lse, int N, int H,
-                                                           bf16* __restrict__ dqkv, int nbh) {
+                                                           bf16* __restrict__ dqkv, int nbh, AttnMaps mp) {
   extern __shared__ __attribute__((aligned(16))) unsigned char smem[];
   constexpr int ROW = HeadImg<DH>::kRow, CH = HeadImg<DH>::kChunks, ND = DH / 16, NW = 16 / KT;
   constexpr int img = Npad * ROW;
@@ -750,13 +821,34 @@
   else if (8 * KT * 16 > Npad) { dq_hh = 1; dq_dt0 = wave - 4; dq_n = (wave >= 4 && wave < 4 + ND) ? 1 : 0; }
   else { dq_hh = (wave - 2) / ND; dq_dt0 = (wave - 2) - dq_hh * ND; dq_n = wave >= 2 ? 1 : 0; }
 
+  uint32_t mq[MAXP], md[MAXP];
+  auto lookup = [&](int item) {
+    const int bh = item_bh(item), b = bh / H;
+    const int ln = opaque(lane);
+#pragma unroll
+    for (int i = 0; i < MAXP; ++i) {
+      const int p = wave + NW * i;
+      mq[i] = md[i] = kZeroRow;
+      if (p < pieces) {
+        const int ci = p * 64 + ln, row = ci / CH, slot = ci - row * CH;
+        const uint32_t src = (uint32_t)((DH == 48 ? slot : (slot ^ ((row >> 1) & 7))) * 16);
+        if (row < N) {
+          const int r = b * N + row;
+          const int sq = mp.qkv_rows ? mp.qkv_rows[r] : r, sd = mp.do_rows ? mp.do_rows[r] : r;
+          mq[i] = (uint32_t)sq * (uint32_t)(rs * 2) + src;
+          if (sd >= 0) md[i] = (uint32_t)sd * (uint32_t)(os * 2) + src;
+        }
+      }
+    }
+  };
   auto prefetch_images = [&](int item, int buf) {
     const int bh = item_bh(item), b = bh / H, h = bh - b * H;
-    const bf16* qb = qkv + (int64_t)b * N * rs + h * DH;
-    const bf16* dob = d_o + (int64_t)b * N * os + h * DH;
-    const attn_i32x4 rq = attn_srd(qb, ((int64_t)(N - 1) * rs + DH) * 2);
-    const attn_i32x4 rk = attn_srd(qb + H * DH, ((int64_t)(N - 1) * rs + DH) * 2);
-    const attn_i32x4 rd = attn_srd(dob, ((int64_t)(N - 1) * os + DH) * 2);
+    const bf16* qb = MAP ? qkv + h * DH : qkv + (int64_t)b * N * rs + h * DH;
+    const bf16* dob = MAP ? d_o + h * DH : d_o + (int64_t)b * N * os + h * DH;
+    const int qrows = MAP ? mp.qkv_src_rows : N, drows = MAP ? mp.do_src_rows : N;
+    const attn_i32x4 rq = attn_srd(qb, ((int64_t)(qrows - 1) * rs + DH) * 2);
+    const attn_i32x4 rk = attn_srd(qb + H * DH, ((int64_t)(qrows - 1) * rs + DH) * 2);
+    const attn_i32x4 rd = attn_srd(dob, ((int64_t)(drows - 1) * os + DH) * 2);
     const uint32_t base = lds0 + buf * bufsz;
     const int ln = opaque(lane);
 #pragma unroll
@@ -765,7 +857,8 @@
       if (p < pieces) {
         const int ci = p * 64 + ln, row = ci / CH, slot = ci - row * CH;
         const uint32_t src = (uint32_t)((DH == 48 ? slot : (slot ^ ((row >> 1) & 7))) * 16);
-        const uint32_t vq = (uint32_t)row * (uint32_t)(rs * 2) + src, vd = (uint32_t)row * (uint32_t)(os * 2) + src;
+        uint32_t vq = (uint32_t)row * (uint32_t)(rs * 2) + src, vd = (uint32_t)row * (uint32_t)(os * 2) + src;
+        if constexpr (MAP) { vq = mq[i]; vd = md[i]; }
         attn_dma16(rq, base + p * 1024, vq);
         attn_dma16(rd, base + img + p * 1024, vd);
         attn_dma16(rk, base + 2 * img + p * 1024, vq);
@@ -778,10 +871,20 @@
   float lN = 0.f;
   auto prefetch_regs = [&](int item) {
     const int bh = item_bh(item), b = bh / H, h = bh - b * H;
-    const bf16* vb = qkv + (int64_t)b * N * rs + 2 * H * DH + h * DH;
+    const bf16* vb = MAP ? qkv + 2 * H * DH + h * DH : qkv + (int64_t)b * N * rs + 2 * H * DH + h * DH;
     const int ln = opaque(lane), tid = wave * 64 + ln;
-#pragma unroll
-    for (int t = 0; t < KT; ++t) vfN[t] = rows_global<DH>(vb, rs, key_base + t * 16, ln, N);
+    if constexpr (MAP) {
+#pragma unroll
+      for (int t = 0; t < KT; ++t) {
+        const int key = key_base + t * 16 + (ln & 15);
+        int64_t sr = 0;
+        if (key < N) sr = mp.qkv_rows ? mp.qkv_rows[b * N + key] : b * N + key;
+        vfN[t] = rows_global<DH>(vb + sr * rs, 0, 0, ln, key < N ? 16 : 0);
+      }
+    } else {
+#pragma unroll
+      for (int t = 0; t < KT; ++t) vfN[t] = rows_global<DH>(vb, rs, key_base + t * 16, ln, N);
+    }
     const bf16* ob = o + (int64_t)b * N * os + h * DH;
 #pragma unroll
     for (int u = 0; u < NU; ++u) {
@@ -794,7 +897,9 @@
 
   int item = blockIdx.x;
   if (item >= nbh) return;
+  if constexpr (MAP) lookup(item);
   prefetch_images(item, 0);
+  if constexpr (MAP) if (item + (int)gridDim.x < nbh) lookup(item + gridDim.x);
   prefetch_regs(item);
   for (int it = 0; item < nbh; item += gridDim.x, ++it) {
     const int cur = it & 1;
@@ -947,6 +1052,7 @@
       asm volatile("s_waitcnt lgkmcnt(0)" ::: "memory");
       __builtin_amdgcn_s_barrier();
     }
+    if constexpr (MAP) if (next + (int)gridDim.x < nbh) lookup(next + gridDim.x);
     if (next < nbh) prefetch_regs(next);
     dq_part(nqb - 1, opaque(lane));
     if (owns_keys) {
@@ -1201,8 +1307,25 @@
 static int launch_fwd_row(const void* qkv, int B, int N, int H, void* o, float* lse, hipStream_t s) {
   const size_t lds = (size_t)2 * NT * 16 * kRowBytes;
   if (int rc = set_lds(attn_fwd_row_kernel<DH, NT>, lds)) return rc;
-  hipLaunchKernelGGL((attn_fwd_row_kernel<DH, NT>), dim3(B * H), dim3(NT <= 4 ? 256 : 512), lds, s, (const bf16*)qkv, N, H, (bf16*)o, lse);
+  hipLaunchKernelGGL((attn_fwd_row_kernel<DH, NT>), dim3(B * H), dim3(NT <= 4 ? 256 : 512), lds, s, (const bf16*)qkv, N, H, (bf16*)o, lse,
+                     AttnMaps{});
   return check_hip(hipGetLastError(), "attention_fwd_row");
+}
+
+bool attention_maps_supported(int N, int H, int dh) {
+  (void)H;
+  return !g_attn_general && dh == 48 && N > 192 && N <= 224;
+}
+
+int attention_fwd_mapped_mfma(const void* qkv, const int32_t* qkv_rows, int qkv_src_rows, int B, int N, int H, void* o, float* lse,
+                              void* o_compact, const int32_t* o_rows, hipStream_t s) {
+  constexpr int NT = 14;
+  const size_t lds = (size_t)2 * NT * 16 * kRowBytes;
+  AttnMaps mp;
+  mp.qkv_rows = qkv_rows; mp.qkv_src_rows = qkv_src_rows; mp.o_rows = o_rows; mp.o_compact = (bf16*)o_compact;
+  if (int rc = set_lds(attn_fwd_row_kernel<48, NT, 8, true>, lds)) return rc;
+  hipLaunchKernelGGL((attn_fwd_row_kernel<48, NT, 8, true>), dim3(B * H), dim3(512), lds, s, (const bf16*)qkv, N, H, (bf16*)o, lse, mp);
+  return check_hip(hipGetLastError(), "attention_fwd_row (mapped)");
 }
 
 static int num_cus_cached() {
@@ -1246,7 +1369,7 @@
     static_assert(l4 <= (size_t)kMaxLds, "bwd4 LDS");                                                                      \
     if (int rc = set_lds(attn_bwd4_kernel<DH_, NPAD_, 1>, l4)) return rc;                                                  \
     hipLaunchKernelGGL((attn_bwd4_kernel<DH_, NPAD_, 1>), dim3(grid), dim3(1024), l4, s, (const bf16*)qkv, (const bf16*)o, \
-                       (const bf16*)d_o, lse, N, H, (bf16*)dqkv, nbh);                                                     \
+                       (const bf16*)d_o, lse, N, H, (bf16*)dqkv, nbh, AttnMaps{});                                         \
     return check_hip(hipGetLastError(), "attention_bwd4");                                                                 \
   } while (0)
   if (!g_attn_general) {
@@ -1281,6 +1404,19 @@
   else { if (w16) HCT_BWD2(64, 16); else if (w8) HCT_BWD2(64, 8); else HCT_BWD2(64, 4); }
 #undef HCT_BWD2
   return check_hip(hipGetLastError(), "attention_bwd2_mfma");
+}
+
+int attention_bwd_mapped_mfma(const void* qkv, const int32_t* qkv_rows, int qkv_src_rows, const void* o, const void* d_o,
+                              const int32_t* do_rows, int do_src_rows, const float* lse, int B, int N, int H, void* dqkv, hipStream_t s) {
+  const int ncu = num_cus_cached();
+  const int nbh = B * H, grid = nbh < ncu ? nbh : ncu;
+  constexpr size_t l4 = bwd4_lds<48>(224);
+  AttnMaps mp;
+  mp.qkv_rows = qkv_rows; mp.qkv_src_rows = qkv_src_rows; mp.do_rows = do_rows; mp.do_src_rows = do_src_rows;
+  if (int rc = set_lds(attn_bwd4_kernel<48, 224, 1, true>, l4)) return rc;
+  hipLaunchKernelGGL((attn_bwd4_kernel<48, 224, 1, true>), dim3(grid), dim3(1024), l4, s, (const bf16*)qkv, (const bf16*)o, (const bf16*)d_o,
+                     lse, N, H, (bf16*)dqkv, nbh, mp);
+  return check_hip(hipGetLastError(), "attention_bwd4 (mapped)");
 }
 
 int attention_dropout_fwd_mfma(const void* qkv, int B, int N, int H, int dh, void* o, float* lse, const DropArgs& da, hipStream_t s) {
diff --git a/headct_foundation_amd/csrc/mae_plan.hip b/headct_foundation_amd/csrc/mae_plan.hip
--- a/headct_foundation_amd/csrc/mae_plan.hip
+++ b/headct_foundation_amd/csrc/mae_plan.hip
@@ -88,6 +88,7 @@
   Mode dec0;
   int Rcat = 0;
   size_t a_kept_rows = 0, a_cat_idx = 0, a_hk = 0, a_x1c = 0, a_mean_c = 0, a_rstd_c = 0, a_qkv_cat = 0, a_dqkv_cat = 0, a_dcat = 0;
+  Mode maps;
   std::vector<size_t> h_enc, h_dec;
   std::vector<BlockA> aenc, adec;
   size_t s_dh, s_dh_shadow, s_dx, s_do, s_small, s_small_bytes, s_gemm, s_gemm_bytes, s_nt_bytes = 0;
@@ -234,6 +235,84 @@
   }
 }
 
+constexpr int kTilesPerWg = 4;
+typedef __attribute__((ext_vector_type(4))) unsigned int tr_u32x4;
+
+__global__ void __launch_bounds__(256) transpose_bf16_batched_kernel(const unsigned short* __restrict__ src, unsigned short* __restrict__ dst,
+                                                                     TransposeTable t) {
+  __shared__ unsigned short tile[kTilesPerWg][64][66];
+  const int ntiles = t.tile_start[t.n];
+  const int l8 = threadIdx.x & 7, rs = threadIdx.x >> 3;
+  int rows[kTilesPerWg], cols[kTilesPerWg], r0[kTilesPerWg], c0[kTilesPerWg];
+  long long so[kTilesPerWg], dof[kTilesPerWg];
+  tr_u32x4 v[kTilesPerWg][2];
+#pragma unroll
+  for (int k = 0; k < kTilesPerWg; ++k) {
+    const int id = blockIdx.x * kTilesPerWg + k;
+    rows[k] = cols[k] = r0[k] = c0[k] = 0;
+    so[k] = dof[k] = 0;
+    if (id < ntiles) {
+      int lo = 0, hi = t.n;
+      while (hi - lo > 1) {
+        const int mid = (lo + hi) >> 1;
+        if (t.tile_start[mid] <= id) lo = mid; else hi = mid;
+      }
+      rows[k] = t.rows[lo]; cols[k] = t.cols[lo];
+      const int local = id - t.tile_start[lo], tcols = (cols[k] + 63) >> 6;
+      r0[k] = (local / tcols) * 64; c0[k] = (local % tcols) * 64;
+      so[k] = t.src[lo]; dof[k] = t.dst[lo];
+    }
+    if (((rows[k] | cols[k]) & 7) == 0) {
+#pragma unroll
+      for (int i = 0; i < 2; ++i) {
+        const int r = r0[k] + rs + 32 * i, c = c0[k] + l8 * 8;
+        v[k][i] = tr_u32x4{0, 0, 0, 0};
+        if (r < rows[k] && c < cols[k]) v[k][i] = *reinterpret_cast<const tr_u32x4*>(src + so[k] + (size_t)r * cols[k] + c);
+      }
+    }
+  }
+#pragma unroll
+  for (int k = 0; k < kTilesPerWg; ++k) {
+    if (((rows[k] | cols[k]) & 7) == 0) {
+#pragma unroll
+      for (int i = 0; i < 2; ++i) {
+        unsigned int* row = reinterpret_cast<unsigned int*>(&tile[k][rs + 32 * i][l8 * 8]);
+#pragma unroll
+        for (int e = 0; e < 4; ++e) row[e] = v[k][i][e];
+      }
+    } else {
+      const int tx = threadIdx.x & 63, ty = threadIdx.x >> 6;
+      for (int i = ty; i < 64; i += 4) {
+        const int r = r0[k] + i, c = c0[k] + tx;
+        tile[k][i][tx] = (r < rows[k] && c < cols[k]) ? src[so[k] + (size_t)r * cols[k] + c] : (unsigned short)0;
+      }
+    }
+  }
+  __syncthreads();
+#pragma unroll
+  for (int k = 0; k < kTilesPerWg; ++k) {
+    if (((rows[k] | cols[k]) & 7) == 0) {
+#pragma unroll
+      for (int i = 0; i < 2; ++i) {
+        const int c = c0[k] + rs + 32 * i, r = r0[k] + l8 * 8;
+        if (c < cols[k] && r < rows[k]) {
+          unsigned int w[4];
+#pragma unroll
+          for (int e = 0; e < 4; ++e)
+            w[e] = (unsigned int)tile[k][l8 * 8 + 2 * e][rs + 32 * i] | ((unsigned int)tile[k][l8 * 8 + 2 * e + 1][rs + 32 * i] << 16);
+          *reinterpret_cast<tr_u32x4*>(dst + dof[k] + (size_t)c * rows[k] + r) = tr_u32x4{w[0], w[1], w[2], w[3]};
+        }
+      }
+    } else {
+      const int tx = threadIdx.x & 63, ty = threadIdx.x >> 6;
+      for (int i = ty; i < 64; i += 4) {
+        const int c = c0[k] + i, r = r0[k] + tx;
+        if (c < cols[k] && r < rows[k]) dst[dof[k] + (size_t)c * rows[k] + r] = tile[k][tx][i];
+      }
+    }
+  }
+}
+
 struct WsAlloc {
   size_t cur = 0;
   size_t take(size_t bytes) {
@@ -504,7 +583,7 @@
     RC(dec0_table(p->pf(p->p_mask), p->pf(p->p_dpos), p->L, d, hk + (size_t)Nc * d, s));
     RC(norm_fwd(p, hk, p->pf(bp.ln1_w), p->pf(bp.ln1_b), Rc, d, 1e-5f, ws + p->a_x1c, p->dt, (float*)(ws + p->a_mean_c), (float*)(ws + p->a_rstd_c), s));
     RC(linear_fwd(p, ws + p->a_x1c, Rc, d, bp.qkv_w, bp.qkv_b, 3 * d, ws + p->a_qkv_cat, p->dt, HCT_ACT_NONE, nullptr, nullptr, s));
-    RC(hct_gather_rows(ws + p->a_qkv_cat, (const int32_t*)(ws + p->a_cat_idx), M, (int)(3 * d * p->esz()), ws + ba.qkv, s));
+    if (!p->maps.fwd) RC(hct_gather_rows(ws + p->a_qkv_cat, (const int32_t*)(ws + p->a_cat_idx), M, (int)(3 * d * p->esz()), ws + ba.qkv, s));
   } else {
     RC(norm_fwd(p, h_in, p->pf(bp.ln1_w), p->pf(bp.ln1_b), M, d, 1e-5f, ws + ba.x1, p->dt, (float*)(ws + ba.mean1), (float*)(ws + ba.rstd1), s));
     RC(linear_fwd(p, ws + ba.x1, M, d, bp.qkv_w, bp.qkv_b, 3 * d, ws + ba.qkv, p->dt, HCT_ACT_NONE, nullptr, nullptr, s));
@@ -512,12 +591,18 @@
   }
   if (p->drop.fwd)
     RC(hct_attention_dropout_fwd(ws + ba.qkv, B, N, heads, d / heads, p->dt, p->drop_p, p->drop_seed, bp.site, ws + ba.o, (float*)(ws + ba.lse), s));
+  else if (p->maps.fwd && rows == Rows::kCat)
+    RC(hct_attention_fwd_mapped(ws + p->a_qkv_cat, (const int32_t*)(ws + p->a_cat_idx), p->Rcat, B, N, heads, d / heads, p->dt, ws + ba.o,
+                                (float*)(ws + ba.lse), nullptr, nullptr, s));
+  else if (p->maps.fwd && rows == Rows::kTail)
+    RC(hct_attention_fwd_mapped(ws + ba.qkv, nullptr, 0, B, N, heads, d / heads, p->dt, ws + ba.o, (float*)(ws + ba.lse), ws + p->a_oc,
+                                (const int32_t*)(ws + p->a_tail_inv), s));
   else
     RC(hct_attention_fwd(ws + ba.qkv, B, N, heads, d / heads, p->dt, ws + ba.o, (float*)(ws + ba.lse), s));
   if (rows != Rows::kTail) return back_half_forward(p, bp, ba, M, ws + ba.o, h_in, h_out, d, sd.m, s);
   const int32_t* tail_rows = (const int32_t*)(ws + p->a_tail_rows);
   float* hin_c = (float*)(ws + p->s_dh);
-  RC(hct_gather_rows(ws + ba.o, tail_rows, p->Mc, (int)(d * p->esz()), ws + p->a_oc, s));
+  if (!p->maps.fwd) RC(hct_gather_rows(ws + ba.o, tail_rows, p->Mc, (int)(d * p->esz()), ws + p->a_oc, s));
   RC(hct_gather_rows(h_in, tail_rows, p->Mc, d * 4, hin_c, s));
   return back_half_forward(p, bp, ba, p->Mc, ws + p->a_oc, hin_c, h_out, d, sd.m, s);
 }
@@ -566,13 +651,19 @@
   if (tail) {
     const int32_t* inv = (const int32_t*)(ws + p->a_tail_inv);
     RC(back_half_backward(p, bp, ba, bg, p->Mc, ws + p->a_oc, (float*)(ws + p->s_dhc), dx, d, sd.m, s));
-    RC(hct_gather_rows(dx, inv, M, (int)(d * p->esz()), d_o, s));
+    if (!p->maps.fwd) RC(hct_gather_rows(dx, inv, M, (int)(d * p->esz()), d_o, s));
   } else {
     RC(back_half_backward(p, bp, ba, bg, M, ws + ba.o, dh, d_o, d, sd.m, s));
   }
   if (drop)
     RC(hct_attention_dropout_bwd(ws + ba.qkv, ws + ba.o, d_o, (const float*)(ws + ba.lse), B, N, heads, d / heads, p->dt, p->drop_p, p->drop_seed,
                                  bp.site, dqkv, s));
+  else if (p->maps.fwd && tail)
+    RC(hct_attention_bwd_mapped(ws + ba.qkv, nullptr, 0, ws + ba.o, dx, (const int32_t*)(ws + p->a_tail_inv), p->Mc, (const float*)(ws + ba.lse), B, N,
+                                heads, d / heads, p->dt, dqkv, s));
+  else if (p->maps.fwd && rows == Rows::kCat)
+    RC(hct_attention_bwd_mapped(ws + p->a_qkv_cat, (const int32_t*)(ws + p->a_cat_idx), p->Rcat, ws + ba.o, d_o, nullptr, 0,
+                                (const float*)(ws + ba.lse), B, N, heads, d / heads, p->dt, dqkv, s));
   else
     RC(hct_attention_bwd(ws + ba.qkv, ws + ba.o, d_o, (const float*)(ws + ba.lse), B, N, heads, d / heads, p->dt, dqkv, s));
   if (rows == Rows::kCat) {
@@ -626,6 +717,7 @@
   auto off = [](const char* name) { const char* v = getenv(name); return v && v[0] == '0'; };
   p->defer_folds = !off("HCT_DEFER_FOLDS");
   p->dec0.on = p->dec0.can && !off("HCT_DEC0_TABLE");
+  p->maps.on = p->maps.can && !off("HCT_ROW_MAPS");
   p->wg_defer = p->dt == HCT_BF16 && !off("HCT_WGRAD_DEFER");
   const char* eb = getenv("HCT_WGRAD_GROUP_BLOCKS");
   p->wg_blocks = eb && *eb ? std::max(0, atoi(eb)) : 0;
@@ -740,6 +832,7 @@
   p->drop.can = p->drop_p > 0.f;
   p->tail.can = !p->vit && p->cfg.decoder_depth >= 1 && p->Mc > 0 && (p->Dd * es) % 16 == 0;
   p->dec0.can = !p->vit && p->cfg.decoder_depth >= 2 && (p->Dd * es) % 16 == 0 && (3 * p->Dd * es) % 16 == 0;
+  p->maps.can = !p->vit && p->dt == HCT_BF16 && p->lora == 0;
   read_env(p);
 
   WsAlloc w;
@@ -907,6 +1000,11 @@
   p->dec0.on = on != 0 && p->dec0.can;
   return p->dec0.on ? 1 : 0;
 }
+int hct_mae_plan_set_row_maps(hct_mae_plan* p, int on) {
+  if (!p) return -1;
+  p->maps.on = on != 0 && p->maps.can;
+  return p->maps.on ? 1 : 0;
+}
 int hct_mae_plan_set_dropout(hct_mae_plan* p, int active, uint64_t seed) {
   if (!p) return -1;
   p->drop.on = active != 0 && p->drop.can;
@@ -936,6 +1034,22 @@
   return 0;
 }
 
+int hct_weight_transpose(const void* src, int src_dtype, int rows, int cols, void* dst, void* stream) {
+  HCT_REQUIRE(src && dst && rows > 0 && cols > 0 && (src_dtype == HCT_F32 || src_dtype == HCT_BF16), "hct_weight_transpose: bad arguments");
+  HCT_REQUIRE(((uintptr_t)src | (uintptr_t)dst) % 16 == 0, "hct_weight_transpose: 16-byte aligned matrices");
+  TransposeTable t;
+  t.n = 1;
+  t.rows[0] = rows; t.cols[0] = cols; t.src[0] = 0; t.dst[0] = 0;
+  t.tile_start[0] = 0;
+  t.tile_start[1] = ((rows + 63) / 64) * ((cols + 63) / 64);
+  if (src_dtype == HCT_F32)
+    hipLaunchKernelGGL(transpose_cast_batched_kernel, dim3(t.tile_start[1]), dim3(256), 0, (hipStream_t)stream, (const float*)src, (bf16*)dst, t);
+  else
+    hipLaunchKernelGGL(transpose_bf16_batched_kernel, dim3((t.tile_start[1] + kTilesPerWg - 1) / kTilesPerWg), dim3(256), 0,
+                       (hipStream_t)stream, (const unsigned short*)src, (unsigned short*)dst, t);
+  return check_hip(hipGetLastError(), "hct_weight_transpose");
+}
+
 int hct_mae_refresh_weights(hct_mae_plan* p, int with_plain, void* stream) {
   HCT_REQUIRE(p && p->params_f32, "hct_mae_refresh_weights: plan not bound");
   if (p->dt != HCT_BF16) return 0;
@@ -945,8 +1059,8 @@
   t.tile_start[0] = 0;
   auto flush = [&]() -> int {
     if (t.n == 0) return 0;
-    hipLaunchKernelGGL(transpose_cast_batched_kernel, dim3(t.tile_start[t.n]), dim3(256), 0, (hipStream_t)stream, p->params_f32,
-                       p->params_bf16_t, t);
+    hipLaunchKernelGGL(transpose_bf16_batched_kernel, dim3((t.tile_start[t.n] + kTilesPerWg - 1) / kTilesPerWg), dim3(256), 0,
+                       (hipStream_t)stream, (const unsigned short*)p->params_bf16, (unsigned short*)p->params_bf16_t, t);
     t.n = 0;
     return check_hip(hipGetLastError(), "hct_mae_refresh_weights");
   };
@@ -975,6 +1089,7 @@
   p->path.fwd = false;
   p->tail.fwd = p->tail.can && p->tail.on && !p->drop.fwd;
   p->dec0.fwd = p->dec0.can && p->dec0.on && !p->drop.fwd;
+  p->maps.fwd = p->maps.can && p->maps.on && !p->drop.fwd && hct_attention_maps_supported(p->B, p->Nd, p->Hd, p->Dd / p->Hd, p->dt) == 1;
   const bool tail = p->tail.fwd, dec0 = p->dec0.fwd;
   int32_t* ids_restore = (int32_t*)(ws + p->a_ids_restore);
   int32_t* ids_shuffle = (int32_t*)(ws + p->a_ids_shuffle);
diff --git a/headct_foundation_amd/mae.py b/headct_foundation_amd/mae.py
--- a/headct_foundation_amd/mae.py
+++ b/headct_foundation_amd/mae.py
@@ -24,6 +24,8 @@
         plan.tail = bool(plan.lib.hct_mae_plan_set_tail(plan.handle, int(train and not dropping and not getattr(model, "full_pred", False))) == 1)
         if not getattr(model, "dec0_table", True):
             plan.lib.hct_mae_plan_set_dec0(plan.handle, 0)
+        if not getattr(model, "row_maps", True):
+            plan.lib.hct_mae_plan_set_row_maps(plan.handle, 0)
         _lib.check(plan.lib.hct_mae_forward(plan.handle, x.data_ptr(), _lib.dtype_code(x), noise.data_ptr(), plan.loss.data_ptr(),
                                             float(model._grad_prescale) if train else 0.0, st), "hct_mae_forward")
         plan.serial += 1
diff --git a/include/headct_hip.h b/include/headct_hip.h
--- a/include/headct_hip.h
+++ b/include/headct_hip.h
@@ -116,6 +116,12 @@
 int hct_attention_fwd(const void* qkv, int B, int N, int H, int dh, int dtype, void* o, float* lse, void* stream);
 int hct_attention_bwd(const void* qkv, const void* o, const void* d_o, const float* lse, int B, int N, int H,
                       int dh, int dtype, void* dqkv, void* stream);
+int hct_attention_maps_supported(int B, int N, int H, int dh, int dtype);
+int hct_attention_fwd_mapped(const void* qkv, const int32_t* qkv_rows, int qkv_src_rows, int B, int N, int H, int dh, int dtype,
+                             void* o, float* lse, void* o_compact, const int32_t* o_rows, void* stream);
+int hct_attention_bwd_mapped(const void* qkv, const int32_t* qkv_rows, int qkv_src_rows, const void* o, const void* d_o,
+                             const int32_t* do_rows, int do_src_rows, const float* lse, int B, int N, int H, int dh, int dtype,
+                             void* dqkv, void* stream);
 
 int hct_dropout_mask(uint64_t seed, int site, int kind, int64_t n, int BH, int N, float p, unsigned char* out, void* stream);
 int hct_dropout_apply(const void* x, int x_dtype, void* y, int y_dtype, const float* residual, const void* x2, void* y2,
@@ -325,10 +331,12 @@
 int hct_mae_plan_len_keep(const hct_mae_plan*);
 int hct_mae_plan_set_tail(hct_mae_plan*, int compact);
 int hct_mae_plan_set_dec0(hct_mae_plan*, int on);
+int hct_mae_plan_set_row_maps(hct_mae_plan*, int on);
 int hct_mae_plan_set_dropout(hct_mae_plan*, int active, uint64_t seed);
 int hct_mae_plan_bind(hct_mae_plan*, float* params, float* grads, void* params_bf16, void* params_bf16_t,
                       void* workspace, size_t workspace_bytes);
 int hct_mae_refresh_weights(hct_mae_plan*, int with_plain, void* stream);
+int hct_weight_transpose(const void* src, int src_dtype, int rows, int cols, void* dst, void* stream);
 int hct_mae_forward(hct_mae_plan*, const void* x, int x_dtype, const float* noise, float* loss, float grad_scale, void* stream);
 int hct_mae_set_loss_grad(hct_mae_plan*, const float* dloss);
 int hct_mae_num_backward_stages(const hct_mae_plan*);
```

After: 7155 CT-volumes/s, median of 6. About the same (+0.5%).
